# mmeidlinger/lut_ldpc

Hardware: AMD Instinct MI355X
Metric: decoded codewords/sec, DVB-S2 N=64800 4-bit LUT 50-iter (higher is better)
Workload: dtype u8

## Files before the change

### include/lut_ldpc_hip.h

```cpp
#ifndef LUT_LDPC_HIP_H
#define LUT_LDPC_HIP_H

#include <stdint.h>
#include <stddef.h>

#ifdef __cplusplus
extern "C" {
#endif

#define LUTLDPC_OK               0
#define LUTLDPC_ERR_ARG         -1
#define LUTLDPC_ERR_PARSE       -2
#define LUTLDPC_ERR_UNSUPPORTED -3
#define LUTLDPC_ERR_HIP         -4
#define LUTLDPC_ERR_STATE       -5

typedef struct lutldpc_decoder lutldpc_decoder;

const char *lutldpc_last_error(void);

const char *lutldpc_version(void);

int lutldpc_device_count(void);

int lutldpc_decoder_create(int nvar, int nchk, const int32_t *dv, const int32_t *dc,
                           const int32_t *cn_msg_idx,
                           int Nq_Cha, const int32_t *Nq_Msg, const uint8_t *reuse_vec, int max_iters,
                           int min_lut, const char *var_trees_txt, const char *chk_trees_txt,
                           int device, lutldpc_decoder **out);

int lutldpc_decoder_destroy(lutldpc_decoder *d);

int lutldpc_decoder_set_exit_conditions(lutldpc_decoder *d, int max_iters, int psc, int pisc);

int lutldpc_decoder_decode_batch(lutldpc_decoder *d, const uint8_t *cha, const uint8_t *msg0, int B,
                                 uint8_t *out_bits, int32_t *out_iters);

#define LUTLDPC_IN_BYTES   0
#define LUTLDPC_IN_NIBBLES 1
typedef struct {
    int32_t in_format;
    const int32_t *cha2msg_map;
    int32_t out_first, out_count;
} lutldpc_packed_io;

int lutldpc_decoder_decode_batch_packed(lutldpc_decoder *d, const lutldpc_packed_io *io, const uint8_t *cha, const uint8_t *msg0,
                                        int B, uint32_t *out_words, int32_t *out_iters);

int lutldpc_decoder_decode_batch_device(lutldpc_decoder *d, const uint8_t *d_cha, const uint8_t *d_msg0, int B,
                                        uint8_t *d_out_bits, int32_t *d_out_iters, int sync);

int lutldpc_decoder_decode_batch_trace(lutldpc_decoder *d, const uint8_t *cha, const uint8_t *msg0, int B, int level, uint8_t *out_bits,
                                       int32_t *out_iters, uint8_t *trace, int64_t trace_cap, int32_t *n_dumps);

int lutldpc_decoder_decode_llr_batch(lutldpc_decoder *d, const double *llr, int B,
                                     const double *qb_Cha, int n_qb_Cha,
                                     const double *qb_Msg, int n_qb_Msg,
                                     int initial_message_mode, const int32_t *cha2msg_map,
                                     uint8_t *out_bits, int32_t *out_iters);

#define LUTLDPC_LLR_F64 0
#define LUTLDPC_LLR_F32 1
#define LUTLDPC_LLR_F16 2
#define LUTLDPC_LLR_I8  3
typedef struct {
    int32_t dtype;
    int32_t on_device;
    int64_t frame_stride;
    double  scale;
    const double *qb_Cha; int32_t n_qb_Cha;
    const double *qb_Msg; int32_t n_qb_Msg;
    int32_t initial_message_mode; const int32_t *cha2msg_map;
    int32_t out_first, out_count;
    int32_t sync;
} lutldpc_llr_io;
int lutldpc_decoder_decode_llr_packed(lutldpc_decoder *d, const lutldpc_llr_io *io, const void *llr, int B,
                                      uint32_t *out_words, int32_t *out_iters, uint8_t *out_cha, uint8_t *out_msg0);

int lutldpc_llr_cell_table(const lutldpc_llr_io *io, int Nq_Cha, int Nq_Msg0,
                           double *thr, int32_t thr_cap, int32_t *n_thr,
                           uint8_t lut_cha[256], uint8_t lut_msg[256]);

typedef struct {
    int32_t n_cells;
    const uint64_t *thr;
    const uint8_t *cha_label;
    const uint8_t *msg_label;
    const uint8_t *slicer_neg;
    const uint8_t *cha_label_mirror;
    const uint8_t *msg_label_mirror;
} lutldpc_channel_cells;

#define LUTLDPC_STREAM_MAX 0x7FFFFFFFu
int lutldpc_check_stream(uint32_t stream);

int lutldpc_decoder_sim_batch(lutldpc_decoder *d, const lutldpc_channel_cells *cells, uint64_t seed, uint32_t stream,
                              uint64_t frame0, int B, const uint8_t *codewords, int K_info, int32_t *frame_stats,
                              uint8_t *cha_out, uint8_t *bits_out);

int lutldpc_decoder_set_generator(lutldpc_decoder *d, int K, int R, const uint64_t *rows);
int lutldpc_decoder_encode_random(lutldpc_decoder *d, uint64_t seed, uint32_t stream, uint64_t frame0, int B, uint8_t *codewords);
int lutldpc_decoder_sim_batch_random(lutldpc_decoder *d, const lutldpc_channel_cells *cells, uint64_t seed, uint32_t stream,
                                     uint64_t frame0, int B, int K_info, int32_t *frame_stats, uint8_t *cha_out, uint8_t *bits_out);

int lutldpc_decoder_sample_labels(lutldpc_decoder *d, const lutldpc_channel_cells *cells, uint64_t seed, uint32_t stream,
                                  uint64_t frame0, int B, const uint8_t *codewords, uint8_t *cha, uint8_t *msg0);

int lutldpc_decoder_set_edge_groups(lutldpc_decoder *d, const int32_t *edge_group, int n_groups);
int lutldpc_decoder_histogram_shape(lutldpc_decoder *d, int level, int32_t *out4);
int lutldpc_decoder_histogram_batch(lutldpc_decoder *d, const uint8_t *cha, const uint8_t *msg0, const uint8_t *sent, int B, int level, int mode,
                                    int n_labels, uint8_t *out_bits, int32_t *out_iters, int64_t *hist, int64_t hist_cap, int32_t *n_dumps);
int lutldpc_decoder_sim_batch_histogram(lutldpc_decoder *d, const lutldpc_channel_cells *cells, uint64_t seed, uint32_t stream, uint64_t frame0,
                                        int B, const uint8_t *codewords, int device_codewords, int level, int mode, int n_labels,
                                        int64_t *hist, int64_t hist_cap, int32_t *n_dumps);

#define LUTLDPC_EV_CODEWORD   0
#define LUTLDPC_EV_INFO       1
#define LUTLDPC_EV_FAILED     2
#define LUTLDPC_EV_UNDETECTED 3
typedef struct {
    int32_t select;
    int32_t max_frames, max_pos, max_chk;
    int32_t *events;
    int32_t *positions;
    int32_t *checks;
    int64_t *node_errors;
    int64_t *check_fails;
    int32_t n_selected;
    int32_t n_stored;
} lutldpc_event_request;

int lutldpc_decoder_events_batch(lutldpc_decoder *d, const uint8_t *cha, const uint8_t *msg0, const uint8_t *sent, int B, int K_info,
                                 uint8_t *out_bits, int32_t *out_iters, lutldpc_event_request *req);
int lutldpc_decoder_sim_batch_events(lutldpc_decoder *d, const lutldpc_channel_cells *cells, uint64_t seed, uint32_t stream, uint64_t frame0,
                                     int B, const uint8_t *codewords, int device_codewords, int K_info, int32_t *frame_stats,
                                     lutldpc_event_request *req);

void *lutldpc_decoder_stream(lutldpc_decoder *d);

#define LUTLDPC_K_CN_PASS   0
#define LUTLDPC_K_VN_PASS   1
#define LUTLDPC_K_DECISION  2
#define LUTLDPC_K_SYNDROME  3
#define LUTLDPC_K_LAYOUT    4
#define LUTLDPC_K_FRONTEND  5
#define LUTLDPC_K_FUSED_PASS 6
#define LUTLDPC_K_RESIDENT  7
#define LUTLDPC_K_HISTOGRAM 8
#define LUTLDPC_K_COUNT     9

int lutldpc_decoder_set_profiling(lutldpc_decoder *d, int enable);
int lutldpc_decoder_get_profile(lutldpc_decoder *d, int kind, double *total_ms, int64_t *launches);
int lutldpc_decoder_reset_profile(lutldpc_decoder *d);
int64_t lutldpc_decoder_device_bytes(lutldpc_decoder *d);
const char *lutldpc_decoder_describe(lutldpc_decoder *d);

int lutldpc_selftest_program_eval(lutldpc_decoder *d, int kind, int set, int cls,
                                  const int32_t *in, int n_in, int32_t *out, int n_out);
int lutldpc_selftest_program_stats(lutldpc_decoder *d, int kind, int set, int cls,
                                   int32_t *n_ops, int32_t *n_ops_naive, int32_t *n_slots);

int64_t lutldpc_selftest_jit_source(lutldpc_decoder *d, int kind, int set, int cls, char *buf, int64_t cap, int compile);
int64_t lutldpc_selftest_resident_source(lutldpc_decoder *d, int G, char *buf, int64_t cap, int compile, int32_t *info);

#ifdef __cplusplus
}
#endif
#endif
```

### lut_ldpc_amd/_capi.py

```python
from __future__ import annotations

import ctypes as C
import os
from pathlib import Path

_PKG = Path(__file__).resolve().parent
LIB_PATH = _PKG / "lib" / "liblut_ldpc_amd.so"
if os.environ.get("LUTLDPC_LIB"):
    LIB_PATH = Path(os.environ["LUTLDPC_LIB"])

OK, ERR_ARG, ERR_PARSE, ERR_UNSUPPORTED, ERR_HIP, ERR_STATE = 0, -1, -2, -3, -4, -5
K_CN_PASS, K_VN_PASS, K_DECISION, K_SYNDROME, K_LAYOUT, K_FRONTEND, K_FUSED_PASS, K_RESIDENT, K_HISTOGRAM, K_COUNT = 0, 1, 2, 3, 4, 5, 6, 7, 8, 9
KIND_NAMES = ["cn_pass", "vn_pass", "decision", "syndrome", "layout", "frontend", "fused_pass", "resident", "histogram"]


class LutLdpcError(RuntimeError):
    def __init__(self, code: int, msg: str):
        super().__init__(f"[{code}] {msg}")
        self.code = code


def _load() -> C.CDLL:
    if not LIB_PATH.exists():
        raise ImportError(
            f"{LIB_PATH} is missing: build it with `python -c 'import __graft_entry__ as g; g.build()'` "
            "or `make -C lut_ldpc_amd/csrc` (hipcc, gfx950). There is no CPU fallback."
        )
    return C.CDLL(str(LIB_PATH), mode=C.RTLD_GLOBAL)


lib = _load()

_vp, _ip, _u8p, _dp, _cp = C.c_void_p, C.POINTER(C.c_int32), C.POINTER(C.c_uint8), C.POINTER(C.c_double), C.c_char_p
_i64p = C.POINTER(C.c_int64)


class EventRequest(C.Structure):
    _fields_ = [("select", C.c_int32), ("max_frames", C.c_int32), ("max_pos", C.c_int32), ("max_chk", C.c_int32),
                ("events", _ip), ("positions", _ip), ("checks", _ip), ("node_errors", _i64p), ("check_fails", _i64p),
                ("n_selected", C.c_int32), ("n_stored", C.c_int32)]


_evp = C.POINTER(EventRequest)
IN_BYTES, IN_NIBBLES = 0, 1


class PackedIO(C.Structure):
    _fields_ = [("in_format", C.c_int32), ("cha2msg_map", _ip), ("out_first", C.c_int32), ("out_count", C.c_int32)]


LLR_F64, LLR_F32, LLR_F16, LLR_I8 = 0, 1, 2, 3


class LlrIO(C.Structure):
    _fields_ = [("dtype", C.c_int32), ("on_device", C.c_int32), ("frame_stride", C.c_int64), ("scale", C.c_double),
                ("qb_Cha", _dp), ("n_qb_Cha", C.c_int32), ("qb_Msg", _dp), ("n_qb_Msg", C.c_int32),
                ("initial_message_mode", C.c_int32), ("cha2msg_map", _ip), ("out_first", C.c_int32), ("out_count", C.c_int32),
                ("sync", C.c_int32)]


_u32p = C.POINTER(C.c_uint32)
_SIGNATURES = {
    "lutldpc_decoder_decode_llr_packed": (C.c_int, [_vp, C.POINTER(LlrIO), _vp, C.c_int, _vp, _vp, _vp, _vp]),
    "lutldpc_llr_cell_table": (C.c_int, [C.POINTER(LlrIO), C.c_int, C.c_int, _dp, C.c_int32, _ip, _u8p, _u8p]),
    "lutldpc_last_error": (_cp, []),
    "lutldpc_version": (_cp, []),
    "lutldpc_device_count": (C.c_int, []),
    "lutldpc_decoder_create": (C.c_int, [C.c_int, C.c_int, _ip, _ip, _ip, C.c_int, _ip, _u8p, C.c_int, C.c_int, _cp, _cp, C.c_int,
                                         C.POINTER(_vp)]),
    "lutldpc_decoder_destroy": (C.c_int, [_vp]),
    "lutldpc_decoder_set_exit_conditions": (C.c_int, [_vp, C.c_int, C.c_int, C.c_int]),
    "lutldpc_decoder_decode_batch": (C.c_int, [_vp, _u8p, _u8p, C.c_int, _u8p, _ip]),
    "lutldpc_decoder_decode_batch_packed": (C.c_int, [_vp, C.POINTER(PackedIO), _u8p, _u8p, C.c_int, _u32p, _ip]),
    "lutldpc_decoder_decode_batch_device": (C.c_int, [_vp, _vp, _vp, C.c_int, _vp, _vp, C.c_int]),
    "lutldpc_decoder_decode_llr_batch": (C.c_int, [_vp, _dp, C.c_int, _dp, C.c_int, _dp, C.c_int, C.c_int, _ip, _u8p, _ip]),
    "lutldpc_decoder_stream": (_vp, [_vp]),
    "lutldpc_decoder_set_profiling": (C.c_int, [_vp, C.c_int]),
    "lutldpc_decoder_get_profile": (C.c_int, [_vp, C.c_int, _dp, C.POINTER(C.c_int64)]),
    "lutldpc_decoder_reset_profile": (C.c_int, [_vp]),
    "lutldpc_decoder_device_bytes": (C.c_int64, [_vp]),
    "lutldpc_decoder_describe": (_cp, [_vp]),
    "lutldpc_selftest_program_eval": (C.c_int, [_vp, C.c_int, C.c_int, C.c_int, _ip, C.c_int, _ip, C.c_int]),
    "lutldpc_selftest_program_stats": (C.c_int, [_vp, C.c_int, C.c_int, C.c_int, _ip, _ip, _ip]),
    "lutldpc_decoder_decode_batch_trace": (C.c_int, [_vp, _u8p, _u8p, C.c_int, C.c_int, _u8p, _ip, _u8p, C.c_int64, _ip]),
    "lutldpc_selftest_jit_source": (C.c_int64, [_vp, C.c_int, C.c_int, C.c_int, C.c_char_p, C.c_int64, C.c_int]),
    "lutldpc_selftest_resident_source": (C.c_int64, [_vp, C.c_int, C.c_char_p, C.c_int64, C.c_int, C.POINTER(C.c_int32)]),
    "lutldpc_check_stream": (C.c_int, [C.c_uint32]),
    "lutldpc_decoder_set_generator": (C.c_int, [_vp, C.c_int, C.c_int, C.POINTER(C.c_uint64)]),
    "lutldpc_decoder_encode_random": (C.c_int, [_vp, C.c_uint64, C.c_uint32, C.c_uint64, C.c_int, _u8p]),
    "lutldpc_decoder_sim_batch_random": (C.c_int, [_vp, _vp, C.c_uint64, C.c_uint32, C.c_uint64, C.c_int, C.c_int, _ip, _u8p, _u8p]),
    "lutldpc_decoder_set_edge_groups": (C.c_int, [_vp, _ip, C.c_int]),
    "lutldpc_decoder_histogram_shape": (C.c_int, [_vp, C.c_int, _ip]),
    "lutldpc_decoder_histogram_batch": (C.c_int, [_vp, _u8p, _u8p, _u8p, C.c_int, C.c_int, C.c_int, C.c_int, _u8p, _ip, _i64p, C.c_int64, _ip]),
    "lutldpc_decoder_sim_batch_histogram": (C.c_int, [_vp, _vp, C.c_uint64, C.c_uint32, C.c_uint64, C.c_int, _u8p, C.c_int, C.c_int, C.c_int, C.c_int,
                                                      _i64p, C.c_int64, _ip]),
    "lutldpc_decoder_events_batch": (C.c_int, [_vp, _u8p, _u8p, _u8p, C.c_int, C.c_int, _u8p, _ip, _evp]),
    "lutldpc_decoder_sim_batch_events": (C.c_int, [_vp, _vp, C.c_uint64, C.c_uint32, C.c_uint64, C.c_int, _u8p, C.c_int, C.c_int, _ip, _evp]),
}
for _name, (_res, _args) in _SIGNATURES.items():
    if hasattr(lib, _name):
        _fn = getattr(lib, _name)
        _fn.restype, _fn.argtypes = _res, _args


def last_error() -> str:
    return lib.lutldpc_last_error().decode()


def check(rc: int) -> None:
    if rc != OK:
        raise LutLdpcError(rc, last_error())


def device_count() -> int:
    return lib.lutldpc_device_count()

_HOST_SIGNATURES = {
    "lutldpc_codec_create": (C.c_int, [_cp, C.c_int, C.c_int, C.c_int, C.POINTER(_vp)]),
    "lutldpc_codec_load": (C.c_int, [_cp, C.c_int, C.POINTER(_vp)]),
    "lutldpc_codec_save": (C.c_int, [_vp, _cp]),
    "lutldpc_codec_destroy": (C.c_int, [_vp]),
    "lutldpc_codec_design_luts": (C.c_int, [_vp, _cp, C.c_int, C.c_double, C.c_int, _u8p, C.c_int, _ip, C.c_int, _dp]),
    "lutldpc_codec_design_from_cache": (C.c_int, [_vp]),
    "lutldpc_codec_set_exit_conditions": (C.c_int, [_vp, C.c_int, C.c_int, C.c_int]),
    "lutldpc_codec_set_initial_message_mode": (C.c_int, [_vp, C.c_int]),
    "lutldpc_codec_initial_message_mode": (C.c_int, [_vp]),
    "lutldpc_codec_set_output_verbosity": (C.c_int, [_vp, C.c_int]),
    "lutldpc_codec_dims": (C.c_int, [_vp, _ip, _ip, _ip, _ip]),
    "lutldpc_codec_graph": (C.c_int, [_vp, _ip, _ip, _ip]),
    "lutldpc_codec_var_trees_txt": (C.c_int64, [_vp, C.c_char_p, C.c_int64]),
    "lutldpc_codec_chk_trees_txt": (C.c_int64, [_vp, C.c_char_p, C.c_int64]),
    "lutldpc_codec_qb": (C.c_int, [_vp, C.c_int, _dp, C.c_int]),
    "lutldpc_codec_cha2msg_map": (C.c_int, [_vp, _ip, C.c_int]),
    "lutldpc_codec_rate": (C.c_double, [_vp]),
    "lutldpc_codec_decoder": (_vp, [_vp]),
    "lutldpc_codec_decode_llr_batch": (C.c_int, [_vp, _dp, C.c_int, _u8p, _ip]),
    "lutldpc_codec_lut_decode_batch": (C.c_int, [_vp, _u8p, _u8p, C.c_int, _u8p, _ip]),
    "lutldpc_codec_lut_decode_dump": (C.c_int64, [_vp, _u8p, _u8p, C.c_int, C.c_int, _u8p, _ip, C.c_char_p, C.c_int64]),
    "lutldpc_codec_encode": (C.c_int, [_vp, _u8p, _u8p]),
    "lutldpc_de_threshold": (C.c_int, [_ip, _dp, C.c_int, _ip, _dp, C.c_int, C.c_int, C.c_int, C.c_int, C.c_int, _cp, _cp, C.c_double,
                                       C.c_double, C.c_double, C.c_int, C.c_int, C.c_double, C.c_int, _dp]),
}
for _name, (_res, _args) in _HOST_SIGNATURES.items():
    if hasattr(lib, _name):
        _fn = getattr(lib, _name)
        _fn.restype, _fn.argtypes = _res, _args

_u64p, _i64p = C.POINTER(C.c_uint64), C.POINTER(C.c_int64)
_SIM_SIGNATURES = {
    "lutldpc_codec_sim_batch": (C.c_int, [_vp, C.c_double, C.c_uint64, C.c_uint32, C.c_uint64, C.c_int, C.c_int, _ip]),
    "lutldpc_codec_sample_labels": (C.c_int, [_vp, C.c_double, C.c_uint64, C.c_uint32, C.c_uint64, C.c_int, C.c_int, _u8p, _u8p, _u8p]),
    "lutldpc_codec_encode_random": (C.c_int, [_vp, C.c_uint64, C.c_uint32, C.c_uint64, C.c_int, _u8p]),
    "lutldpc_codec_channel_cells": (C.c_int, [_vp, C.c_double, _u64p, _u8p, _u8p, _u8p, _u8p, _u8p]),
    "lutldpc_ber_sim_run": (C.c_int, [_cp, _cp, C.c_int, _cp, C.c_int, C.c_int, C.c_int, _dp, _i64p, C.c_int]),
    "lutldpc_ber_sim_main": (C.c_int, [C.c_int, C.POINTER(C.c_char_p)]),
    "lutldpc_selftest_write_results_it": (C.c_int, [_cp, _dp, _i64p, C.c_int, C.c_int, C.c_int, C.c_double]),
    "lutldpc_bersim_create": (C.c_int, [_cp, _cp, C.c_int, _cp, C.c_int, C.POINTER(_vp)]),
    "lutldpc_bersim_destroy": (C.c_int, [_vp]),
    "lutldpc_bersim_info": (C.c_int, [_vp, _i64p, _dp, _dp, C.c_int]),
    "lutldpc_bersim_batch": (C.c_int, [_vp, C.c_int, C.c_int64, C.c_int, _ip]),
    "lutldpc_bersim_add_point": (C.c_int, [_vp, C.c_double, _i64p]),
    "lutldpc_bersim_save": (C.c_int, [_vp, C.c_double]),
    "lutldpc_bersim_results_path": (C.c_int64, [_vp, C.c_char_p, C.c_int64]),
    "lutldpc_codec_message_histogram": (C.c_int, [_vp, C.c_double, C.c_uint64, C.c_uint32, C.c_uint64, C.c_int, C.c_int, C.c_int, C.c_int, C.c_int,
                                                  _i64p, C.c_int64, _ip]),
    "lutldpc_bersim_message_histogram": (C.c_int, [_vp, C.c_int, C.c_int64, C.c_int, C.c_int, C.c_int, C.c_int, _i64p, C.c_int64, _ip]),
    "lutldpc_codec_error_events": (C.c_int, [_vp, C.c_double, C.c_uint64, C.c_uint32, C.c_uint64, C.c_int, C.c_int, _evp]),
    "lutldpc_bersim_error_events": (C.c_int, [_vp, C.c_int, C.c_int64, C.c_int, _evp]),
    "lutldpc_bersim_decoder": (_vp, [_vp]),
    "lutldpc_bersim_code": (C.c_int, [_vp, _ip, _ip, _ip, _ip, _ip]),
}
for _name, (_res, _args) in _SIM_SIGNATURES.items():
    if hasattr(lib, _name):
        _fn = getattr(lib, _name)
        _fn.restype, _fn.argtypes = _res, _args
```

### lut_ldpc_amd/csrc/hip/decoder.hip

```cpp
#include "decoder_state.hpp"

#include <climits>
#include <cstdlib>

#pragma GCC visibility push(hidden)

static thread_local std::string g_err;
int fail(int code, const std::string &msg) { g_err = msg; return code; }

hipEvent_t ev_get(lutldpc_decoder *d) {
    if (!d->ev_pool.empty()) { hipEvent_t e = d->ev_pool.back(); d->ev_pool.pop_back(); return e; }
    hipEvent_t e;
    (void)hipEventCreate(&e);
    return e;
}
void prof_fold(lutldpc_decoder *d) {
    if (d->ev_live.empty()) return;
    (void)hipStreamSynchronize(d->stream);
    for (auto &e : d->ev_live) {
        float ms = 0;
        if (hipEventElapsedTime(&ms, e.a, e.b) == hipSuccess) { d->prof_ms[e.kind] += ms; d->prof_n[e.kind]++; }
        d->ev_pool.push_back(e.a); d->ev_pool.push_back(e.b);
    }
    d->ev_live.clear();
}

static uint32_t crc32(uint32_t crc, const void *p, size_t n) {
    crc = ~crc;
    for (size_t i = 0; i < n; i++) {
        crc ^= static_cast<const uint8_t *>(p)[i];
        for (int k = 0; k < 8; k++) crc = (crc >> 1) ^ (0xEDB88320u & (0u - (crc & 1u)));
    }
    return ~crc;
}

void make_describe(lutldpc_decoder *d) {
    std::ostringstream o;
    o << "{\"build\":\"" << __DATE__ << " " << __TIME__ << "\",\"kernel_sources\":\"" <<
#include "kernel_src_hash.inc"
      << "\",\"tile_frames\":" << d->tile() << ",\"message_bytes\":" << (d->pack == 2 ? "0.5" : "1") << ",\"pack\":" << d->pack << ",\"vector_bytes_per_lane\":4"
      << ",\"nodes_per_block\":" << d->opt.nodes_per_block << ",\"vn_edges_per_wave\":" << d->opt.vn_edges_per_wave << ",\"cn_edges_per_wave\":" << d->cn_epw() << ",\"use_fast\":" << d->opt.use_fast
      << ",\"nodes_per_wave\":" << d->opt.nodes_per_wave << ",\"nodes_per_wave_cn\":" << d->opt.nodes_per_wave_cn << ",\"tail_front\":" << d->opt.tail_front
      << ",\"fused_prio\":" << d->opt.fused_prio << ",\"chk_full_labels\":" << d->opt.chk_full_labels
      << ",\"vn_classes\":[";
    for (size_t i = 0; i < d->vclass.size(); i++) {
        const TreeClassPlan *t = d->tree_class(TT_VAR, 0, (int)i);
        const bool f = t && fast_covers(d, t->fast, d->vclass[i].deg);
        o << (i ? "," : "") << "{\"deg\":" << d->vclass[i].deg << ",\"nodes\":" << d->vclass[i].nodes.size() << ",\"nodes_per_wave\":" << d->npw_vn(d->vclass[i].deg) << ",\"kernel\":\""
          << (f ? "vn_balanced_fast_kernel" : t && t->jit ? "lutldpc_jit_pass" : "tree_pass_kernel<VAR>") << "\"}";
    }
    o << "],\"cn_classes\":[";
    for (size_t i = 0; i < d->cclass.size(); i++) {
        int n_fast = 0;
        for (int nq : d->Nq_Msg)
            n_fast += d->opt.use_fast && d->min_lut && cn_minsum_shape(nq / 2, d->cclass[i].deg);
        const char *minsum = n_fast == (int)d->Nq_Msg.size() ? "cn_minsum_fast_kernel"
                           : n_fast == 0 ? "cn_minsum_generic_kernel" : "cn_minsum_fast_kernel+cn_minsum_generic_kernel";
        int chained = 0;
        if (d->opt.use_chain && d->cclass[i].chain_off >= 0)
            for (size_t j = 0; j < d->cclass[i].nodes.size(); j++) chained += d->fast_idx[(size_t)d->cclass[i].chain_off + 2 * j + 1] != 0;
        const TreeClassPlan *t = d->tree_class(TT_CHK, 0, (int)i);
        o << (i ? "," : "") << "{\"deg\":" << d->cclass[i].deg << ",\"nodes\":" << d->cclass[i].nodes.size() << ",\"nodes_per_wave\":" << d->npw_cn_class(i)
          << ",\"chain_nodes\":" << chained << ",\"kernel\":\""
          << (d->min_lut ? minsum
                         : t && t->jit ? "lutldpc_jit_pass" : "tree_pass_kernel<CHK>") << "\"}";
    }
    o << "],\"resident\":" << (resident_active(d) ? 1 : 0) << ",\"skewed_pipeline\":" << ((d->opt.skew && d->skew_ok) ? 1 : 0) << ",\"fused_bucket\":" << d->fused_bucket_id << ",\"compaction\":" << (d->opt.use_compact < 0 ? 2 : d->opt.use_compact) << ",\"compaction_min_groups\":" << compaction_min_groups(d) << ",\"chain_nodes\":" << (d->opt.use_chain ? d->n_chain_nodes : 0) << ",\"placement\":" << d->place_info;
    if (d->gen_set) o << ",\"generator\":{\"K\":" << d->gen_K << ",\"R\":" << d->gen_R << "}";
    {
        uint32_t ops = 0;
        for (const Op &op : d->all_ops) ops = crc32(crc32(ops, &op, offsetof(Op, child) + sizeof(op.child)), &op.mult, sizeof(Op) - offsetof(Op, mult));
        char b[160];
        snprintf(b, sizeof(b), ",\"static\":{\"ops\":%zu,\"ops_crc\":\"%08x\",\"tables_bytes\":%zu,\"tables_crc\":\"%08x\",\"index_words\":%zu,\"index_crc\":\"%08x\"}", d->all_ops.size(), ops,
                 d->all_tables.size(), crc32(0, d->all_tables.data(), d->all_tables.size()), d->fast_idx.size(), crc32(0, d->fast_idx.data(), 4 * d->fast_idx.size()));
        o << b;
    }
    o << "}";
    d->describe = o.str();
}

using Options = lutldpc_decoder::Options;
enum KnobType { FLAG, INT, REAL, REAL_BELOW };
struct Knob { const char *name; KnobType type; int Options::*i; double Options::*r; double lo, hi; const char *meaning; };
#define KNOB_F(name, field, meaning) {name, FLAG, &Options::field, nullptr, 0, 1, meaning}
#define KNOB_I(name, field, lo, hi, meaning) {name, INT, &Options::field, nullptr, lo, hi, meaning}
#define KNOB_R(name, type, field, lo, hi, meaning) {name, type, nullptr, &Options::field, lo, hi, meaning}
static const Knob kKnobs[] = {
    KNOB_F("LUTLDPC_USE_FAST", use_fast, "1: compile-time specialised kernels (and with them the fused pipeline, the generated kernels, the resident decoder); 0: interpreter kernels only"),
    KNOB_F("LUTLDPC_JIT", use_jit, "1: run-time generated kernels for shapes the compile-time path does not cover (jit.hpp)"),
    KNOB_I("LUTLDPC_PACK", pack, 1, 1, "1: byte rows even where every alphabet has <= 16 labels (unset: nibble rows there)"),
    KNOB_F("LUTLDPC_CHK_FULL", chk_full_labels, "1: generated check kernels on full-label tables; 0: on (sign, magnitude) tables as the reference walks them"),
    KNOB_F("LUTLDPC_COMPOSE", use_compose, "1: exact table composition for the resident kernel's trees (measured slower: LDS bank conflicts, see compile_all)"),
    KNOB_I("LUTLDPC_COMPOSE_SPACE", compose_space, 0, 65536, "largest composed table, entries"),
    KNOB_F("LUTLDPC_CHAIN", use_chain, "1: degree-2 nodes between neighbouring checks of a wave are updated inside the check pass (build_fast_index)"),
    KNOB_F("LUTLDPC_LATE_HARD", late_hard, "1: decided bits of early-terminated frames recovered once, at the end, from their frozen messages; 0: stored by every variable pass"),
    KNOB_F("LUTLDPC_FIRST_FROM_NODES", first_from_nodes, "1: the first check pass reads the initial-message rows; 0: init_edges_kernel copies them to the edge rows first"),
    KNOB_I("LUTLDPC_NODES_PER_BLOCK", nodes_per_block, 1, 4096, "interpreter kernels: nodes per 64-thread block"),
    KNOB_I("LUTLDPC_NODES_PER_WAVE", nodes_per_wave, 1, 4096, "specialised kernels: fixed nodes per wave, variable AND check side (unset: edges per wave / degree)"),
    KNOB_I("LUTLDPC_NODES_PER_WAVE_CN", nodes_per_wave_cn, 1, 4096, "... check side only (overrides LUTLDPC_NODES_PER_WAVE there)"),
    KNOB_I("LUTLDPC_VN_EDGES_PER_WAVE", vn_edges_per_wave, 1, 65536, "variable side: edges per wave"),
    KNOB_I("LUTLDPC_CN_EDGES_PER_WAVE", cn_edges_per_wave, 1, 65536, "check side: edges per wave (unset: 42, chain-rich classes widened by build_fast_index; given: no widening)"),
    KNOB_F("LUTLDPC_SKEW", skew, "1: two-half skewed pipeline through pass_fused_kernel where every class has a case in it"),
    KNOB_I("LUTLDPC_FUSED_BUCKET_MIN", fused_bucket_min, 0, kFusedBuckets - 1, "run a code of small degrees through a wider bucket's fused kernel (can only widen; what a bucket costs)"),
    KNOB_F("LUTLDPC_PRIO", fused_prio, "1: the look-up-heavy (variable) waves of the fused kernel raise their issue priority (no gain measured)"),
    KNOB_R("LUTLDPC_TAIL_FRONT", REAL_BELOW, tail_front, 0, 0.9, "fused launches: share of the item list that the slowest role stays clear of at the end"),
    KNOB_I("LUTLDPC_PLACE", place_candidates, 0, 32, "placement search of the row buffers: at most n candidate allocations, 0 / 1: off (place_rows)"),
    KNOB_F("LUTLDPC_GRAPH", use_graph, "1: repeated decodes replayed as one hipGraph launch"),
    KNOB_F("LUTLDPC_COMPACT", use_compact, "1 / 0: on / off (unset: automatic, long iterations only -- compaction_on)"),
    KNOB_F("LUTLDPC_COMPACT_KEEP", compact_keep, "1: frames that left keep their rows, bits recovered once at the end; 0: recovered at the check point, rows dropped"),
    KNOB_I("LUTLDPC_COMPACT_FIRST", compact_first, 1, INT_MAX, "first iteration with a check point"),
    KNOB_I("LUTLDPC_COMPACT_EVERY", compact_every, 1, INT_MAX, "iterations between check points (unset: 2)"),
    KNOB_R("LUTLDPC_COMPACT_MARGIN", REAL_BELOW, compact_margin, 0, 100, "permute when the remaining iterations pay for it by this factor (0: whenever a group falls idle)"),
    KNOB_R("LUTLDPC_COMPACT_MIN_SHARE", REAL, compact_min_share, 0, 1, "... and at least this share of the live groups falls idle at once"),
    KNOB_I("LUTLDPC_RESIDENT", use_resident, INT_MIN, INT_MAX, "0: off (streaming kernels); 1: where the code fits and it pays; >= 2: wherever it fits"),
    KNOB_I("LUTLDPC_RESIDENT_S", resident_force_S, 1, 64, "sets (64 frames each) per workgroup (unset: resident_pick)"),
    KNOB_I("LUTLDPC_RESIDENT_NT", resident_force_NT, 256, 1024, "threads per workgroup: 256, 512, 768 or 1024 (unset: resident_pick)"),
    KNOB_I("LUTLDPC_RESIDENT_U", resident_U, 1, 4, "frames per lane step of the variable items: 1, 2 or 4 (unset: generator's choice)"),
    KNOB_F("LUTLDPC_RESIDENT_XCD", resident_xcd, "1: workgroup ids remapped so that neighbours share an XCD"),
    KNOB_F("LUTLDPC_RESIDENT_FM", resident_fm, "1: the kernel reads / writes the caller's frame-major buffers itself; 0: always through the row layout"),
    KNOB_F("LUTLDPC_RESIDENT_FLAG_REDUCE", resident_flag_reduce, "wave-reduced exit-test flags (unset: small trees only, resident_spec)"),
    KNOB_F("LUTLDPC_RESIDENT_CN_PERSISTENT", resident_cn_persistent, "check items keep their LDS addresses in registers (unset: where registers allow, resident_spec)"),
    KNOB_I("LUTLDPC_RESIDENT_WAVES_EU", resident_waves_eu, 0, 8, "amdgpu_waves_per_eu of the generated kernel (0: none)"),
    KNOB_F("LUTLDPC_VALIDATE", validate, "1: the class parameters of every per-class launch checked against the allocation sizes (fused roles always are), stream synchronised after every launch so that a device fault names ONE launch; no graph replay"),
    KNOB_F("LUTLDPC_DEBUG_ADDR", debug_addr, "1: print where the row buffers landed (tools/config4_place_ab.sh)"),
};
#undef KNOB_F
#undef KNOB_I
#undef KNOB_R

static void read_knobs(Options &o) {
    for (const Knob &k : kKnobs) {
        const char *e = getenv(k.name);
        if (!e) continue;
        if (k.type == FLAG) o.*k.i = atoi(e) ? 1 : 0;
        else if (k.type == INT) { const int v = atoi(e); if (v >= k.lo && v <= k.hi) o.*k.i = v; }
        else { const double v = atof(e); if (v >= k.lo && (k.type == REAL ? v <= k.hi : v < k.hi)) o.*k.r = v; }
    }
    if (o.nodes_per_wave_cn == 0) o.nodes_per_wave_cn = o.nodes_per_wave;
    o.use_resident = o.use_resident >= 2 ? 2 : o.use_resident ? 1 : 0;
    if (o.resident_force_NT % 256) o.resident_force_NT = 0;
    if (o.resident_U == 3) o.resident_U = 0;
    if (o.validate) o.use_graph = 0;
    o.compact_margin = (float)o.compact_margin; o.compact_min_share = (float)o.compact_min_share;
}

lutldpc_decoder::~lutldpc_decoder() {
    if (device < 0) return;
    (void)hipSetDevice(device);
    if (stream) (void)hipStreamSynchronize(stream);
    drop_graphs();
    for (auto &e : ev_live) { (void)hipEventDestroy(e.a); (void)hipEventDestroy(e.b); }
    for (auto &e : ev_pool) (void)hipEventDestroy(e);
}

static int decode_staged_labels(lutldpc_decoder *d, int B, uint8_t *out_bits, int32_t *out_iters) {
    const size_t n = (size_t)B * (size_t)d->nvar;
    HIP_TRY(d->d_out_bits.alloc(n)); HIP_TRY(d->d_out_iters.alloc((size_t)B));
    int rc = decode_device(d, d->d_in_cha.p, d->d_in_msg.p, B, d->d_out_bits.p, d->d_out_iters.p);
    if (rc || (rc = copy_to_host(d, out_bits, d->d_out_bits.p, n)) || (rc = iters_to_host(d, out_iters, B))) return rc;
    HIP_TRY(hipStreamSynchronize(d->stream));
    return LUTLDPC_OK;
}

struct TraceScope {
    lutldpc_decoder *d;
    explicit TraceScope(lutldpc_decoder *d_) : d(d_) {}
    ~TraceScope() { d->trace = lutldpc_decoder::Trace(); }
};

#pragma GCC visibility pop

extern "C" {

const char *lutldpc_last_error(void) { return g_err.c_str(); }
void lutldpc_set_last_error(const char *msg) { g_err = msg ? msg : ""; }
const char *lutldpc_version(void) { return "lut_ldpc_amd 0.1 gfx950"; }

int lutldpc_device_count(void) {
    int n = 0;
    if (hipGetDeviceCount(&n) != hipSuccess) return 0;
    return n;
}

int lutldpc_decoder_create(int nvar, int nchk, const int32_t *dv, const int32_t *dc, const int32_t *cn_msg_idx,
                           int Nq_Cha, const int32_t *Nq_Msg, const uint8_t *reuse_vec, int max_iters,
                           int min_lut, const char *var_trees_txt, const char *chk_trees_txt, int device,
                           lutldpc_decoder **out) {
    if (!out) return fail(LUTLDPC_ERR_ARG, "out is NULL");
    *out = nullptr;
    if (nvar <= 0 || nchk <= 0 || !dv || !dc || !cn_msg_idx || !Nq_Msg || !reuse_vec || max_iters < 1 || !var_trees_txt)
        return fail(LUTLDPC_ERR_ARG, "missing or non-positive argument");
    if (Nq_Cha < 2 || Nq_Cha > 128 || (Nq_Cha & 1)) return fail(LUTLDPC_ERR_ARG, "Nq_Cha must be even and in [2,128]");
    for (int i = 0; i < max_iters; i++)
        if (Nq_Msg[i] < 2 || Nq_Msg[i] > 128 || (Nq_Msg[i] & 1)) return fail(LUTLDPC_ERR_ARG, "Nq_Msg entries must be even and in [2,128]");
    if (reuse_vec[0] || reuse_vec[max_iters - 1]) return fail(LUTLDPC_ERR_ARG, "first and last iteration are exempt from tree reuse");
    std::unique_ptr<lutldpc_decoder> d(new lutldpc_decoder);
    d->nvar = nvar; d->nchk = nchk;
    d->dv.assign(dv, dv + nvar); d->dc.assign(dc, dc + nchk);
    long long ev = 0, ec = 0;
    for (int v = 0; v < nvar; v++) { if (dv[v] < 1 || dv[v] > 255) return fail(LUTLDPC_ERR_ARG, "variable degree outside [1,255]"); ev += dv[v]; }
    for (int c = 0; c < nchk; c++) { if (dc[c] < 1 || dc[c] > 255) return fail(LUTLDPC_ERR_ARG, "check degree outside [1,255]"); ec += dc[c]; }
    if (ev != ec || ev > (1ll << 30)) return fail(LUTLDPC_ERR_ARG, "sum(dv) != sum(dc)");
    d->E = (int)ev;
    d->cn_msg_idx.assign(cn_msg_idx, cn_msg_idx + d->E);
    d->vn_ptr.resize((size_t)nvar + 1); d->cn_ptr.resize((size_t)nchk + 1);
    for (int v = 0; v < nvar; v++) d->vn_ptr[(size_t)v + 1] = d->vn_ptr[(size_t)v] + dv[v];
    for (int c = 0; c < nchk; c++) d->cn_ptr[(size_t)c + 1] = d->cn_ptr[(size_t)c] + dc[c];
    {
        d->edge_vn.resize((size_t)d->E);
        for (int v = 0; v < nvar; v++) for (int e = d->vn_ptr[(size_t)v]; e < d->vn_ptr[(size_t)v + 1]; e++) d->edge_vn[(size_t)e] = v;
        std::vector<uint8_t> seen((size_t)d->E, 0);
        d->cn_vn.resize((size_t)d->E);
        for (int k = 0; k < d->E; k++) {
            int e = cn_msg_idx[k];
            if (e < 0 || e >= d->E || seen[(size_t)e]) return fail(LUTLDPC_ERR_ARG, "cn_msg_idx is not a permutation of the edges");
            seen[(size_t)e] = 1;
            d->cn_vn[(size_t)k] = d->edge_vn[(size_t)e];
        }
    }
    if ((uint64_t)d->E * kRowBytes >= (1ull << 32) || (uint64_t)nvar * kRowBytes >= (1ull << 32))
        return fail(LUTLDPC_ERR_UNSUPPORTED, "code too large: the rows of one frame group must stay below 4 GiB");
    build_classes(d->dv, d->vclass, d->vn_list);
    build_classes(d->dc, d->cclass, d->cn_list);
    d->Nq_Cha = Nq_Cha; d->Nq_Msg.assign(Nq_Msg, Nq_Msg + max_iters);
    d->max_iters_created = d->max_iters = max_iters; d->psc = 1; d->pisc = 0; d->min_lut = min_lut ? 1 : 0;
    d->iter_set.resize((size_t)max_iters);
    { int cum = 0; for (int i = 0; i < max_iters; i++) { cum += reuse_vec[i] ? 0 : 1; d->iter_set[(size_t)i] = cum - 1; } }
    std::string err;
    if (!parse_tree_array(var_trees_txt, d->var_trees, err)) return fail(LUTLDPC_ERR_PARSE, "var_trees_txt: " + err);
    if (!d->min_lut) {
        if (!chk_trees_txt || !parse_tree_array(chk_trees_txt, d->chk_trees, err)) return fail(LUTLDPC_ERR_PARSE, "chk_trees_txt: " + err);
    }
    read_knobs(d->opt);
    d->pack = 2;
    if (Nq_Cha > 16 || d->opt.pack == 1) d->pack = 1;
    for (int i = 0; i < max_iters; i++) if (Nq_Msg[i] > 16) d->pack = 1;
    int rc = compile_all(d.get());
    if (rc) return rc;
    d->skew_ok = skew_eligible(d.get());
    {
        int max_cn = 0, max_vn = 0;
        for (auto &c : d->cclass) max_cn = std::max(max_cn, c.deg);
        for (auto &c : d->vclass) max_vn = std::max(max_vn, c.deg);
        d->fused_bucket_id = std::max(0, fused_bucket(max_vn, max_cn));
        const int v = d->opt.fused_bucket_min;
        if (v >= 0 && fused_bucket_rank(v) > fused_bucket_rank(d->fused_bucket_id)) d->fused_bucket_id = v;
    }
    d->device = device;
    if (device >= 0) { rc = upload_static(d.get()); if (rc) return rc; }
    d->resident_ok = resident_eligible(d.get());
    make_describe(d.get());
    *out = d.release();
    return LUTLDPC_OK;
}

int lutldpc_decoder_destroy(lutldpc_decoder *d) {
    if (!d) return LUTLDPC_OK;
    delete d;
    return LUTLDPC_OK;
}

int lutldpc_decoder_set_exit_conditions(lutldpc_decoder *d, int max_iters, int psc, int pisc) {
    if (!d) return fail(LUTLDPC_ERR_ARG, "NULL decoder");
    if (max_iters < 1 || max_iters > d->max_iters_created) return fail(LUTLDPC_ERR_ARG, "max_iters outside [1, value at creation]");
    if (!d->tree_set(TT_DEC, d->iter_set[(size_t)(max_iters - 1)])->valid)
        return fail(LUTLDPC_ERR_ARG, "the tree set of iteration max_iters-1 is not a decision tree set");
    d->max_iters = max_iters; d->psc = psc ? 1 : 0; d->pisc = pisc ? 1 : 0;
    return LUTLDPC_OK;
}

int lutldpc_decoder_decode_batch_device(lutldpc_decoder *d, const uint8_t *d_cha, const uint8_t *d_msg0, int B,
                                        uint8_t *d_out_bits, int32_t *d_out_iters, int sync) {
    if (!d || !d_cha || !d_msg0 || !d_out_bits || !d_out_iters) return fail(LUTLDPC_ERR_ARG, "NULL argument");
    int rc = batch_entry(d, B);
    if (rc || (rc = decode_device(d, d_cha, d_msg0, B, d_out_bits, d_out_iters))) return rc;
    if (sync) HIP_TRY(hipStreamSynchronize(d->stream));
    return LUTLDPC_OK;
}

int lutldpc_decoder_decode_batch(lutldpc_decoder *d, const uint8_t *cha, const uint8_t *msg0, int B, uint8_t *out_bits, int32_t *out_iters) {
    if (!d || !cha || !msg0 || !out_bits || !out_iters) return fail(LUTLDPC_ERR_ARG, "NULL argument");
    int rc = batch_entry(d, B);
    if (rc || (rc = labels_from_host(d, cha, msg0, B))) return rc;
    return decode_staged_labels(d, B, out_bits, out_iters);
}

int lutldpc_decoder_decode_batch_trace(lutldpc_decoder *d, const uint8_t *cha, const uint8_t *msg0, int B, int level, uint8_t *out_bits, int32_t *out_iters,
                                       uint8_t *trace, int64_t trace_cap, int32_t *n_dumps) {
    if (!d || !cha || !msg0 || !out_bits || !out_iters || !trace) return fail(LUTLDPC_ERR_ARG, "NULL argument");
    if (level < 2 || level > 3) return fail(LUTLDPC_ERR_ARG, "trace level must be 2 or 3");
    int rc = batch_entry(d, B);
    if (rc) return rc;
    if (B > 4096) return fail(LUTLDPC_ERR_ARG, "the message trace is a debug path: 1..4096 frames");
    const int64_t need = (int64_t)(1 + d->max_iters * (level - 1)) * B * d->E;
    if (trace_cap < need) return fail(LUTLDPC_ERR_ARG, "trace buffer too small: " + std::to_string(need) + " bytes needed");
    TraceScope scope(d);
    d->trace.level = level; d->trace.host = trace; d->trace.cap = (size_t)trace_cap; d->trace.n = 0; d->trace.B = B;
    if ((rc = labels_from_host(d, cha, msg0, B)) == LUTLDPC_OK) rc = decode_staged_labels(d, B, out_bits, out_iters);
    if (n_dumps) *n_dumps = d->trace.n;
    return rc;
}

int lutldpc_decoder_decode_llr_batch(lutldpc_decoder *d, const double *llr, int B, const double *qb_Cha, int n_qb_Cha,
                                     const double *qb_Msg, int n_qb_Msg, int mode, const int32_t *map,
                                     uint8_t *out_bits, int32_t *out_iters) {
    if (!d || !llr || !qb_Cha || !out_bits || !out_iters) return fail(LUTLDPC_ERR_ARG, "NULL argument");
    int rc = batch_entry(d, B);
    if (rc) return rc;
    if (n_qb_Cha != d->Nq_Cha - 1) return fail(LUTLDPC_ERR_ARG, "qb_Cha must hold Nq_Cha-1 boundaries");
    if (mode == 0 && (!qb_Msg || n_qb_Msg != d->Nq_Msg[0] - 1)) return fail(LUTLDPC_ERR_ARG, "qb_Msg must hold Nq_Msg[0]-1 boundaries");
    if (mode == 1 && !map) return fail(LUTLDPC_ERR_ARG, "QCHA mode needs cha2msg_map");
    if (mode != 0 && mode != 1) return fail(LUTLDPC_ERR_ARG, "initial_message_mode must be 0 (CONT) or 1 (QCHA)");
    size_t n = (size_t)B * (size_t)d->nvar;
    HIP_TRY(d->d_llr.alloc(n)); HIP_TRY(d->d_in_cha.alloc(n)); HIP_TRY(d->d_in_msg.alloc(n));
    HIP_TRY(d->d_qb_cha.alloc((size_t)n_qb_Cha)); HIP_TRY(d->d_qb_msg.alloc((size_t)(n_qb_Msg > 0 ? n_qb_Msg : 1))); HIP_TRY(d->d_map.alloc((size_t)d->Nq_Cha));
    HIP_TRY(hipMemcpyAsync(d->d_llr.p, llr, n * sizeof(double), hipMemcpyHostToDevice, d->stream));
    HIP_TRY(hipMemcpyAsync(d->d_qb_cha.p, qb_Cha, sizeof(double) * (size_t)n_qb_Cha, hipMemcpyHostToDevice, d->stream));
    if (mode == 0) HIP_TRY(hipMemcpyAsync(d->d_qb_msg.p, qb_Msg, sizeof(double) * (size_t)n_qb_Msg, hipMemcpyHostToDevice, d->stream));
    else HIP_TRY(hipMemcpyAsync(d->d_map.p, map, sizeof(int32_t) * (size_t)d->Nq_Cha, hipMemcpyHostToDevice, d->stream));
    if ((rc = launch_quantize_llr(d, n, n_qb_Cha, n_qb_Msg, mode))) return rc;
    return decode_staged_labels(d, B, out_bits, out_iters);
}

void *lutldpc_decoder_stream(lutldpc_decoder *d) { return d ? (void *)d->stream.s : nullptr; }

int lutldpc_decoder_set_profiling(lutldpc_decoder *d, int enable) {
    if (!d) return fail(LUTLDPC_ERR_ARG, "NULL decoder");
    if (!enable && d->device >= 0) prof_fold(d);
    d->profiling = enable != 0;
    return LUTLDPC_OK;
}
int lutldpc_decoder_get_profile(lutldpc_decoder *d, int kind, double *total_ms, int64_t *launches) {
    if (!d || kind < 0 || kind >= LUTLDPC_K_COUNT) return fail(LUTLDPC_ERR_ARG, "bad kind");
    if (d->device >= 0) prof_fold(d);
    if (total_ms) *total_ms = d->prof_ms[kind];
    if (launches) *launches = d->prof_n[kind];
    return LUTLDPC_OK;
}
int lutldpc_decoder_reset_profile(lutldpc_decoder *d) {
    if (!d) return fail(LUTLDPC_ERR_ARG, "NULL decoder");
    if (d->device >= 0) prof_fold(d);
    for (int i = 0; i < LUTLDPC_K_COUNT; i++) { d->prof_ms[i] = 0; d->prof_n[i] = 0; }
    return LUTLDPC_OK;
}
int64_t lutldpc_decoder_device_bytes(lutldpc_decoder *d) {
    if (!d) return 0;
    return (int64_t)(d->d_msgs.bytes() + d->d_cha_t.bytes() + d->d_msg0_t.bytes() + d->d_hard.bytes() + d->d_state.bytes() + d->d_vfail.bytes() +
                     d->d_iters.bytes() + d->d_in_cha.bytes() + d->d_in_msg.bytes() + d->d_out_bits.bytes() + d->d_out_iters.bytes() + d->d_llr.bytes() + d->d_llr_in.bytes() +
                     d->d_ops.bytes() + d->d_tables.bytes() + d->d_cn_idx.bytes() + d->d_cn_vn.bytes());
}
const char *lutldpc_decoder_describe(lutldpc_decoder *d) { return d ? d->describe.c_str() : ""; }

static const Program *find_prog(lutldpc_decoder *d, int kind, int set, int cls) {
    const bool full = kind == TT_CHK + 32, comp = !full && (kind & 16) != 0;
    const TreeClassPlan *c = d->tree_class(full ? TT_CHK : kind & 15, set, cls);
    if (!c || (full && c->full.tab.bytes == 0)) return nullptr;
    return full ? &c->full.prog : comp ? &c->composed.prog : &c->base.prog;
}
int lutldpc_selftest_program_eval(lutldpc_decoder *d, int kind, int set, int cls, const int32_t *in, int n_in, int32_t *out, int n_out) {
    if (!d || !in || !out) return fail(LUTLDPC_ERR_ARG, "NULL argument");
    const Program *p = find_prog(d, kind, set, cls);
    if (!p) return fail(LUTLDPC_ERR_ARG, "no such program");
    if (n_in != p->n_in || n_out != p->n_out) return fail(LUTLDPC_ERR_ARG, "program arity mismatch");
    if (!eval_program(*p, in, out)) return fail(LUTLDPC_ERR_ARG, "input label outside its alphabet");
    return LUTLDPC_OK;
}
int lutldpc_selftest_program_stats(lutldpc_decoder *d, int kind, int set, int cls, int32_t *n_ops, int32_t *n_ops_naive, int32_t *n_slots) {
    if (!d) return fail(LUTLDPC_ERR_ARG, "NULL decoder");
    const Program *p = find_prog(d, kind, set, cls);
    if (!p) return fail(LUTLDPC_ERR_ARG, "no such program");
    if (n_ops) *n_ops = (int32_t)p->ops.size();
    if (n_ops_naive) *n_ops_naive = p->n_ops_naive;
    if (n_slots) *n_slots = p->n_slots;
    return LUTLDPC_OK;
}

static int64_t give_source(const std::string &src, char *buf, int64_t cap, int compile) {
    if (compile) {
        std::vector<char> code; std::string log;
        if (!jit_compile(src, code, log)) return fail(LUTLDPC_ERR_HIP, "hiprtc: " + log.substr(0, 4000));
    }
    if (buf && cap > (int64_t)src.size()) std::memcpy(buf, src.c_str(), src.size() + 1);
    return (int64_t)src.size() + 1;
}

int64_t lutldpc_selftest_jit_source(lutldpc_decoder *d, int kind, int set, int cls, char *buf, int64_t cap, int compile) {
    if (!d) return fail(LUTLDPC_ERR_ARG, "NULL decoder");
    const Program *p = find_prog(d, kind, set, cls);
    if (!p) return fail(LUTLDPC_ERR_ARG, "no such program");
    std::string src, err;
    if (!jit_class_source(d, kind, (size_t)set, (size_t)cls, src, err)) return fail(LUTLDPC_ERR_UNSUPPORTED, err);
    return give_source(src, buf, cap, compile);
}

int64_t lutldpc_selftest_resident_source(lutldpc_decoder *d, int G, char *buf, int64_t cap, int compile, int32_t *info) {
    if (!d || G < 1) return fail(LUTLDPC_ERR_ARG, "NULL decoder / bad G");
    int S = 0, NT = 0, lds = 0;
    if (!resident_pick(d, G, S, NT, lds)) return fail(LUTLDPC_ERR_UNSUPPORTED, "resident decoder: the code does not fit the LDS");
    std::string src, err;
    if (!jit_resident_source(resident_spec(d, S, NT), src, err)) return fail(LUTLDPC_ERR_UNSUPPORTED, "resident decoder: " + err);
    if (info) { info[0] = S; info[1] = NT; info[2] = lds; }
    return give_source(src, buf, cap, compile);
}

}
```

### lut_ldpc_amd/csrc/hip/decoder_setup.hip

```cpp
#include "decoder_state.hpp"

#pragma GCC visibility push(hidden)

void build_classes(const std::vector<int> &deg, std::vector<NodeClass> &cls, std::vector<int> &list) {
    std::map<int, std::vector<int>> by;
    for (size_t i = 0; i < deg.size(); i++) by[deg[i]].push_back((int)i);
    cls.clear(); list.clear();
    for (auto &kv : by) { NodeClass c; c.deg = kv.first; c.nodes = kv.second; cls.push_back(std::move(c)); }
    for (auto &c : cls) list.insert(list.end(), c.nodes.begin(), c.nodes.end());
}

static int build_plan(lutldpc_decoder *d, const std::vector<NodeClass> &cls, const TreeSetPlan *set, PassPlan &plan) {
    if ((int)cls.size() > kMaxSeg) return fail(LUTLDPC_ERR_UNSUPPORTED, "more than 32 distinct node degrees in one pass");
    PassParams &P = plan.P;
    std::memset(&P, 0, sizeof(P));
    P.n_seg = (int)cls.size();
    P.nodes_per_block = d->opt.nodes_per_block;
    P.E = d->E; P.N = d->nvar;
    int blk = 0, node_off = 0, max_slots = 0, max_tab = 0, max_out = 1;
    for (size_t i = 0; i < cls.size(); i++) {
        PassSeg &S = P.seg[i];
        S.block_begin = blk;
        S.n_nodes = (int)cls[i].nodes.size();
        S.node_off = node_off;
        S.deg = cls[i].deg;
        if (set) {
            const TreeClassPlan &c = set->cls[i];
            const Program &pr = c.base.prog;
            S.op_off = c.op_off; S.n_ops = (int)pr.ops.size();
            S.tab_off = c.base.tab.off; S.tab_bytes = c.base.tab.bytes;
            S.n_in = pr.n_in; S.n_out = pr.n_out; S.n_slots = pr.n_slots;
            max_slots = std::max(max_slots, pr.n_slots);
            max_tab = std::max(max_tab, c.base.tab.bytes);
            max_out = std::max(max_out, pr.n_out);
        }
        blk += (S.n_nodes + P.nodes_per_block - 1) / P.nodes_per_block;
        node_off += S.n_nodes;
    }
    P.blocks_per_group = blk;
    P.slots_lds = max_slots;
    plan.out_slots = max_out;
    int slots_bytes = (max_slots + max_out) * kWave * 4;
    if (slots_bytes > 60 * 1024) return fail(LUTLDPC_ERR_UNSUPPORTED, "node program needs more than 60 KiB of LDS slots");
    plan.lds_tab = (slots_bytes + max_tab) <= 64 * 1024;
    plan.lds_bytes = slots_bytes + (plan.lds_tab ? max_tab : 0);
    plan.valid = true;
    return LUTLDPC_OK;
}

static void build_fast_index(lutldpc_decoder *d) {
    d->fast_idx.clear();
    for (auto &c : d->cclass) { c.chain_off = -1; c.npw = 0; }
    for (auto &c : d->vclass) {
        c.red_off = -1; c.red_n = 0;
        c.idx_off = (int)d->fast_idx.size();
        for (int v : c.nodes) { d->fast_idx.push_back(v); d->fast_idx.push_back(d->vn_ptr[(size_t)v]); }
    }
    std::vector<int> edge_chk((size_t)d->E, -1), cls_of((size_t)d->nchk, -1), pos_of((size_t)d->nchk, -1);
    for (int c = 0; c < d->nchk; c++)
        for (int k = d->cn_ptr[(size_t)c]; k < d->cn_ptr[(size_t)c + 1]; k++) edge_chk[(size_t)d->cn_msg_idx[(size_t)k]] = c;
    for (size_t ci = 0; ci < d->cclass.size(); ci++)
        for (size_t j = 0; j < d->cclass[ci].nodes.size(); j++) { cls_of[(size_t)d->cclass[ci].nodes[j]] = (int)ci; pos_of[(size_t)d->cclass[ci].nodes[j]] = (int)j; }
    std::vector<int> back((size_t)d->nchk, 0), fwd((size_t)d->nchk, 0);
    std::vector<char> internal((size_t)d->nvar, 0);
    if (d->opt.use_chain && d->min_lut) {
        std::vector<int> cand(d->cclass.size(), 0);
        for (int v = 0; v < d->nvar; v++) {
            if (d->dv[(size_t)v] != 2) continue;
            const int e0 = d->vn_ptr[(size_t)v], c1 = edge_chk[(size_t)e0], c2 = edge_chk[(size_t)e0 + 1];
            if (c1 < 0 || c2 < 0 || c1 == c2 || cls_of[(size_t)c1] != cls_of[(size_t)c2]) continue;
            if (std::abs(pos_of[(size_t)c1] - pos_of[(size_t)c2]) == 1) cand[(size_t)cls_of[(size_t)c1]]++;
        }
        for (size_t ci = 0; ci < d->cclass.size(); ci++)
            if (2 * cand[ci] >= (int)d->cclass[ci].nodes.size() && d->opt.nodes_per_wave_cn <= 0) {
                const int n = (int)d->cclass[ci].nodes.size();
                d->cclass[ci].npw = std::max(4, d->npw_cn(d->cclass[ci].deg));
                if (d->opt.cn_edges_per_wave <= 0) d->cclass[ci].npw = std::max(d->cclass[ci].npw, std::min(12, n / 2048));
            }
    }
    if (d->opt.use_chain && d->min_lut)
        for (int v = 0; v < d->nvar; v++) {
            if (d->dv[(size_t)v] != 2) continue;
            const int e0 = d->vn_ptr[(size_t)v];
            int c1 = edge_chk[(size_t)e0], c2 = edge_chk[(size_t)e0 + 1];
            if (c1 < 0 || c2 < 0 || c1 == c2 || cls_of[(size_t)c1] != cls_of[(size_t)c2]) continue;
            if (pos_of[(size_t)c1] > pos_of[(size_t)c2]) std::swap(c1, c2);
            const int deg = d->cclass[(size_t)cls_of[(size_t)c1]].deg, npw = d->npw_cn_class((size_t)cls_of[(size_t)c1]);
            if (deg < 2 || deg > fused_max_cn_deg() || pos_of[(size_t)c2] != pos_of[(size_t)c1] + 1 || pos_of[(size_t)c1] / npw != pos_of[(size_t)c2] / npw) continue;
            if (fwd[(size_t)c1] || back[(size_t)c2]) continue;
            fwd[(size_t)c1] = v + 1; back[(size_t)c2] = v + 1; internal[(size_t)v] = 1;
        }
    for (size_t ci = 0; ci < d->cclass.size(); ci++) {
        auto &c = d->cclass[ci];
        c.idx_off = (int)d->fast_idx.size();
        bool any = false;
        for (int cn : c.nodes) {
            std::vector<int> es;
            for (int k = 0; k < c.deg; k++) es.push_back(d->cn_msg_idx[(size_t)(d->cn_ptr[(size_t)cn] + k)]);
            auto to_slot = [&](int v1, size_t slot) {
                if (!v1) return;
                for (size_t k = 0; k < es.size(); k++)
                    if (es[k] == d->vn_ptr[(size_t)(v1 - 1)] || es[k] == d->vn_ptr[(size_t)(v1 - 1)] + 1) { std::swap(es[k], es[slot]); return; }
            };
            to_slot(back[(size_t)cn], 0); to_slot(fwd[(size_t)cn], 1);
            if (back[(size_t)cn] && fwd[(size_t)cn] && c.deg >= 2) {
                const int vb = back[(size_t)cn] - 1;
                if (es[0] != d->vn_ptr[(size_t)vb] && es[0] != d->vn_ptr[(size_t)vb] + 1) to_slot(back[(size_t)cn], 0);
            }
            for (int e : es) d->fast_idx.push_back(e);
            any = any || back[(size_t)cn] || fwd[(size_t)cn];
        }
        if (any) {
            c.chain_off = (int)d->fast_idx.size();
            for (int cn : c.nodes) { d->fast_idx.push_back(back[(size_t)cn]); d->fast_idx.push_back(fwd[(size_t)cn]); }
        }
    }
    for (auto &c : d->cclass) {
        const size_t off = (size_t)c.idx_off, cnt = c.nodes.size() * (size_t)c.deg;
        c.nidx_off = (int)d->fast_idx.size();
        for (size_t j = 0; j < cnt; j++) d->fast_idx.push_back(d->edge_vn[(size_t)d->fast_idx[off + j]]);
    }
    for (auto &c : d->cclass) {
        const size_t n = c.nodes.size();
        c.tidx_off = (int)d->fast_idx.size();
        for (int k = 0; k < c.deg; k++) for (size_t j = 0; j < n; j++) d->fast_idx.push_back(d->cn_msg_idx[(size_t)(d->cn_ptr[(size_t)c.nodes[j]] + k)]);
        c.tnidx_off = (int)d->fast_idx.size();
        for (int k = 0; k < c.deg; k++) for (size_t j = 0; j < n; j++) d->fast_idx.push_back(d->edge_vn[(size_t)d->cn_msg_idx[(size_t)(d->cn_ptr[(size_t)c.nodes[j]] + k)]]);
    }
    for (auto &c : d->vclass) {
        c.tidx_off = (int)d->fast_idx.size();
        for (int v : c.nodes) d->fast_idx.push_back(v);
        for (int v : c.nodes) d->fast_idx.push_back(d->vn_ptr[(size_t)v]);
    }
    for (size_t vi = 0; vi < d->vclass.size(); vi++) {
        auto &c = d->vclass[vi];
        if (c.deg != 2) continue;
        c.red_off = (int)d->fast_idx.size();
        for (int v : c.nodes)
            if (!internal[(size_t)v]) { d->fast_idx.push_back(v); d->fast_idx.push_back(d->vn_ptr[(size_t)v]); c.red_n++; }
        d->chain_vclass = (int)vi;
    }
    d->n_chain_nodes = 0;
    for (char x : internal) d->n_chain_nodes += x;
    d->chain_internal.assign(internal.begin(), internal.end());
}

static int validate_fast_index(const lutldpc_decoder *d) {
    const size_t n = d->fast_idx.size();
    int rc = LUTLDPC_OK;
    auto check = [&](const char *name, int off, size_t cnt, size_t first, size_t step, int hi) {
        if (rc) return;
        if (off < 0 || (size_t)off + cnt > n) { rc = fail(LUTLDPC_ERR_STATE, std::string("index table check failed: ") + name + " table outside the blob"); return; }
        for (size_t j = first; j < cnt && !rc; j += step)
            if (d->fast_idx[(size_t)off + j] < 0 || d->fast_idx[(size_t)off + j] >= hi) rc = fail(LUTLDPC_ERR_STATE, std::string("index table check failed: ") + name + " entry out of range");
    };
    for (const auto &c : d->vclass) {
        const size_t m = c.nodes.size(), r = (size_t)c.red_n;
        const int N = d->nvar, e_hi = d->E - c.deg + 1;
        check("variable class", c.idx_off, 2 * m, 0, 2, N); check("variable class", c.idx_off, 2 * m, 1, 2, e_hi);
        if (c.red_off >= 0) { check("reduced variable class", c.red_off, 2 * r, 0, 2, N); check("reduced variable class", c.red_off, 2 * r, 1, 2, e_hi); }
        check("transposed variable class", c.tidx_off, m, 0, 1, N); check("transposed variable class", c.tidx_off, 2 * m, m, 1, e_hi);
    }
    for (const auto &c : d->cclass) {
        const size_t cnt = c.nodes.size() * (size_t)c.deg;
        check("check class edge", c.idx_off, cnt, 0, 1, d->E); check("check class node", c.nidx_off, cnt, 0, 1, d->nvar);
        check("transposed check class edge", c.tidx_off, cnt, 0, 1, d->E); check("transposed check class node", c.tnidx_off, cnt, 0, 1, d->nvar);
        if (c.chain_off >= 0) check("chain link", c.chain_off, 2 * c.nodes.size(), 0, 1, d->nvar + 1);
    }
    return rc;
}

static void append_tables(lutldpc_decoder *d, ProgramForm &f, bool align16) {
    while (align16 && (d->all_tables.size() & 15)) d->all_tables.push_back(0);
    f.tab = {(int)d->all_tables.size(), (int)f.prog.tables.size()};
    d->all_tables.insert(d->all_tables.end(), f.prog.tables.begin(), f.prog.tables.end());
}

static int add_forms(lutldpc_decoder *d, int kind, int s, bool composed) {
    const std::vector<Tree> &trees = (kind == TT_CHK ? d->chk_trees : d->var_trees)[(size_t)s];
    const std::vector<NodeClass> &cls = kind == TT_CHK ? d->cclass : d->vclass;
    TreeSetPlan &S = *d->tree_set(kind, s);
    if (!composed) S.cls.assign(cls.size(), TreeClassPlan());
    for (size_t i = 0; i < cls.size(); i++) {
        if (cls[i].tree_class >= (int)trees.size()) return fail(LUTLDPC_ERR_ARG, "tree set is missing a degree class");
        const Tree &t = trees[(size_t)cls[i].tree_class];
        TreeClassPlan &c = S.cls[i];
        ProgramForm &f = composed ? c.composed : c.base;
        std::string e;
        if (!(composed ? compile_program(compose_tree(t, kind, d->opt.use_compose ? (uint64_t)d->opt.compose_space : 0), kind, cls[i].deg, f.prog, e)
                       : compile_program(t, kind, cls[i].deg, f.prog, e)))
            return fail(LUTLDPC_ERR_UNSUPPORTED, (composed ? "composed tree, degree " : "degree ") + std::to_string(cls[i].deg) + ": " + e);
        append_tables(d, f, false);
        if (composed) { f.prog.node_tabs.clear(); continue; }
        c.op_off = (int)d->all_ops.size();
        d->all_ops.insert(d->all_ops.end(), f.prog.ops.begin(), f.prog.ops.end());
        if (kind != TT_CHK) {
            std::map<const TreeNode *, std::pair<uint32_t, uint32_t>> tab_of;
            for (auto &nt : f.prog.node_tabs) tab_of[nt.first] = {(uint32_t)f.tab.off + nt.second[0], nt.second[1]};
            c.fast = plan_fast_vn(t, kind, cls[i].deg, tab_of);
        }
    }
    if (!composed) {
        if (int rc = build_plan(d, cls, &S, S.pass)) return rc;
        S.valid = true;
    }
    for (size_t i = 0; i < cls.size() && kind == TT_CHK && d->opt.chk_full_labels; i++) {
        ProgramForm f;
        if (!chk_full_label_program((composed ? S.cls[i].composed : S.cls[i].base).prog, f.prog) || f.prog.tables.empty()) continue;
        append_tables(d, f, true);
        (composed ? S.cls[i].composed_full : S.cls[i].full) = std::move(f);
    }
    return LUTLDPC_OK;
}

int compile_all(lutldpc_decoder *d) {
    std::string err;
    build_fast_index(d);
    if (int rc = validate_fast_index(d)) return rc;
    if (d->var_trees.empty()) return fail(LUTLDPC_ERR_ARG, "no variable-node trees");
    int n_sets = 0;
    for (int i = 0; i < d->max_iters_created; i++) n_sets = std::max(n_sets, d->iter_set[(size_t)i] + 1);
    if ((int)d->var_trees.size() < n_sets) return fail(LUTLDPC_ERR_ARG, "fewer variable tree sets than reuse_vec requires");
    for (auto &c : d->vclass) {
        c.tree_class = -1;
        for (size_t k = 0; k < d->var_trees[0].size(); k++) if (d->var_trees[0][k].num_leaves == c.deg) { c.tree_class = (int)k; break; }
        if (c.tree_class < 0) return fail(LUTLDPC_ERR_ARG, "no variable tree for degree " + std::to_string(c.deg));
    }
    if (!d->min_lut) {
        if ((int)d->chk_trees.size() < n_sets) return fail(LUTLDPC_ERR_ARG, "fewer check tree sets than reuse_vec requires");
        for (auto &c : d->cclass) {
            c.tree_class = -1;
            for (size_t k = 0; k < d->chk_trees[0].size(); k++) if (d->chk_trees[0][k].num_leaves + 1 == c.deg) { c.tree_class = (int)k; break; }
            if (c.tree_class < 0) return fail(LUTLDPC_ERR_ARG, "no check tree for degree " + std::to_string(c.deg));
        }
    }
    d->all_ops.clear(); d->all_tables.clear();
    for (auto &plans : d->tree_plans) plans.assign((size_t)n_sets, TreeSetPlan());
    for (int s = 0; s < n_sets; s++) {
        const int vkind = !d->var_trees[(size_t)s].empty() && d->var_trees[(size_t)s][0].type == TT_DEC ? TT_DEC : TT_VAR;
        int rc;
        if ((rc = add_forms(d, vkind, s, false))) return rc;
        if (!d->min_lut && (rc = add_forms(d, TT_CHK, s, false))) return rc;
        if ((rc = add_forms(d, vkind, s, true))) return rc;
        if (!d->min_lut && (rc = add_forms(d, TT_CHK, s, true))) return rc;
    }
    if (d->min_lut) { int rc = build_plan(d, d->cclass, nullptr, d->cn_minsum_plan); if (rc) return rc; }
    return LUTLDPC_OK;
}

JitRegistry &jit_registry() { static JitRegistry *r = new JitRegistry; return *r; }

JitKernel *jit_get(int device, const std::string &src, std::string &log) {
    JitRegistry &reg = jit_registry();
    std::lock_guard<std::mutex> lock(reg.mu);
    const std::string key = std::to_string(device) + "\n" + src;
    auto it = reg.by_src.find(key);
    if (it == reg.by_src.end()) {
        if (reg.by_src.size() >= kJitRegistryMax) return nullptr;
        std::vector<char> code; JitKernel k; std::string out;
        if (!jit_compile(src, code, out) || !jit_load(code, k, out)) { k = JitKernel(); log = out.empty() ? "hiprtc returned no code object" : out; }
        it = reg.by_src.emplace(key, k).first;
    }
    return &it->second;
}

bool jit_class_source(const lutldpc_decoder *d, int kind, size_t s, size_t i, std::string &src, std::string &err) {
    const bool full = kind == TT_CHK + 32;
    const TreeClassPlan *c = d->tree_class(full ? TT_CHK : kind, (int)s, (int)i);
    if (!c || (full && c->full.tab.bytes == 0)) { err = "only variable / decision / check-tree programs are generated"; return false; }
    const ProgramForm &f = full ? c->full : c->base;
    return full || kind == TT_CHK ? jit_cn_source(f.prog, d->cclass[i].deg, d->pack, f.tab.bytes, src, err)
                                 : jit_vn_source(f.prog, kind, d->vclass[i].deg, d->pack, f.tab.bytes, src, err);
}

static int preload_code_objects(int device) {
    static std::mutex mu;
    static std::vector<int> done;
    std::lock_guard<std::mutex> lock(mu);
    if (std::find(done.begin(), done.end(), device) != done.end()) return LUTLDPC_OK;
    HIP_TRY(preload_stream_kernels()); HIP_TRY(preload_frontend_kernels());
    HIP_TRY((preload_fused<2, 0>())); HIP_TRY((preload_fused<2, 1>())); HIP_TRY((preload_fused<2, 2>())); HIP_TRY((preload_fused<2, 3>()));
    HIP_TRY((preload_vn_fast<TT_VAR, 1>())); HIP_TRY((preload_vn_fast<TT_VAR, 2>())); HIP_TRY((preload_vn_fast<TT_DEC, 2>()));
    HIP_TRY((preload_cn_fast<2>()));
    HIP_TRY(preload_compact_kernels());
    HIP_TRY(preload_stats_kernels());
    HIP_TRY(preload_events_kernels());
    HIP_TRY(preload_packed_kernels());
    HIP_TRY(preload_llr_kernels());
    HIP_TRY(hipDeviceSynchronize());
    done.push_back(device);
    return LUTLDPC_OK;
}

static void build_jit(lutldpc_decoder *d) {
    if (!d->opt.use_jit || !d->opt.use_fast) return;
    for (size_t s = 0; s < d->tree_plans[TT_VAR].size(); s++)
        for (int kind : {TT_VAR, TT_DEC, TT_CHK}) {
            TreeSetPlan &S = *d->tree_set(kind, (int)s);
            const auto &cls = kind == TT_CHK ? d->cclass : d->vclass;
            for (size_t i = 0; i < S.cls.size(); i++) {
                if (kind != TT_CHK && fast_covers(d, S.cls[i].fast, cls[i].deg)) continue;
                std::string src, log;
                const bool full = kind == TT_CHK && d->chk_form((int)s, (int)i, false) == &S.cls[i].full;
                if (!jit_class_source(d, full ? TT_CHK + 32 : kind, s, i, src, log)) { d->jit_log = log; continue; }
                JitKernel *k = jit_get(d->device, src, log);
                if (!k) { d->jit_log = "generated-kernel registry full"; continue; }
                if (!log.empty()) d->jit_log = log;
                if (k->ok()) S.cls[i].jit = k;
            }
        }
}

int upload_static(lutldpc_decoder *d) {
    HIP_TRY(hipSetDevice(d->device));
    if (int rc = preload_code_objects(d->device)) return rc;
    HIP_TRY(hipStreamCreateWithFlags(&d->stream.s, hipStreamNonBlocking));
    HIP_TRY(d->d_vn_ptr.upload(d->vn_ptr));
    HIP_TRY(d->d_cn_ptr.upload(d->cn_ptr));
    HIP_TRY(d->d_cn_idx.upload(d->cn_msg_idx));
    {
        std::vector<int32_t> f((size_t)d->E + 8, 0);
        for (int c = 0; c < d->nchk; c++)
            for (int k = d->cn_ptr[(size_t)c]; k < d->cn_ptr[(size_t)c + 1]; k++)
                f[(size_t)k] = (int32_t)((uint32_t)d->cn_vn[(size_t)k] | (k + 1 == d->cn_ptr[(size_t)c + 1] ? 0x80000000u : 0u));
        HIP_TRY(d->d_cn_vn.upload(f));
    }
    HIP_TRY(d->d_vn_list.upload(d->vn_list));
    HIP_TRY(d->d_cn_list.upload(d->cn_list));
    HIP_TRY(d->d_fast_idx.upload(d->fast_idx));
    HIP_TRY(d->d_chain_internal.upload(d->chain_internal));
    HIP_TRY(d->d_edge_vn.upload(d->edge_vn));
    HIP_TRY(d->d_ops.upload(d->all_ops));
    {
        std::vector<uint8_t> t = d->all_tables;
        t.resize((t.size() + 3) / 4 * 4 + 16, 0);
        HIP_TRY(d->d_tables.upload(t));
    }
    build_jit(d);
    return LUTLDPC_OK;
}

#pragma GCC visibility pop
```

### lut_ldpc_amd/csrc/hip/decoder_state.hpp

```cpp
#pragma once
#include "../../../include/lut_ldpc_hip.h"
#include "kernels_common.hpp"
#include "kernels_fast.hpp"
#include "lut_program.hpp"
#include "jit.hpp"
#include "jit_resident.hpp"

#include <algorithm>
#include <array>
#include <cmath>
#include <cstdio>
#include <cstring>
#include <map>
#include <memory>
#include <mutex>
#include <sstream>
#include <string>
#include <vector>

namespace lutldpc { LUTLDPC_FAST_LAUNCHERS(extern) }
namespace lutldpc { struct ChannelCells; }

using namespace lutldpc;

#pragma GCC visibility push(hidden)

int fail(int code, const std::string &msg);

#define HIP_TRY(expr)                                                                               \
    do {                                                                                            \
        hipError_t e_ = (expr);                                                                     \
        if (e_ != hipSuccess)                                                                       \
            return fail(LUTLDPC_ERR_HIP, std::string(#expr) + ": " + hipGetErrorString(e_));        \
    } while (0)

template <class T>
struct DevBuf {
    T *p = nullptr;
    size_t n = 0;
    DevBuf() = default;
    DevBuf(const DevBuf &) = delete;
    DevBuf &operator=(const DevBuf &) = delete;
    DevBuf(DevBuf &&o) noexcept : p(o.p), n(o.n) { o.p = nullptr; o.n = 0; }
    DevBuf &operator=(DevBuf &&o) noexcept {
        if (this != &o) { release(); p = o.p; n = o.n; o.p = nullptr; o.n = 0; }
        return *this;
    }
    ~DevBuf() { release(); }
    hipError_t alloc(size_t count) {
        if (count <= n) return hipSuccess;
        release();
        hipError_t e = hipMalloc((void **)&p, count * sizeof(T));
        if (e == hipSuccess) n = count; else p = nullptr;
        return e;
    }
    hipError_t upload(const std::vector<T> &h) {
        hipError_t e = alloc(h.size() ? h.size() : 1);
        if (e != hipSuccess || h.empty()) return e;
        return hipMemcpy(p, h.data(), h.size() * sizeof(T), hipMemcpyHostToDevice);
    }
    void release() { if (p) (void)hipFree(p); p = nullptr; n = 0; }
    size_t bytes() const { return n * sizeof(T); }
};

struct StreamHolder {
    hipStream_t s = nullptr;
    StreamHolder() = default;
    StreamHolder(const StreamHolder &) = delete;
    StreamHolder &operator=(const StreamHolder &) = delete;
    ~StreamHolder() { if (s) (void)hipStreamDestroy(s); }
    operator hipStream_t() const { return s; }
};

struct NodeClass {
    int deg = 0;
    std::vector<int> nodes;
    int tree_class = -1;
    int idx_off = 0, tidx_off = 0;
    int nidx_off = 0, tnidx_off = 0, chain_off = -1, npw = 0;
    int red_off = -1, red_n = 0;
};

struct PassPlan {
    PassParams P{};
    int lds_bytes = 0;
    int out_slots = 0;
    bool lds_tab = true;
    bool valid = false;
};

struct TreeClassPlan {
    ProgramForm base;
    int op_off = 0;
    ProgramForm full;
    ProgramForm composed, composed_full;
    FastClassPlan fast;
    const JitKernel *jit = nullptr;
};
struct TreeSetPlan {
    bool valid = false;
    PassPlan pass;
    std::vector<TreeClassPlan> cls;
};

#pragma GCC visibility pop

struct lutldpc_decoder {
    struct Options {
        int nodes_per_block = 16;
        int use_fast = 1;
        int pack = 0;
        int nodes_per_wave = 0, nodes_per_wave_cn = 0;
        int vn_edges_per_wave = 16, cn_edges_per_wave = 0;
        int first_from_nodes = 1;
        int use_jit = 1;
        int use_compose = 0, compose_space = 4096;
        int chk_full_labels = 1;
        int use_chain = 1;
        int use_resident = 1, resident_force_S = 0, resident_force_NT = 0, resident_U = 0, resident_xcd = 1, resident_fm = 1;
        int resident_flag_reduce = -1, resident_cn_persistent = -1, resident_waves_eu = 0;
        int place_candidates = 16;
        int use_compact = -1, compact_keep = 1, compact_first = 8, compact_every = 0;
        double compact_margin = 1.0, compact_min_share = 0.35;
        int use_graph = 1;
        int fused_prio = 0;
        double tail_front = 0.25;
        int skew = 1;
        int late_hard = 1;
        int validate = 0;
        int fused_bucket_min = -1;
        int debug_addr = 0;
    } opt;
    int nvar = 0, nchk = 0, E = 0;
    std::vector<int> dv, dc, cn_msg_idx, vn_ptr, cn_ptr, cn_vn;
    std::vector<NodeClass> vclass, cclass;
    std::vector<int> vn_list, cn_list;
    int Nq_Cha = 0, max_iters_created = 0, max_iters = 0, psc = 1, pisc = 0, min_lut = 1;
    std::vector<int> Nq_Msg, iter_set;
    TreeArray var_trees, chk_trees;
    std::vector<TreeSetPlan> tree_plans[3];
    const TreeSetPlan *tree_set(int kind, int set) const {
        return kind >= 0 && kind < 3 && set >= 0 && (size_t)set < tree_plans[kind].size() ? &tree_plans[kind][(size_t)set] : nullptr;
    }
    const TreeClassPlan *tree_class(int kind, int set, int cls) const {
        const TreeSetPlan *s = tree_set(kind, set);
        return s && cls >= 0 && (size_t)cls < s->cls.size() ? &s->cls[(size_t)cls] : nullptr;
    }
    const ProgramForm *chk_form(int set, int cls, bool composed) const {
        const TreeClassPlan *c = tree_class(TT_CHK, set, cls);
        if (!c) return nullptr;
        const ProgramForm &f = composed ? c->composed_full : c->full;
        return f.tab.bytes > 0 ? &f : composed ? &c->composed : &c->base;
    }
    TreeSetPlan *tree_set(int kind, int set) { return const_cast<TreeSetPlan *>(const_cast<const lutldpc_decoder *>(this)->tree_set(kind, set)); }
    TreeClassPlan *tree_class(int kind, int set, int cls) { return const_cast<TreeClassPlan *>(const_cast<const lutldpc_decoder *>(this)->tree_class(kind, set, cls)); }
    std::vector<Op> all_ops;
    std::vector<uint8_t> all_tables;
    PassPlan cn_minsum_plan;
    std::vector<int32_t> fast_idx;
    int chain_vclass = -1, n_chain_nodes = 0;
    std::vector<uint8_t> chain_internal;
    std::vector<int32_t> edge_vn;
    int pack = 1;
    bool skew_ok = false;
    int fused_bucket_id = 0;
    bool resident_ok = false;
    int device = -1;
    StreamHolder stream;
    DevBuf<int32_t> d_vn_ptr, d_cn_ptr, d_cn_idx, d_cn_vn, d_vn_list, d_cn_list, d_fast_idx;
    DevBuf<Op> d_ops;
    DevBuf<uint8_t> d_tables;
    DevBuf<uint8_t> d_chain_internal;
    DevBuf<int32_t> d_edge_vn;
    int Bcap = 0;
    DevBuf<uint8_t> d_msgs, d_cha_t, d_msg0_t, d_hard, d_state, d_vfail;
    DevBuf<int32_t> d_iters;
    DevBuf<uint8_t> d_in_cha, d_in_msg, d_out_bits;
    DevBuf<int32_t> d_out_iters;
    DevBuf<uint32_t> d_out_words;
    DevBuf<double> d_llr, d_qb_cha, d_qb_msg;
    DevBuf<uint64_t> d_llr_in;
    DevBuf<int32_t> d_map;
    DevBuf<uint8_t> d_codewords;
    DevBuf<int32_t> d_stats;
    bool gen_set = false;
    int gen_K = 0, gen_R = 0, gen_W32p = 0;
    DevBuf<uint32_t> d_gen;
    DevBuf<uint8_t> d_sent;
    DevBuf<int32_t> d_frame_of, d_perm, d_tmp3, d_ctl, d_slot_of, d_iters_tmp;
    DevBuf<int32_t> d_grp;
    struct ParamArena {
        std::map<std::string, size_t> off_of;
        std::vector<DevBuf<uint8_t>> chunks;
        std::vector<size_t> chunk_base;
        size_t used = 0, cap = 0;
        void clear() { chunks.clear(); chunk_base.clear(); off_of.clear(); used = cap = 0; }
    } params;
    struct Trace {
        int level = 0; uint8_t *host = nullptr; size_t cap = 0; int n = 0; int B = 0;
        unsigned long long *hist = nullptr; const uint8_t *sent = nullptr; const int32_t *last_dump = nullptr; int n_labels = 0, n_dumps = 0;
    };
    Trace trace;
    DevBuf<uint8_t> d_trace;
    int hist_groups = 1, hist_chunk_edges = 0;
    std::vector<int32_t> hist_edges, hist_run, hist_chunks;
    DevBuf<int32_t> d_hist_edges, d_hist_chunks, d_last_dump;
    DevBuf<unsigned long long> d_hist;
    struct Events {
        DevBuf<int32_t> frame_w, slot_of, counters, records, positions, checks, off_n, off_c;
        DevBuf<uint8_t> cnt_n, cnt_c;
        DevBuf<unsigned long long> node_errors, check_fails;
    } ev;
    const uint8_t *fm_cha = nullptr, *fm_msg0 = nullptr;
    uint8_t *fm_bits = nullptr;
    struct ResidentPlan { int S = 0, NT = 0, lds = 0; const JitKernel *k = nullptr; };
    std::map<int, ResidentPlan> resident_plans;
    std::string resident_log;
    std::string jit_log;
    struct GraphSlot { int seen = 0; hipGraphExec_t exec = nullptr; };
    std::map<std::array<int, 4>, GraphSlot> graphs;
    void drop_graphs() { for (auto &kv : graphs) if (kv.second.exec) (void)hipGraphExecDestroy(kv.second.exec); graphs.clear(); }
    int cn_epw() const { return opt.cn_edges_per_wave > 0 ? opt.cn_edges_per_wave : 42; }
    int npw_vn(int deg) const { return opt.nodes_per_wave > 0 ? opt.nodes_per_wave : std::max(1, opt.vn_edges_per_wave / std::max(deg, 1)); }
    int npw_cn(int deg) const { return opt.nodes_per_wave_cn > 0 ? opt.nodes_per_wave_cn : std::max(1, cn_epw() / std::max(deg, 1)); }
    int npw_cn_class(size_t ci) const { return cclass[ci].npw > 0 ? cclass[ci].npw : npw_cn(cclass[ci].deg); }
    std::string place_info = "null";
    struct SkewSlot { int n_roles = 0; size_t role_off = 0; const int32_t *items = nullptr; int nb = 0; int state_half = -1, state_ii = 0; };
    struct SkewPlan { std::vector<SkewSlot> slots; std::vector<ClassParams> h_roles; DevBuf<ClassParams> d_roles; };
    std::map<std::array<int, 3>, std::unique_ptr<SkewPlan>> skew_plans;
    std::map<std::pair<std::vector<int>, std::vector<int>>, DevBuf<int32_t>> item_tabs;
    void drop_plans() { skew_plans.clear(); item_tabs.clear(); }
    int tile() const { return kRowBytes * pack; }
    int bpad(int B) const { return (B + tile() - 1) / tile() * tile(); }
    bool profiling = false;
    struct Ev { hipEvent_t a, b; int kind; };
    std::vector<Ev> ev_live;
    std::vector<hipEvent_t> ev_pool;
    double prof_ms[LUTLDPC_K_COUNT] = {0};
    int64_t prof_n[LUTLDPC_K_COUNT] = {0};
    std::string describe;

    lutldpc_decoder() = default;
    lutldpc_decoder(const lutldpc_decoder &) = delete;
    lutldpc_decoder &operator=(const lutldpc_decoder &) = delete;
    ~lutldpc_decoder();
};

#pragma GCC visibility push(hidden)

#define LAUNCH_CHECK()                                                                              \
    do {                                                                                            \
        hipError_t e_ = hipGetLastError();                                                          \
        if (e_ != hipSuccess) return fail(LUTLDPC_ERR_HIP, std::string("kernel launch: ") + hipGetErrorString(e_)); \
        if (d->opt.validate) {                                                                      \
            e_ = hipStreamSynchronize(d->stream);                                                   \
            if (e_ == hipSuccess) e_ = hipGetLastError();                                           \
            if (e_ != hipSuccess) return fail(LUTLDPC_ERR_HIP, std::string("launch failed on the device (") + __func__ + ":" + std::to_string(__LINE__) + "): " + hipGetErrorString(e_)); \
        }                                                                                           \
    } while (0)

const void *dev_param_bytes(lutldpc_decoder *d, const void *src, size_t n);
template <class T> const T *dev_param(lutldpc_decoder *d, const T &v) { return static_cast<const T *>(dev_param_bytes(d, &v, sizeof(T))); }
#define DEV_PARAM(var, d, v)                      \
    const auto *var = dev_param((d), (v));        \
    if (!var) return LUTLDPC_ERR_HIP

#define PACK_DISPATCH(d, ...)                        \
    do {                                             \
        if ((d)->pack == 2) { constexpr int PK = 2; __VA_ARGS__; } \
        else { constexpr int PK = 1; __VA_ARGS__; }  \
    } while (0)

hipEvent_t ev_get(lutldpc_decoder *d);
void prof_fold(lutldpc_decoder *d);
struct Timed {
    lutldpc_decoder *d; int kind; hipEvent_t a{}, b{};
    Timed(lutldpc_decoder *d_, int k) : d(d_), kind(k) {
        if (d->profiling) { a = ev_get(d); b = ev_get(d); (void)hipEventRecord(a, d->stream); }
    }
    ~Timed() {
        if (d->profiling) { (void)hipEventRecord(b, d->stream); d->ev_live.push_back({a, b, kind}); }
    }
};
void make_describe(lutldpc_decoder *d);

void build_classes(const std::vector<int> &deg, std::vector<NodeClass> &cls, std::vector<int> &list);
int compile_all(lutldpc_decoder *d);
int upload_static(lutldpc_decoder *d);
struct JitRegistry { std::mutex mu; std::map<std::string, JitKernel> by_src; };
constexpr size_t kJitRegistryMax = 4096;
JitRegistry &jit_registry();
JitKernel *jit_get(int device, const std::string &src, std::string &log);
bool jit_class_source(const lutldpc_decoder *d, int kind, size_t s, size_t i, std::string &src, std::string &err);

int ensure_batch(lutldpc_decoder *d, int B);
int check_batch_buffers(const lutldpc_decoder *d, int Bpad);
int device_entry(lutldpc_decoder *d);
int batch_entry(lutldpc_decoder *d, int B, uint32_t stream = 0);
int tiles_from_device(lutldpc_decoder *d, const uint8_t *d_cha, const uint8_t *d_msg0, int B);
int labels_from_host(lutldpc_decoder *d, const uint8_t *cha, const uint8_t *msg0, int B);
int tiles_from_host(lutldpc_decoder *d, const uint8_t *cha, const uint8_t *msg0, int B);
int copy_to_host(lutldpc_decoder *d, void *host_dst, const void *src, size_t bytes);
int rows_to_host(lutldpc_decoder *d, const uint8_t *rows, uint8_t *host_dst, int B, int n_rows = 0);
int iters_to_host(lutldpc_decoder *d, int32_t *dst, int B);

hipError_t preload_stream_kernels();
int launch_state(lutldpc_decoder *d, int B, int Bpad, int mode, int value, int f0 = 0, int f1 = -1, int sel = 0);
int launch_transpose_in(lutldpc_decoder *d, const uint8_t *src, uint8_t *dst_rows, int B, int G, int limit);
int launch_transpose_out(lutldpc_decoder *d, const uint8_t *src_rows, uint8_t *dst, int B, int G, int rows = 0);
int launch_quantize_llr(lutldpc_decoder *d, size_t n, int n_qb_Cha, int n_qb_Msg, int mode);
bool chain_active(const lutldpc_decoder *d, int set);
struct HalfRange { int g0, G; };
constexpr int kPerClassLaunch = -1;
ClassParams cn_class_params(const lutldpc_decoder *d, size_t ci, HalfRange groups, int nz, int check, int skew_ii = kPerClassLaunch);
ClassParams lut_cn_class_params(const lutldpc_decoder *d, int set, size_t ci, HalfRange groups, int nz, int check);
ClassParams vn_class_params(const lutldpc_decoder *d, int kind, int set, size_t ci, HalfRange groups, int nz, int check, int write_hard, int skew_ii = kPerClassLaunch);
inline bool fast_covers(const lutldpc_decoder *d, const FastClassPlan &f, int deg) { return d->opt.use_fast && f.ok && deg <= kFastMaxDeg; }
struct KernelCases { int tree_kind; bool generated; int max_vn_deg, max_cn_deg; const char *limit; };
int validate_class(const lutldpc_decoder *d, const ClassParams &P, const std::string &where, const KernelCases &k);
inline PassBufs pass_bufs(const lutldpc_decoder *d) {
    return {d->d_msgs.p, d->d_cha_t.p, d->d_hard.p, reinterpret_cast<const uint32_t *>(d->d_state.p), reinterpret_cast<uint32_t *>(d->d_vfail.p), d->d_tables.p,
            d->d_fast_idx.p, d->d_msg0_t.p};
}
bool late_hard_active(const lutldpc_decoder *d, bool skewed, bool *chain_skip);
int launch_late_hard(lutldpc_decoder *d, bool skewed, int g0, int G, const int32_t *ctl);
int decode_tiles(lutldpc_decoder *d, int B);
int decode_device(lutldpc_decoder *d, const uint8_t *d_cha, const uint8_t *d_msg0, int B, uint8_t *d_out_bits, int32_t *d_out_iters);

hipError_t preload_compact_kernels();
bool skew_eligible(const lutldpc_decoder *d);
bool compaction_on(const lutldpc_decoder *d, int G);
int compaction_min_groups(const lutldpc_decoder *d);
int launch_uncompaction(lutldpc_decoder *d, const HalfRange (&half)[2], int Bpad);
int iterate_skewed(lutldpc_decoder *d, int B, int Bpad, int G);

ResidentSpec resident_spec(const lutldpc_decoder *d, int S, int NT);
bool resident_eligible(const lutldpc_decoder *d);
bool resident_pick(const lutldpc_decoder *d, int G, int &S_out, int &NT_out, int &lds_out);
inline bool resident_active(const lutldpc_decoder *d) { return d->resident_ok && d->opt.use_resident; }
int resident_plan_for(lutldpc_decoder *d, int G, lutldpc_decoder::ResidentPlan **out);
int launch_resident(lutldpc_decoder *d, int G, int B);

hipError_t preload_frontend_kernels();
int fill_cells(const lutldpc_channel_cells *c, const lutldpc_decoder *d, ChannelCells &C);
int sample_tiles(lutldpc_decoder *d, const ChannelCells &C, uint64_t seed, uint32_t stream, uint64_t frame0, int B, const uint8_t *sent_rows);
int encode_tiles(lutldpc_decoder *d, uint64_t seed, uint32_t stream, uint64_t frame0, int B);
int sent_rows_of(lutldpc_decoder *d, const uint8_t *codewords, bool device_codewords, uint64_t seed, uint32_t stream, uint64_t frame0, int B,
                 const uint8_t **rows);
int sim_batch_impl(lutldpc_decoder *d, const lutldpc_channel_cells *cells, uint64_t seed, uint32_t stream, uint64_t frame0, int B, const uint8_t *codewords,
                   bool device_codewords, int K_info, int32_t *frame_stats, uint8_t *cha_out, uint8_t *bits_out, lutldpc_event_request *req = nullptr);

hipError_t preload_stats_kernels();
int hist_dump(lutldpc_decoder *d);
int sent_rows_from_host(lutldpc_decoder *d, const uint8_t *codewords, int B, const uint8_t **rows);

hipError_t preload_events_kernels();
int event_request_check(const lutldpc_event_request *req);
int capture_events(lutldpc_decoder *d, int B, int K_info, const uint8_t *sent_rows, const int32_t *stats, lutldpc_event_request *req);

hipError_t preload_packed_kernels();
int launch_bits_out(lutldpc_decoder *d, uint32_t *dst, int B, int G, int first, int count);

hipError_t preload_llr_kernels();

#pragma GCC visibility pop
```

### lut_ldpc_amd/csrc/hip/decoder_stream.hip

```cpp
#include "decoder_state.hpp"
#include "kernels_generic.hpp"

#pragma GCC visibility push(hidden)

hipError_t preload_stream_kernels() {
    hipFuncAttributes a;
    return hipFuncGetAttributes(&a, reinterpret_cast<const void *>(&frame_state_kernel));
}

int launch_state(lutldpc_decoder *d, int B, int Bpad, int mode, int value, int f0, int f1, int sel) {
    Timed t(d, LUTLDPC_K_LAYOUT);
    if (f1 < 0) f1 = Bpad;
    if (f1 <= f0) return LUTLDPC_OK;
    if (mode == 0) HIP_TRY(hipMemsetAsync(d->d_vfail.p + (size_t)kVfailSlots * d->Bcap, 0, (size_t)kVfailSlots * d->Bcap, d->stream));
    launch_k(frame_state_kernel, dim3((unsigned)((f1 - f0) / 256)), dim3(256), 0, d->stream,
                       d->d_state.p, d->d_vfail.p + (size_t)sel * kVfailSlots * d->Bcap, d->d_iters.p, B, f0, f1, mode, value, d->Bcap);
    LAUNCH_CHECK();
    return LUTLDPC_OK;
}

static int launch_syndrome(lutldpc_decoder *d, int G, int sel = 0) {
    Timed t(d, LUTLDPC_K_SYNDROME);
    const int cpw = 8;
    unsigned bx = (unsigned)((d->nchk + 4 * cpw - 1) / (4 * cpw));
    PACK_DISPATCH(d, launch_k(syndrome_bits_kernel<PK>, dim3(bx, (unsigned)G), dim3(256), 0, d->stream, d->d_hard.p,
                       reinterpret_cast<const uint32_t *>(d->d_state.p), reinterpret_cast<uint32_t *>(d->d_vfail.p + (size_t)sel * kVfailSlots * d->Bcap),
                       d->d_cn_ptr.p, reinterpret_cast<const uint32_t *>(d->d_cn_vn.p), d->nchk, d->nvar, cpw, d->Bcap / 4, -1, (const int32_t *)nullptr, (int32_t *)nullptr));
    LAUNCH_CHECK();
    return LUTLDPC_OK;
}
static int launch_syndrome_of_labels(lutldpc_decoder *d, int G) {
    Timed t(d, LUTLDPC_K_SYNDROME);
    const int cpw = 8, sbit = __builtin_ctz((unsigned)(d->Nq_Cha / 2));
    HIP_TRY(hipMemsetAsync(d->d_grp.p, 0, sizeof(int32_t) * (size_t)G, d->stream));
#define SYN_ARGS(CPW, SKIP, OUT) d->d_cha_t.p, reinterpret_cast<const uint32_t *>(d->d_state.p), reinterpret_cast<uint32_t *>(d->d_vfail.p), d->d_cn_ptr.p, \
                     reinterpret_cast<const uint32_t *>(d->d_cn_vn.p), d->nchk, d->nvar, CPW, d->Bcap / 4, sbit, SKIP, OUT
    PACK_DISPATCH(d, launch_k(syndrome_bits_kernel<PK>, dim3(1u, (unsigned)G), dim3(64), 0, d->stream, SYN_ARGS(64, (const int32_t *)nullptr, d->d_grp.p)));
    unsigned bx = (unsigned)((d->nchk + 4 * cpw - 1) / (4 * cpw));
    PACK_DISPATCH(d, launch_k(syndrome_bits_kernel<PK>, dim3(bx, (unsigned)G), dim3(256), 0, d->stream, SYN_ARGS(cpw, (const int32_t *)d->d_grp.p, (int32_t *)nullptr)));
#undef SYN_ARGS
    LAUNCH_CHECK();
    return LUTLDPC_OK;
}

int launch_transpose_in(lutldpc_decoder *d, const uint8_t *src, uint8_t *dst_rows, int B, int G, int limit) {
    const int N = d->nvar;
    if (N % 4 == 0 && (reinterpret_cast<uintptr_t>(src) & 3u) == 0)
        PACK_DISPATCH(d, launch_k(transpose_in_vec_kernel<PK>, dim3((unsigned)((N + 127) / 128), (unsigned)G), dim3(256), 0, d->stream, src, dst_rows, B, N, limit));
    else
        PACK_DISPATCH(d, launch_k(transpose_in_kernel<PK>, dim3((unsigned)((N + 31) / 32), (unsigned)G), dim3(256), 0, d->stream, src, dst_rows, B, N, limit));
    LAUNCH_CHECK();
    return LUTLDPC_OK;
}
int launch_transpose_out(lutldpc_decoder *d, const uint8_t *src_rows, uint8_t *dst, int B, int G, int rows) {
    const int N = rows > 0 ? rows : d->nvar;
    if (N % 4 == 0 && (reinterpret_cast<uintptr_t>(dst) & 3u) == 0)
        PACK_DISPATCH(d, launch_k(transpose_out_vec_kernel<PK>, dim3((unsigned)((N + 127) / 128), (unsigned)G), dim3(256), 0, d->stream, src_rows, dst, B, N));
    else
        PACK_DISPATCH(d, launch_k(transpose_out_kernel<PK>, dim3((unsigned)((N + 31) / 32), (unsigned)G), dim3(256), 0, d->stream, src_rows, dst, B, N));
    LAUNCH_CHECK();
    return LUTLDPC_OK;
}

static PassParams filter_params(const PassParams &P, const std::vector<char> &keep) {
    PassParams Q = P;
    Q.n_seg = 0;
    int blk = 0;
    for (int i = 0; i < P.n_seg; i++) {
        if (!keep[(size_t)i]) continue;
        PassSeg S = P.seg[i];
        S.block_begin = blk;
        blk += (S.n_nodes + P.nodes_per_block - 1) / P.nodes_per_block;
        Q.seg[Q.n_seg++] = S;
    }
    Q.blocks_per_group = blk;
    return Q;
}

static ClassParams class_params(const lutldpc_decoder *d, int kind, const NodeClass &c, int n_nodes, int idx_off, int npw, HalfRange g, int nz, int check) {
    ClassParams P{};
    P.kind = kind; P.deg = c.deg; P.g0 = g.g0; P.G = g.G;
    P.n_nodes = n_nodes; P.nodes_per_wave = npw; P.waves_per_group = (n_nodes + npw - 1) / npw;
    P.idx_off = idx_off; P.E = d->E; P.N = d->nvar; P.nz = nz; P.check = check; P.vfail_stride_w = d->Bcap / 4;
    return P;
}
ClassParams cn_class_params(const lutldpc_decoder *d, size_t ci, HalfRange groups, int nz, int check, int skew_ii) {
    const NodeClass &c = d->cclass[ci];
    ClassParams P = class_params(d, 0, c, (int)c.nodes.size(), c.idx_off, skew_ii == kPerClassLaunch ? d->npw_cn(c.deg) : d->npw_cn_class(ci), groups, nz, check);
    if (skew_ii == kPerClassLaunch) return P;
    const int ii = skew_ii, buf_w = kVfailSlots * d->Bcap / 4;
    P.vfail_off_w = (ii & 1) * buf_w;
    if (ii == 0 && d->opt.first_from_nodes) { P.first = 1; P.nidx_off = c.nidx_off; }
    const bool on = ii != d->max_iters - 1 && chain_active(d, d->iter_set[(size_t)ii]);
    const bool hard = d->psc && ii >= 1 && chain_active(d, d->iter_set[(size_t)(ii - 1)]) && !late_hard_active(d, true, nullptr);
    if ((on || hard) && c.chain_off >= 0) {
        P.chain.idx_off = c.chain_off;
        P.chain.hard = hard ? 1 : 0;
        if (on) {
            const FastClassPlan &F2 = d->tree_class(TT_VAR, d->iter_set[(size_t)ii], d->chain_vclass)->fast;
            P.chain.on = 1;
            P.chain.tab_off = F2.tab_off[0]; P.chain.tab_len = F2.tab_len[0]; P.chain.tab_shift = F2.tab_shift[0];
            P.chain.check = d->psc ? 1 : 0;
            P.chain.vfail_off_w = ((ii + 1) & 1) * buf_w;
            P.chain.sbit_out = __builtin_ctz((unsigned)(d->Nq_Msg[(size_t)(ii + 1)] / 2) | 0x100u);
        }
    }
    return P;
}
ClassParams lut_cn_class_params(const lutldpc_decoder *d, int set, size_t ci, HalfRange groups, int nz, int check) {
    ClassParams P = cn_class_params(d, ci, groups, nz, check);
    const TabRef tab = d->chk_form(set, (int)ci, false)->tab;
    P.tab_off[0] = tab.off; P.tab_len[0] = tab.bytes;
    return P;
}
ClassParams vn_class_params(const lutldpc_decoder *d, int kind, int set, size_t ci, HalfRange groups, int nz, int check, int write_hard, int skew_ii) {
    const NodeClass &c = d->vclass[ci];
    int n_nodes = (int)c.nodes.size(), idx_off = c.idx_off;
    if (skew_ii != kPerClassLaunch && chain_active(d, set) && (int)ci == d->chain_vclass) { n_nodes = c.red_n; idx_off = c.red_off; }
    ClassParams P = class_params(d, 1, c, n_nodes, idx_off, d->npw_vn(c.deg), groups, nz, check);
    P.write_hard = write_hard;
    if (skew_ii != kPerClassLaunch) P.vfail_off_w = ((skew_ii + 1) & 1) * (kVfailSlots * d->Bcap / 4);
    const TreeClassPlan &t = *d->tree_class(kind, set, (int)ci);
    const FastClassPlan &f = t.fast;
    if (fast_covers(d, f, c.deg)) {
        P.shift_msg = f.shift_msg;
        for (int t = 0; t < f.n_tables; t++) { P.tab_off[t] = f.tab_off[t]; P.tab_len[t] = f.tab_len[t]; P.tab_shift[t] = f.tab_shift[t]; }
    } else {
        P.tab_off[0] = t.base.tab.off; P.tab_len[0] = t.base.tab.bytes;
    }
    return P;
}

int validate_class(const lutldpc_decoder *d, const ClassParams &R, const std::string &where, const KernelCases &k) {
    auto bad = [&](const std::string &what) { return fail(LUTLDPC_ERR_STATE, where + ": " + what); };
    const int groups = d->Bcap / d->tile();
    const size_t idx_n = d->fast_idx.size(), tab_n = d->d_tables.n, vfail_w = d->d_vfail.n / 4;
    auto table_ok = [&](int off, int len, int min_len, int max_len) { return off >= 0 && len >= min_len && len <= max_len && !(off & 3) && (size_t)off + (size_t)len <= tab_n; };
    if (R.G < 1 || R.g0 < 0 || R.g0 + R.G > groups) return bad("frame groups outside the batch buffers");
    if (R.E != d->E || R.N != d->nvar) return bad("E / N");
    if (R.n_nodes < 1 || R.nodes_per_wave < 1 || R.waves_per_group != (R.n_nodes + R.nodes_per_wave - 1) / R.nodes_per_wave) return bad("waves per group");
    if (R.vfail_stride_w != d->Bcap / 4 || R.vfail_off_w < 0 || (size_t)R.vfail_off_w + (size_t)kVfailSlots * (size_t)R.vfail_stride_w > vfail_w) return bad("flag buffer");
    if (R.kind != (k.tree_kind == TT_CHK ? 0 : 1)) return bad("kind");
    if (R.kind == 0) {
        if (R.deg < 2 || R.deg > k.max_cn_deg) return bad(std::string("check degree outside ") + k.limit);
        if (R.idx_off < 0 || (size_t)R.idx_off + (size_t)R.n_nodes * (size_t)R.deg > idx_n) return bad("edge table");
        if (!k.generated && (!is_pow2(R.nz) || R.nz > 64)) return bad("nz");
        if (R.first && (R.nidx_off < 0 || (size_t)R.nidx_off + (size_t)R.n_nodes * (size_t)R.deg > idx_n || R.check || R.chain.hard)) return bad("node table of the first check pass");
        if (R.chain.on || R.chain.hard) {
            if (R.chain.idx_off < 0 || (size_t)R.chain.idx_off + 2 * (size_t)R.n_nodes > idx_n) return bad("chain link table");
            if (R.chain.on && (R.chain.tab_off < 0 || R.chain.tab_len < 4 || R.chain.tab_len > 1024 || (size_t)R.chain.tab_off + (size_t)R.chain.tab_len > tab_n)) return bad("chain table");
            if (R.chain.on && R.chain.check && (R.chain.vfail_off_w < 0 || (size_t)R.chain.vfail_off_w + (size_t)kVfailSlots * (size_t)R.vfail_stride_w > vfail_w)) return bad("chain flag buffer");
        }
    } else {
        if (R.deg < 1 || R.deg > k.max_vn_deg) return bad(std::string("variable degree outside ") + k.limit);
        if (R.idx_off < 0 || (size_t)R.idx_off + 2 * (size_t)R.n_nodes > idx_n) return bad("node table");
    }
    if (k.generated) {
        if (!table_ok(R.tab_off[0], R.tab_len[0], 0, INT32_MAX)) return bad("class tables");
    } else if (R.kind) {
        const int leaves = k.tree_kind == TT_DEC ? R.deg : R.deg - 1, nt = leaves > 1 ? leaves : 1;
        for (int t = 0; t < nt; t++)
            if (!table_ok(R.tab_off[t], R.tab_len[t], 1, kFastTableStride)) return bad("table " + std::to_string(t));
    }
    return LUTLDPC_OK;
}
static int check_class_launch(const lutldpc_decoder *d, const ClassParams &P, int i, int tree_kind, bool generated) {
    if (!d->opt.validate) return LUTLDPC_OK;
    const KernelCases k = generated ? KernelCases{tree_kind, true, INT32_MAX, INT32_MAX, "the generated kernel"} : KernelCases{tree_kind, false, kFastMaxDeg, kFastMaxCnDeg, "the compile-time kernels"};
    return validate_class(d, P, "class launch check failed, class " + std::to_string(i), k);
}

template <int KIND>
static int launch_tree_pass(lutldpc_decoder *d, int set, int G, int nz, int check, int write_hard, int kind_id) {
    const TreeSetPlan *S = d->tree_set(KIND, set);
    if (!S || !S->valid) return fail(LUTLDPC_ERR_STATE, "pass plan missing for this tree set");
    const PassPlan &plan = S->pass;
    Timed t(d, kind_id);
    PassParams P = plan.P;
    P.G = G; P.nz = nz; P.check = check; P.write_hard = write_hard; P.vfail_stride_w = d->Bcap / 4;
    std::vector<char> keep((size_t)P.n_seg, 1);
    bool any = false;
    const PassBufs bufs = pass_bufs(d);
    auto class_of = [&](int i) { return KIND == TT_CHK ? lut_cn_class_params(d, set, (size_t)i, {0, G}, nz, check) : vn_class_params(d, KIND, set, (size_t)i, {0, G}, nz, check, write_hard); };
    const bool sign_bit = KIND != TT_VAR || is_pow2(nz);
    if constexpr (KIND != TT_CHK)
        for (int i = 0; i < P.n_seg && sign_bit; i++) {
            if (!fast_covers(d, S->cls[(size_t)i].fast, P.seg[i].deg)) continue;
            bool ok = false;
            const ClassParams FP = class_of(i);
            if (int rc = check_class_launch(d, FP, i, KIND, false)) return rc;
            DEV_PARAM(dFP, d, FP);
            PACK_DISPATCH(d, ok = launch_vn_fast<KIND, PK>(d->stream, FP, dFP, bufs));
            if (ok) keep[(size_t)i] = 0;
        }
    if (sign_bit)
        for (int i = 0; i < P.n_seg; i++) {
            const JitKernel *k = S->cls[(size_t)i].jit;
            if (!keep[(size_t)i] || !k) continue;
            const ClassParams F = class_of(i);
            if (int rc = check_class_launch(d, F, i, KIND, true)) return rc;
            DEV_PARAM(dF, d, F);
            void *args[] = {&dF, (void *)&bufs.msgs, (void *)&bufs.cha, (void *)&bufs.hard, (void *)&bufs.state_w, (void *)&bufs.vfail_w, (void *)&bufs.tables, (void *)&bufs.fast_idx};
            HIP_TRY(hipModuleLaunchKernel(k->fn, class_blocks(F), 1, 1, 256, 1, 1, 0, d->stream, args, nullptr));
            keep[(size_t)i] = 0;
        }
    for (char k : keep) any = any || k;
    if (any) {
        P = filter_params(P, keep);
        DEV_PARAM(dP, d, P);
        dim3 grid((unsigned)(P.blocks_per_group * G)), block(64);
        const int32_t *list = KIND == TT_CHK ? d->d_cn_list.p : d->d_vn_list.p;
        const int32_t *ptr = KIND == TT_CHK ? d->d_cn_ptr.p : d->d_vn_ptr.p;
        if (plan.lds_tab)
            PACK_DISPATCH(d, launch_k(tree_pass_kernel<KIND, true, PK>, grid, block, (size_t)plan.lds_bytes, d->stream, dP, bufs.msgs, bufs.cha, bufs.hard, bufs.state_w,
                               bufs.vfail_w, d->d_ops.p, bufs.tables, list, ptr, d->d_cn_idx.p, plan.out_slots));
        else
            PACK_DISPATCH(d, launch_k(tree_pass_kernel<KIND, false, PK>, grid, block, (size_t)plan.lds_bytes, d->stream, dP, bufs.msgs, bufs.cha, bufs.hard, bufs.state_w,
                               bufs.vfail_w, d->d_ops.p, bufs.tables, list, ptr, d->d_cn_idx.p, plan.out_slots));
    }
    LAUNCH_CHECK();
    return LUTLDPC_OK;
}

static int launch_cn_minsum(lutldpc_decoder *d, int G, int nz, int check) {
    Timed t(d, LUTLDPC_K_CN_PASS);
    PassParams P = d->cn_minsum_plan.P;
    P.G = G; P.nz = nz; P.check = check; P.vfail_stride_w = d->Bcap / 4;
    std::vector<char> keep((size_t)P.n_seg, 1);
    bool any = false;
    const PassBufs bufs = pass_bufs(d);
    if (d->opt.use_fast)
        for (int i = 0; i < P.n_seg; i++) {
            if (!cn_minsum_shape(nz, P.seg[i].deg)) continue;
            bool ok = false;
            const ClassParams FP = cn_class_params(d, (size_t)i, {0, G}, nz, check);
            if (int rc = check_class_launch(d, FP, i, TT_CHK, false)) return rc;
            DEV_PARAM(dFP, d, FP);
            PACK_DISPATCH(d, ok = launch_cn_fast<PK>(d->stream, FP, dFP, bufs));
            if (ok) keep[(size_t)i] = 0;
        }
    for (char k : keep) any = any || k;
    if (any) {
        P = filter_params(P, keep);
        DEV_PARAM(dP, d, P);
        PACK_DISPATCH(d, launch_k(cn_minsum_generic_kernel<PK>, dim3((unsigned)(P.blocks_per_group * G)), dim3(64), 0, d->stream, dP, bufs.msgs, bufs.state_w, bufs.vfail_w,
                           d->d_cn_list.p, d->d_cn_ptr.p, d->d_cn_idx.p));
    }
    LAUNCH_CHECK();
    return LUTLDPC_OK;
}

bool late_hard_active(const lutldpc_decoder *d, bool skewed, bool *chain_skip) {
    if (chain_skip) *chain_skip = false;
    if (!d->opt.late_hard || !d->psc || !d->min_lut) return false;
    for (int i = 1; i < d->max_iters; i++) if (d->Nq_Msg[(size_t)i] != d->Nq_Msg[0]) return false;
    if (!skewed) return true;
    int on = 0, off = 0;
    for (int ii = 0; ii + 1 < d->max_iters; ii++) (chain_active(d, d->iter_set[(size_t)ii]) ? on : off)++;
    if (on && off) return false;
    if (chain_skip) *chain_skip = on > 0;
    return true;
}

bool chain_active(const lutldpc_decoder *d, int set) {
    if (!d->opt.use_chain || d->chain_vclass < 0 || d->n_chain_nodes == 0) return false;
    const TreeClassPlan *t = d->tree_class(TT_VAR, set, d->chain_vclass);
    return t && t->fast.ok && t->fast.n_tables == 1 && t->fast.tab_len[0] <= 1024;
}

int launch_late_hard(lutldpc_decoder *d, bool skewed, int g0, int G, const int32_t *ctl) {
    bool chain_skip = false;
    if (!late_hard_active(d, skewed, &chain_skip) || G <= 0) return LUTLDPC_OK;
    const unsigned gx = ctl ? 1024u : 2048u;
    PACK_DISPATCH(d, launch_k(hard_from_frozen_kernel<PK>, dim3(std::min<unsigned>(gx, (unsigned)((d->nvar + 3) / 4)), (unsigned)G), dim3(256), 0, d->stream, d->d_msgs.p, d->d_hard.p,
                                        reinterpret_cast<const uint32_t *>(d->d_state.p), d->d_vn_ptr.p, chain_skip ? d->d_chain_internal.p : nullptr, d->nvar, d->E,
                                        d->Nq_Msg[0] / 2, g0, ctl));
    if (chain_skip)
        for (size_t i = 0; i < d->cclass.size(); i++) {
            if (d->cclass[i].chain_off < 0) continue;
            const int n = (int)d->cclass[i].nodes.size(), npw = d->npw_cn_class(i), runs = (n + npw - 1) / npw;
            PACK_DISPATCH(d, launch_k(chain_hard_kernel<PK>, dim3(std::min<unsigned>(512u, (unsigned)((runs + 3) / 4)), (unsigned)G), dim3(256), 0, d->stream, d->d_hard.p,
                                                reinterpret_cast<const uint32_t *>(d->d_state.p), d->d_fast_idx.p + d->cclass[i].idx_off, d->d_fast_idx.p + d->cclass[i].chain_off,
                                                d->d_edge_vn.p, n, d->cclass[i].deg, npw, d->nvar, g0, ctl));
        }
    LAUNCH_CHECK();
    return LUTLDPC_OK;
}

static int trace_dump(lutldpc_decoder *d) {
    lutldpc_decoder::Trace &T = d->trace;
    if (T.hist) return hist_dump(d);
    const size_t one = (size_t)T.B * (size_t)d->E;
    if ((size_t)(T.n + 1) * one > T.cap) return fail(LUTLDPC_ERR_ARG, "trace buffer too small");
    const int G = d->bpad(T.B) / d->tile();
    HIP_TRY(d->d_trace.alloc(one));
    if (int rc = launch_transpose_out(d, d->d_msgs.p, d->d_trace.p, T.B, G, d->E)) return rc;
    LAUNCH_CHECK();
    HIP_TRY(hipMemcpyAsync(T.host + (size_t)T.n * one, d->d_trace.p, one, hipMemcpyDeviceToHost, d->stream));
    HIP_TRY(hipStreamSynchronize(d->stream));
    T.n++;
    return LUTLDPC_OK;
}

int launch_quantize_llr(lutldpc_decoder *d, size_t n, int n_qb_Cha, int n_qb_Msg, int mode) {
    launch_k(quantize_llr_kernel, dim3((unsigned)((n + 255) / 256)), dim3(256), 0, d->stream, d->d_llr.p, n, d->d_qb_cha.p, n_qb_Cha,
                       d->d_qb_msg.p, n_qb_Msg, mode, d->d_map.p, d->d_in_cha.p, d->d_in_msg.p);
    LAUNCH_CHECK();
    return LUTLDPC_OK;
}

static int decode_tiles_launch(lutldpc_decoder *d, int B) {
    int rc;
    const int Bpad = d->bpad(B), G = Bpad / d->tile();
    const int N = d->nvar, E = d->E, I = d->max_iters;
    const int last_set = d->iter_set[(size_t)(I - 1)];
    if (!d->tree_set(TT_DEC, last_set)->valid)
        return fail(LUTLDPC_ERR_STATE, "the tree set of iteration max_iters-1 is not a decision tree set");
    if ((rc = launch_state(d, B, Bpad, 0, 0))) return rc;
    const bool tracing = d->trace.level > 1;
    if (resident_active(d) && !tracing) {
        if ((rc = launch_resident(d, G, B))) return rc;
        if (d->profiling && d->ev_live.size() > 8192) prof_fold(d);
        return LUTLDPC_OK;
    }
    if (d->pisc) {
        if (is_pow2(d->Nq_Cha / 2)) {
            if ((rc = launch_syndrome_of_labels(d, G))) return rc;
        } else {
            {
                Timed t(d, LUTLDPC_K_LAYOUT);
                const size_t n_words = (size_t)G * (size_t)N * kRowBytes / 4;
                PACK_DISPATCH(d, launch_k(hard_from_labels_kernel<PK>, dim3((unsigned)((n_words + 255) / 256)), dim3(256), 0, d->stream, d->d_cha_t.p, d->d_hard.p, n_words, d->Nq_Cha / 2));
                LAUNCH_CHECK();
            }
            if ((rc = launch_syndrome(d, G))) return rc;
        }
        if ((rc = launch_state(d, B, Bpad, 1, 0))) return rc;
        {
            Timed t(d, LUTLDPC_K_LAYOUT);
            PACK_DISPATCH(d, launch_k(hard_from_labels_masked_kernel<PK>, dim3(std::min<unsigned>(1024u, (unsigned)((N + 3) / 4)), (unsigned)G), dim3(256), 0, d->stream,
                                                d->d_cha_t.p, d->d_hard.p, reinterpret_cast<const uint32_t *>(d->d_state.p), N, d->Nq_Cha / 2, 0));
            LAUNCH_CHECK();
        }
    }
    const bool skewed = d->opt.skew && d->skew_ok && !tracing;
    if (!(skewed && d->opt.first_from_nodes)) {
        Timed t(d, LUTLDPC_K_LAYOUT);
        launch_k(init_edges_kernel, dim3((unsigned)((N + 3) / 4), (unsigned)G), dim3(256), 0, d->stream, d->d_msg0_t.p, d->d_msgs.p, d->d_vn_ptr.p, N, E);
        LAUNCH_CHECK();
    }
    if (tracing && (rc = trace_dump(d))) return rc;
    if (skewed && (rc = iterate_skewed(d, B, Bpad, G))) return rc;
    for (int ii = 0; ii < I && !skewed; ii++) {
        const int set = d->iter_set[(size_t)ii];
        const int nz_in = d->Nq_Msg[(size_t)ii] / 2;
        const int chk_check = (d->psc && ii > 0) ? 1 : 0;
        if (d->min_lut) rc = launch_cn_minsum(d, G, nz_in, chk_check);
        else rc = launch_tree_pass<TT_CHK>(d, set, G, nz_in, chk_check, 0, LUTLDPC_K_CN_PASS);
        if (rc) return rc;
        if (chk_check && (rc = launch_state(d, B, Bpad, 2, ii))) return rc;
        if (d->trace.level > 2 && (rc = trace_dump(d))) return rc;
        if (ii != I - 1) {
            const int nz_out = d->Nq_Msg[(size_t)(ii + 1)] / 2;
            rc = launch_tree_pass<TT_VAR>(d, set, G, nz_out, d->psc ? 1 : 0,
                                          (d->psc && !late_hard_active(d, false, nullptr)) ? 1 : 0, LUTLDPC_K_VN_PASS);
            if (rc) return rc;
        }
        if (tracing && (rc = trace_dump(d))) return rc;
    }
    if (d->trace.hist) {
        if (d->profiling && d->ev_live.size() > 8192) prof_fold(d);
        return LUTLDPC_OK;
    }
    {
        Timed t(d, LUTLDPC_K_LAYOUT);
        if ((rc = launch_late_hard(d, skewed, 0, G, nullptr))) return rc;
        if (skewed && d->psc && d->pisc && compaction_on(d, G) && late_hard_active(d, true, nullptr) && d->opt.compact_keep) {
            PACK_DISPATCH(d, launch_k(hard_from_labels_masked_kernel<PK>, dim3(std::min<unsigned>(1024u, (unsigned)((N + 3) / 4)), (unsigned)G), dim3(256), 0, d->stream,
                                                d->d_cha_t.p, d->d_hard.p, reinterpret_cast<const uint32_t *>(d->d_state.p), N, d->Nq_Cha / 2, 0));
            LAUNCH_CHECK();
        }
    }
    if ((rc = launch_tree_pass<TT_DEC>(d, last_set, G, 0, 0, 0, LUTLDPC_K_DECISION))) return rc;
    const int fsel = skewed ? (I & 1) : 0;
    if ((rc = launch_syndrome(d, G, fsel))) return rc;
    if ((rc = launch_state(d, B, Bpad, 3, I, 0, -1, fsel))) return rc;
    if (skewed && d->psc && compaction_on(d, G)) {
        const HalfRange half[2] = {{0, (G + 1) / 2}, {(G + 1) / 2, G - (G + 1) / 2}};
        if ((rc = launch_uncompaction(d, half, Bpad))) return rc;
    }
    if (d->profiling && d->ev_live.size() > 8192) prof_fold(d);
    return LUTLDPC_OK;
}

int decode_tiles(lutldpc_decoder *d, int B) {
    if (int rc = check_batch_buffers(d, d->bpad(B))) return rc;
    if (resident_active(d) && !d->trace.hist) {
        lutldpc_decoder::ResidentPlan *pl = nullptr;
        if (int rc = resident_plan_for(d, d->bpad(B) / d->tile(), &pl)) return rc;
    }
    if (!d->opt.use_graph || d->profiling || d->trace.level > 1 || resident_active(d)) return decode_tiles_launch(d, B);
    const std::array<int, 4> key = {B, d->psc, d->pisc, d->max_iters};
    if (d->graphs.size() > 32 && !d->graphs.count(key)) d->drop_graphs();
    auto &slot = d->graphs[key];
    if (slot.exec) {
        HIP_TRY(hipGraphLaunch(slot.exec, d->stream));
        return LUTLDPC_OK;
    }
    if (slot.seen++ == 0) return decode_tiles_launch(d, B);
    HIP_TRY(hipStreamBeginCapture(d->stream, hipStreamCaptureModeThreadLocal));
    const int rc = decode_tiles_launch(d, B);
    hipGraph_t g = nullptr;
    const hipError_t e = hipStreamEndCapture(d->stream, &g);
    if (rc || e != hipSuccess || !g) {
        if (g) (void)hipGraphDestroy(g);
        (void)hipGetLastError();
        d->opt.use_graph = 0;
        return rc ? rc : decode_tiles_launch(d, B);
    }
    const hipError_t ei = hipGraphInstantiate(&slot.exec, g, nullptr, nullptr, 0);
    (void)hipGraphDestroy(g);
    if (ei != hipSuccess) { slot.exec = nullptr; d->opt.use_graph = 0; (void)hipGetLastError(); return decode_tiles_launch(d, B); }
    HIP_TRY(hipGraphLaunch(slot.exec, d->stream));
    return LUTLDPC_OK;
}

int decode_device(lutldpc_decoder *d, const uint8_t *d_cha, const uint8_t *d_msg0, int B, uint8_t *d_out_bits, int32_t *d_out_iters) {
    const bool direct = resident_active(d) && d->opt.resident_fm && d->trace.level <= 1;
    int rc = direct ? ensure_batch(d, B) : tiles_from_device(d, d_cha, d_msg0, B);
    if (rc) return rc;
    const int G = d->bpad(B) / d->tile();
    if (direct) { d->fm_cha = d_cha; d->fm_msg0 = d_msg0; d->fm_bits = d_out_bits; }
    rc = decode_tiles(d, B);
    d->fm_cha = d->fm_msg0 = nullptr; d->fm_bits = nullptr;
    if (rc) return rc;
    {
        Timed t(d, LUTLDPC_K_LAYOUT);
        if (!direct && (rc = launch_transpose_out(d, d->d_hard.p, d_out_bits, B, G))) return rc;
        HIP_TRY(hipMemcpyAsync(d_out_iters, d->d_iters.p, sizeof(int32_t) * (size_t)B, hipMemcpyDeviceToDevice, d->stream));
    }
    return LUTLDPC_OK;
}

#pragma GCC visibility pop
```

### lut_ldpc_amd/csrc/hip/kernels_common.hpp

```cpp
#pragma once
#ifndef __HIPCC_RTC__
#include <hip/hip_runtime.h>
#include <stdint.h>
#else
typedef unsigned char uint8_t;
typedef unsigned short uint16_t;
typedef unsigned int uint32_t;
typedef unsigned long long uint64_t;
typedef short int16_t;
typedef int int32_t;
typedef long long int64_t;
#endif

namespace lutldpc {

constexpr int kRowBytes = 256;
constexpr int kTileFrames = kRowBytes;
constexpr int kWave = 64;
constexpr int kMaxSeg = 32;

constexpr uint32_t ST_ACTIVE = 0, ST_DONE_PSC = 1, ST_DONE_PISC = 2, ST_PAD = 3;
constexpr uint32_t ST_DONE_SAVED = 4;

struct PassSeg {
    int32_t block_begin;
    int32_t n_nodes;
    int32_t node_off;
    int32_t deg;
    int32_t op_off;
    int32_t n_ops;
    int32_t tab_off;
    int32_t tab_bytes;
    int32_t n_in, n_out, n_slots;
    int32_t fast;
};

struct PassParams {
    int32_t n_seg;
    int32_t blocks_per_group;
    int32_t nodes_per_block;
    int32_t G;
    int32_t E;
    int32_t N;
    int32_t nz;
    int32_t check;
    int32_t write_hard;
    int32_t slots_lds;
    int32_t vfail_stride_w;
    PassSeg seg[kMaxSeg];
};

template <int PACK>
__device__ __forceinline__ uint32_t unpack_half(uint32_t x, int h) {
    if constexpr (PACK == 1) return x;
    else return h ? ((x >> 4) & 0x0F0F0F0Fu) : (x & 0x0F0F0F0Fu);
}
template <int PACK>
__device__ __forceinline__ uint32_t pack_halves(const uint32_t (&r)[PACK]) {
    if constexpr (PACK == 1) return r[0];
    else return r[0] | (r[1] << 4);
}
template <int PACK>
__device__ __forceinline__ uint32_t pack_masks(const uint32_t (&m)[PACK]) {
    if constexpr (PACK == 1) return m[0];
    else return (m[0] & 0x0F0F0F0Fu) | (m[1] & 0xF0F0F0F0u);
}
template <int PACK>
__device__ __forceinline__ int frame_word(int g, int lane, int h) { return (g * kWave + lane) * PACK + h; }

__device__ __forceinline__ uint32_t swar_lt(uint32_t x, uint32_t t) {
    uint32_t d = (x | 0x80808080u) - t * 0x01010101u;
    return (~d >> 7) & 0x01010101u;
}
__device__ __forceinline__ uint32_t swar_zero_mask(uint32_t x) {
    uint32_t nz = ((x & 0x7F7F7F7Fu) + 0x7F7F7F7Fu) | x;
    uint32_t z = (~nz >> 7) & 0x01010101u;
    return z * 0xFFu;
}
__device__ __forceinline__ uint32_t bfi(uint32_t m, uint32_t a, uint32_t b) { return __builtin_amdgcn_bitop3_b32(m, a, b, (0xCC & 0xF0) | (0xAA & 0x0F)); }

using rsrc_t = __amdgpu_buffer_rsrc_t;
__device__ __forceinline__ rsrc_t make_rsrc(const void *p, uint32_t bytes) {
    return __builtin_amdgcn_make_buffer_rsrc(const_cast<void *>(p), 0, (int)bytes, 0x00020000);
}
#ifndef LUTLDPC_LD_AUX
#define LUTLDPC_LD_AUX 2
#endif
#ifndef LUTLDPC_ST_AUX
#define LUTLDPC_ST_AUX 2
#endif
__device__ __forceinline__ uint32_t ld_row(rsrc_t r, uint32_t row_off, uint32_t lane4) {
    return (uint32_t)__builtin_amdgcn_raw_buffer_load_b32(r, (int)lane4, (int)row_off, LUTLDPC_LD_AUX);
}
__device__ __forceinline__ void st_row(rsrc_t r, uint32_t row_off, uint32_t lane4, uint32_t v) {
    __builtin_amdgcn_raw_buffer_store_b32(v, r, (int)lane4, (int)row_off, LUTLDPC_ST_AUX);
}

__device__ __forceinline__ void pipeline_entry_fence() {
    asm volatile("" ::: "memory");
    __builtin_amdgcn_sched_barrier(0);
    __builtin_amdgcn_s_waitcnt(0x0F70);
    __builtin_amdgcn_sched_barrier(0);
    asm volatile("" ::: "memory");
}

__device__ __forceinline__ bool wave_all_zero(uint32_t x) { return __ballot(x != 0) == 0ull; }

template <int PACK>
__device__ __forceinline__ bool load_active(const uint32_t *__restrict__ state_w, int g, int lane, uint32_t (&amask)[PACK]) {
    uint32_t any = 0;
#pragma unroll
    for (int h = 0; h < PACK; h++) { amask[h] = swar_zero_mask(state_w[frame_word<PACK>(g, lane, h)]); any |= amask[h]; }
    return wave_all_zero(any);
}

template <int PACK>
__device__ __forceinline__ void store_blend(uint32_t *p, uint32_t val, uint32_t old, uint32_t smask) {
    *p = bfi(smask, val, old);
}
template <int PACK>
__device__ __forceinline__ void store_row_masked(uint32_t *p, uint32_t val, uint32_t smask) {
    if (smask == 0xFFFFFFFFu) *p = val;
    else if (smask) *p = bfi(smask, val, *p);
}

constexpr int kVfailSlots = 32;
template <int PACK>
__device__ __forceinline__ void flag_frames(uint32_t *__restrict__ vfail_w, int stride_w, int g, int lane, const uint32_t (&fail)[PACK], const uint32_t (&amask)[PACK]) {
    uint32_t *slot = vfail_w + (size_t)(blockIdx.x & (kVfailSlots - 1)) * (size_t)stride_w;
#pragma unroll
    for (int h = 0; h < PACK; h++) {
        const uint32_t f = fail[h] & amask[h] & 0x01010101u;
        if (f) atomicOr(&slot[frame_word<PACK>(g, lane, h)], f);
    }
}

constexpr int kFastMaxTables = 32;
constexpr int kFastTableStride = 256;

struct ChainParams {
    int32_t on;
    int32_t idx_off;
    int32_t tab_off, tab_len, tab_shift;
    int32_t check, hard, vfail_off_w, sbit_out;
};
struct ClassParams {
    int32_t kind;
    int32_t deg;
    int32_t g0, G;
    int32_t n_nodes, nodes_per_wave, waves_per_group;
    int32_t idx_off;
    int32_t E, N;
    int32_t nz;
    int32_t shift_msg;
    int32_t check, write_hard;
    int32_t vfail_stride_w;
    int32_t vfail_off_w;
    int32_t first, nidx_off;
    ChainParams chain;
    int32_t tab_off[kFastMaxTables];
    int32_t tab_len[kFastMaxTables];
    int32_t tab_shift[kFastMaxTables];
};

__device__ __forceinline__ uint32_t lshl_or(uint32_t x, int s, uint32_t y) {
    uint32_t r;
    asm("v_lshl_or_b32 %0, %1, %2, %3" : "=v"(r) : "v"(x), "s"(s), "v"(y));
    return r;
}

__device__ __forceinline__ uint32_t xad(uint32_t a, uint32_t b, uint32_t c) {
    uint32_t r;
    asm("v_xad_u32 %0, %1, %2, %3" : "=v"(r) : "v"(a), "s"(b), "v"(c));
    return r;
}
__device__ __forceinline__ uint32_t xor3(uint32_t a, uint32_t b, uint32_t c) { return __builtin_amdgcn_bitop3_b32(a, b, c, 0xF0 ^ 0xCC ^ 0xAA); }
__device__ __forceinline__ uint32_t xor_or(uint32_t a, uint32_t b, uint32_t c) { return __builtin_amdgcn_bitop3_b32(a, b, c, (0xF0 ^ 0xCC) | 0xAA); }

#ifndef __HIPCC_RTC__
constexpr size_t kMaxKernelArgBytes = 128;
template <typename... KArgs, typename... Args>
inline void launch_k(void (*kernel)(KArgs...), dim3 grid, dim3 block, size_t shmem, hipStream_t stream, Args &&...args) {
    static_assert((((sizeof(KArgs) + 7) / 8 * 8) + ... + 0) <= kMaxKernelArgBytes, "kernel argument segment above 128 bytes: pass the structure through device memory");
    hipLaunchKernelGGL(kernel, grid, block, shmem, stream, static_cast<KArgs>(args)...);
}
#endif

__device__ __forceinline__ int find_seg(const PassParams &P, int b) {
    int s = 0;
#pragma unroll 1
    for (int i = 1; i < P.n_seg; i++) if (b >= P.seg[i].block_begin) s = i;
    return s;
}

}
```

### lut_ldpc_amd/csrc/hip/kernels_fast.hpp

```cpp
#pragma once
#include "kernels_common.hpp"
#include "lut_program.hpp"

#include <utility>

namespace lutldpc {

constexpr int kCnAllButOneMaxDeg = 16;
template <int DEG, int UNR, int PACK, bool CHAIN, bool FIRST = false, int ABO = kCnAllButOneMaxDeg>
__device__ __forceinline__ void cn_minsum_body(
    const ClassParams &P, int block, uint8_t *msgs, const uint32_t *__restrict__ state_w, uint32_t *__restrict__ vfail_w,
    const int32_t *__restrict__ fast_idx, uint8_t *lds_tab = nullptr,
    const uint8_t *cha = nullptr, const uint8_t *__restrict__ tables = nullptr, uint8_t *hard = nullptr, const uint8_t *msg0 = nullptr)
{
    static_assert(!CHAIN || (UNR == 1 && DEG >= 2), "chain fusion: one check per step");
    const ChainParams CH = P.chain;
    if constexpr (CHAIN) {
        const int i = threadIdx.x;
        if (CH.on && i < CH.tab_len / 4) reinterpret_cast<uint32_t *>(lds_tab)[i] = reinterpret_cast<const uint32_t *>(tables + CH.tab_off)[i];
        __syncthreads();
    }
    const int lane = threadIdx.x & 63;
    const int wave = __builtin_amdgcn_readfirstlane(block * 4 + (threadIdx.x >> 6));
    const int gl = wave / P.waves_per_group;
    if (gl >= P.G) return;
    const int chunk = wave - gl * P.waves_per_group;
    const int g = gl + P.g0;
    uint32_t amask[PACK];
    if (load_active<PACK>(state_w, g, lane, amask)) return;
    const uint32_t smask = pack_masks<PACK>(amask);
    const bool all_active = __ballot(smask != 0xFFFFFFFFu) == 0ull;
    const rsrc_t base = make_rsrc(msgs + (size_t)g * (size_t)P.E * kRowBytes, (uint32_t)P.E * kRowBytes);
    const uint32_t lane4 = (uint32_t)lane * 4u;
    const int32_t *edges = fast_idx + P.idx_off;
    const int32_t *nodes = edges;
    rsrc_t nbase = base;
    if constexpr (FIRST) {
        nodes = fast_idx + P.nidx_off;
        nbase = make_rsrc(msg0 + (size_t)g * (size_t)P.N * kRowBytes, (uint32_t)P.N * kRowBytes);
    }
    const int first = chunk * P.nodes_per_wave;
    int last = first + P.nodes_per_wave;
    if (last > P.n_nodes) last = P.n_nodes;
    constexpr uint32_t ONE = PACK == 2 ? 0x11111111u : 0x01010101u;
    const int sbit = __builtin_ctz((unsigned)P.nz);
    const uint32_t SB = (uint32_t)P.nz * ONE, LOW = SB - ONE;
    const uint32_t odd = (DEG & 1) ? SB : 0u;
    uint32_t failw = 0;

    const int32_t *links = CHAIN ? fast_idx + CH.idx_off : nullptr;
    const rsrc_t cbase = CHAIN ? make_rsrc(cha + (size_t)g * (size_t)P.N * kRowBytes, (uint32_t)P.N * kRowBytes) : base;
    int lb = 0, lf = 0, lbn = 0, lfn = 0;
    uint32_t xc = 0, xcn = 0;
    uint32_t pend = 0, pend_old = 0, chainfail = 0;
    int pend_e = 0;
    auto fetch = [&](int i, uint32_t (&xx)[UNR][DEG], int (&ee)[UNR][DEG]) {
#pragma unroll
        for (int u = 0; u < UNR; u++) {
            const int ii = (i + u < last) ? i + u : last - 1;
#pragma unroll
            for (int k = 0; k < DEG; k++) ee[u][k] = edges[(size_t)ii * DEG + k];
            if constexpr (CHAIN) { lbn = links[2 * (size_t)ii]; lfn = links[2 * (size_t)ii + 1]; }
        }
#pragma unroll
        for (int u = 0; u < UNR; u++) {
            const uint32_t off = lane4 | ((i + u < last) ? 0u : 0x80000000u);
#pragma unroll
            for (int k = 0; k < DEG; k++) {
                if constexpr (FIRST) {
                    const int ii = (i + u < last) ? i + u : last - 1;
                    xx[u][k] = ld_row(nbase, (uint32_t)nodes[(size_t)ii * DEG + k] * kRowBytes, off);
                } else xx[u][k] = ld_row(base, (uint32_t)ee[u][k] * kRowBytes, off);
            }
            if constexpr (CHAIN) xcn = ld_row(cbase, (uint32_t)(lbn > 0 ? lbn - 1 : 0) * kRowBytes, (i + u < last && lbn > 0 && CH.on) ? lane4 : (lane4 | 0x80000000u));
        }
    };
    auto to_mc = [&](uint32_t xh) -> uint32_t {
        const uint32_t pos = xh & SB;
        return (xh ^ (pos - (pos >> sbit))) & LOW;
    };
    auto from_mc = [&](uint32_t mc, uint32_t po) -> uint32_t {
        return xor_or(mc, po - (po >> sbit), po);
    };
    auto eval = [&](int i, const uint32_t (&x)[UNR][DEG], const int (&e)[UNR][DEG]) {
#pragma unroll
        for (int u = 0; u < UNR; u++) {
            if (i + u >= last) break;
            uint32_t r[DEG];
            uint32_t tn;
            if constexpr (DEG <= ABO) {
            auto mx = [&](uint32_t a, uint32_t b) -> uint32_t {
                const uint32_t gt = xad(b, LOW, a) & SB;
                return bfi(gt - (gt >> sbit), a, b);
            };
            uint32_t mcs[DEG], spp = 0;
#pragma unroll
            for (int k = 0; k < DEG; k++) {
                const uint32_t xh = x[u][k];
                mcs[k] = to_mc(xh);
                if (k & 1) spp = xor3(spp, x[u][k - 1], xh);
                else if (k == DEG - 1) spp ^= xh;
            }
            tn = (spp ^ odd) & SB;
            uint32_t oc[DEG];
            if constexpr (DEG == 1) oc[0] = 0u;
            else if constexpr (DEG == 2) { oc[0] = mcs[1]; oc[1] = mcs[0]; }
            else {
                uint32_t suf[DEG];
                suf[DEG - 1] = mcs[DEG - 1];
#pragma unroll
                for (int k = DEG - 2; k >= 1; k--) suf[k] = mx(mcs[k], suf[k + 1]);
                uint32_t pre = mcs[0];
                oc[0] = suf[1];
#pragma unroll
                for (int k = 1; k <= DEG - 2; k++) { oc[k] = mx(pre, suf[k + 1]); pre = mx(pre, mcs[k]); }
                oc[DEG - 1] = pre;
            }
#pragma unroll
            for (int k = 0; k < DEG; k++) r[k] = from_mc(oc[k], (tn ^ x[u][k]) & SB);
            } else {
            uint32_t min1 = LOW, min2 = LOW, spp = 0;
            uint32_t mg[DEG];
#pragma unroll
            for (int k = 0; k < DEG; k++) {
                const uint32_t xh = x[u][k];
                const uint32_t mag = to_mc(xh) ^ LOW;
                spp ^= xh;
                mg[k] = mag;
                if (k == 0) {
                    min1 = mag;
                } else {
                    const uint32_t g1 = ((mag | SB) - min1) & SB;
                    const uint32_t k1 = g1 - (g1 >> sbit);
                    const uint32_t lo = bfi(k1, min1, mag);
                    const uint32_t hi = mag ^ min1 ^ lo;
                    if (k == 1) {
                        min2 = hi;
                    } else {
                        const uint32_t g2 = ((min2 | SB) - hi) & SB;
                        const uint32_t k2 = g2 - (g2 >> sbit);
                        min2 = bfi(k2, hi, min2);
                    }
                    min1 = lo;
                }
            }
            tn = (spp ^ odd) & SB;
            const uint32_t m1c = min1 ^ LOW, m2c = min2 ^ LOW;
#pragma unroll
            for (int k = 0; k < DEG; k++) {
                const uint32_t eq = ~(((mg[k] ^ min1) | SB) - ONE) & SB;
                const uint32_t ke = eq - (eq >> sbit);
                r[k] = from_mc(bfi(ke, m2c, m1c), (tn ^ x[u][k]) & SB);
            }
            }
            if (P.check) failw |= tn >> sbit;
            if constexpr (CHAIN) {
                [[maybe_unused]] constexpr int F = 4 * PACK, BITS = 8 / PACK;
                if (lb && CH.hard) {
                    const uint32_t neg = (~x[u][0] >> sbit) & ONE;
                    store_row_masked<PACK>(reinterpret_cast<uint32_t *>(hard + ((size_t)g * (size_t)P.N + (size_t)(lb - 1)) * kRowBytes + lane4), neg, smask);
                }
                if (lb && CH.on) {
                    uint32_t o_prev = 0, o_this = 0, dif = 0;
                    if constexpr (PACK == 2) {
                        constexpr uint32_t NIB = 0x0F0F0F0Fu;
                        const uint32_t c_lo = xc & NIB, c_hi = (xc >> 4) & NIB;
                        const uint32_t ia_lo = lshl_or(c_lo, CH.tab_shift, pend & NIB), ia_hi = lshl_or(c_hi, CH.tab_shift, (pend >> 4) & NIB);
                        const uint32_t ib_lo = lshl_or(c_lo, CH.tab_shift, r[0] & NIB), ib_hi = lshl_or(c_hi, CH.tab_shift, (r[0] >> 4) & NIB);
#pragma unroll 1
                        for (int s = 0; s < 32; s += 8) {
                            const uint32_t vp0 = lds_tab[__builtin_amdgcn_ubfe(ib_lo, (uint32_t)s, 8u)], vt0 = lds_tab[__builtin_amdgcn_ubfe(ia_lo, (uint32_t)s, 8u)];
                            const uint32_t vp1 = lds_tab[__builtin_amdgcn_ubfe(ib_hi, (uint32_t)s, 8u)], vt1 = lds_tab[__builtin_amdgcn_ubfe(ia_hi, (uint32_t)s, 8u)];
                            o_prev = lshl_or(vp0, s, o_prev);
                            o_this = lshl_or(vt0, s, o_this);
                            o_prev = lshl_or(vp1, s + 4, o_prev);
                            o_this = lshl_or(vt1, s + 4, o_this);
                        }
                    } else {
#pragma unroll 1
                    for (int s = 0; s < F * BITS; s += 2 * BITS) {
#pragma unroll
                        for (int t = 0; t < 2; t++) {
                            const int sb = s + t * BITS;
                            const uint32_t a = __builtin_amdgcn_ubfe(pend, (uint32_t)sb, (uint32_t)BITS), b = __builtin_amdgcn_ubfe(r[0], (uint32_t)sb, (uint32_t)BITS);
                            const uint32_t c = __builtin_amdgcn_ubfe(xc, (uint32_t)sb, (uint32_t)BITS);
                            const uint32_t vp = lds_tab[lshl_or(c, CH.tab_shift, b)], vt = lds_tab[lshl_or(c, CH.tab_shift, a)];
                            o_prev = lshl_or(vp, sb, o_prev);
                            o_this = lshl_or(vt, sb, o_this);
                        }
                    }
                    }
                    if (CH.check) dif = ((o_prev ^ o_this) >> CH.sbit_out) & ONE;
                    chainfail |= dif;
                    st_row(base, (uint32_t)__builtin_amdgcn_readfirstlane(pend_e) * kRowBytes, lane4, bfi(smask, o_prev, pend_old));
                    r[0] = o_this;
                }
                if (lf && CH.on) { pend = r[1]; pend_e = e[u][1]; pend_old = x[u][1]; }
#pragma unroll
                for (int k = 0; k < DEG; k++)
                    if (!(k == 1 && lf && CH.on)) st_row(base, (uint32_t)e[u][k] * kRowBytes, lane4, bfi(smask, r[k], x[u][k]));
            } else if (all_active) {
#pragma unroll
                for (int k = 0; k < DEG; k++) st_row(base, (uint32_t)e[u][k] * kRowBytes, lane4, r[k]);
            } else {
#pragma unroll
                for (int k = 0; k < DEG; k++) st_row(base, (uint32_t)e[u][k] * kRowBytes, lane4, bfi(smask, r[k], x[u][k]));
            }
        }
    };
    if constexpr (DEG <= 16) {
        uint32_t x[UNR][DEG], xn[UNR][DEG];
        int e[UNR][DEG], en[UNR][DEG];
        fetch(first, x, e);
        if constexpr (CHAIN) { lb = lbn; lf = lfn; xc = xcn; }
        fetch(first + UNR, xn, en);
        eval(first, x, e);
        pipeline_entry_fence();
        for (int i = first + UNR; i < last; i += UNR) {
#pragma unroll
            for (int u = 0; u < UNR; u++)
#pragma unroll
                for (int k = 0; k < DEG; k++) { x[u][k] = xn[u][k]; e[u][k] = en[u][k]; }
            if constexpr (CHAIN) { lb = lbn; lf = lfn; xc = xcn; }
            fetch(i + UNR, xn, en);
            eval(i, x, e);
        }
    } else {
        for (int i = first; i < last; i += UNR) {
            uint32_t x[UNR][DEG];
            int e[UNR][DEG];
            fetch(i, x, e);
            if constexpr (CHAIN) { lb = lbn; lf = lfn; xc = xcn; }
            eval(i, x, e);
        }
    }
    if (P.check) {
        uint32_t fail[PACK];
#pragma unroll
        for (int h = 0; h < PACK; h++) fail[h] = unpack_half<PACK>(failw, h);
        flag_frames<PACK>(vfail_w + P.vfail_off_w, P.vfail_stride_w, g, lane, fail, amask);
    }
    if constexpr (CHAIN) {
        if (CH.check && CH.on) {
            uint32_t fail[PACK];
#pragma unroll
            for (int h = 0; h < PACK; h++) fail[h] = unpack_half<PACK>(chainfail, h);
            flag_frames<PACK>(vfail_w + CH.vfail_off_w, P.vfail_stride_w, g, lane, fail, amask);
        }
    }
}

template <int DEG, int UNR, int PACK>
__global__ __launch_bounds__(256) void cn_minsum_fast_kernel(
    const ClassParams *__restrict__ Pp, uint8_t *__restrict__ msgs, const uint32_t *__restrict__ state_w, uint32_t *__restrict__ vfail_w,
    const int32_t *__restrict__ fast_idx)
{
    const ClassParams &P = *Pp;
    cn_minsum_body<DEG, UNR, PACK, false>(P, (int)blockIdx.x, msgs, state_w, vfail_w, fast_idx);
}

template <int N>
struct BalShape {
    static constexpr int NI = N > 1 ? N - 1 : 0;
    int left[NI > 0 ? NI : 1] = {};
    int right[NI > 0 ? NI : 1] = {};
    int size[2 * N] = {};
    int first[2 * N] = {};
    int off[NI > 0 ? NI : 1] = {};
    int top = 0;
    int total = 0;
};

template <int N>
constexpr BalShape<N> make_bal_shape() {
    BalShape<N> S{};
    int fifo[2 * N + 2] = {};
    int head = 0, tail = 0, next = N;
    for (int l = 0; l < N; l++) { fifo[tail++] = l; S.size[l] = 1; }
    while (tail - head > 1) {
        const int a = fifo[head++], b = fifo[head++];
        S.left[next - N] = a; S.right[next - N] = b;
        S.size[next] = S.size[a] + S.size[b];
        fifo[tail++] = next++;
    }
    S.top = fifo[head];
    int stack[2 * N + 2] = {};
    int sp = 0, pos = 0;
    stack[sp++] = S.top;
    while (sp > 0) {
        const int nd = stack[--sp];
        S.first[nd] = pos;
        if (nd < N) { pos += 1; continue; }
        stack[sp++] = S.right[nd - N];
        stack[sp++] = S.left[nd - N];
    }
    int total = 0;
    for (int j = 0; j < BalShape<N>::NI; j++) { S.off[j] = total; total += S.size[N + j] + 1; }
    S.total = total;
    return S;
}


__device__ __forceinline__ uint32_t lut1(const uint8_t *lds_tab, int t, uint32_t a, uint32_t b, int sh) {
    return lds_tab[t * kFastTableStride + lshl_or(b, sh, a)];
}

template <int N, int C, int KC>
__device__ __forceinline__ uint32_t bal_child(const uint32_t *in, const uint32_t *v) {
    constexpr BalShape<N> S = make_bal_shape<N>();
    if constexpr (C < N) { constexpr int idx = S.first[C] + (KC ? 0 : 1); return in[idx]; }
    else { constexpr int idx = S.off[C - N] + KC; return v[idx]; }
}

template <int N, int J, int K>
__device__ __forceinline__ void bal_node_variant(const uint32_t *in, uint32_t *v, const uint8_t *tab, int sh) {
    constexpr BalShape<N> S = make_bal_shape<N>();
    constexpr int L = S.left[J], R = S.right[J], sl = S.size[L];
    constexpr int kl = K < sl ? K : sl, kr = K > sl ? K - sl : 0;
    constexpr int dst = S.off[J] + K;
    v[dst] = lut1(tab, J, bal_child<N, L, kl>(in, v), bal_child<N, R, kr>(in, v), sh);
}

template <int N, int J, int... Ks>
__device__ __forceinline__ void bal_node_all(const uint32_t *in, uint32_t *v, const uint8_t *tab, int sh, std::integer_sequence<int, Ks...>) {
    (bal_node_variant<N, J, Ks>(in, v, tab, sh), ...);
}
template <int N, bool ALL, int... Js>
__device__ __forceinline__ void bal_all_nodes(const uint32_t *in, uint32_t *v, const uint8_t *tab, int sh, std::integer_sequence<int, Js...>) {
    if constexpr (ALL) (bal_node_all<N, Js>(in, v, tab, sh, std::make_integer_sequence<int, make_bal_shape<N>().size[N + Js] + 1>{}), ...);
    else (bal_node_variant<N, Js, make_bal_shape<N>().size[N + Js]>(in, v, tab, sh), ...);
}

template <int DV, int KIND, bool CHECK, int PACK>
__device__ __forceinline__ void vn_balanced_body(
    const ClassParams &P, int block, uint8_t *lds_tab, uint8_t *msgs, const uint8_t *cha, uint8_t *__restrict__ hard,
    const uint32_t *__restrict__ state_w, uint32_t *__restrict__ vfail_w, const uint8_t *__restrict__ tables,
    const int32_t *__restrict__ fast_idx)
{
    constexpr int N = (KIND == TT_DEC) ? DV : DV - 1;
    constexpr int NI = N > 1 ? N - 1 : 0;
    constexpr int NB = N > 1 ? N : 2;
    {
        uint32_t tmp[NI + 1];
        const int i = threadIdx.x;
#pragma unroll
        for (int t = 0; t <= NI; t++) tmp[t] = (i < P.tab_len[t] / 4) ? reinterpret_cast<const uint32_t *>(tables + P.tab_off[t])[i] : 0u;
#pragma unroll
        for (int t = 0; t <= NI; t++) if (i < P.tab_len[t] / 4) reinterpret_cast<uint32_t *>(lds_tab + t * kFastTableStride)[i] = tmp[t];
    }
    __syncthreads();

    const int lane = threadIdx.x & 63;
    const int wave = __builtin_amdgcn_readfirstlane(block * 4 + (threadIdx.x >> 6));
    const int gl = wave / P.waves_per_group;
    if (gl >= P.G) return;
    const int chunk = wave - gl * P.waves_per_group;
    const int g = gl + P.g0;
    uint32_t amask[PACK];
    if (load_active<PACK>(state_w, g, lane, amask)) return;
    const uint32_t smask = pack_masks<PACK>(amask);
    const int32_t *vtab = fast_idx + P.idx_off;
    const rsrc_t mbase = make_rsrc(msgs + (size_t)g * (size_t)P.E * kRowBytes, (uint32_t)P.E * kRowBytes);
    const rsrc_t cbase = make_rsrc(cha + (size_t)g * (size_t)P.N * kRowBytes, (uint32_t)P.N * kRowBytes);
    uint8_t *hbase = hard + (size_t)g * (size_t)P.N * kRowBytes;
    const uint32_t lane4 = (uint32_t)lane * 4u;
    const int first = chunk * P.nodes_per_wave;
    int last = first + P.nodes_per_wave;
    if (last > P.n_nodes) last = P.n_nodes;
    const int sh = P.shift_msg, shr = P.tab_shift[NI];
    const int sbit = (KIND == TT_VAR && CHECK) ? __builtin_ctz((unsigned)P.nz | 0x100u) : 0;
    uint32_t failw = 0;

    auto fetch = [&](int i, int &vv, int &ee, uint32_t (&r)[DV + 1]) {
        const int ic = i < last ? i : last - 1;
        vv = vtab[2 * (size_t)ic]; ee = vtab[2 * (size_t)ic + 1];
        const uint32_t off = lane4 | (i < last ? 0u : 0x80000000u);
#pragma unroll
        for (int k = 0; k < DV; k++) r[k] = ld_row(mbase, (uint32_t)(ee + k) * kRowBytes, off);
        r[DV] = ld_row(cbase, (uint32_t)vv * kRowBytes, off);
    };
    auto eval = [&](const uint32_t (&raw)[DV + 1], int v, int e0) {
        constexpr int F = 4 * PACK, BITS = 8 / PACK;
        constexpr int U = DV <= 8 ? 2 : 1;
        constexpr BalShape<NB> SH = make_bal_shape<NB>();
        constexpr int top_off = SH.off[SH.top - NB];
        uint32_t out[DV], hardw = 0;
#pragma unroll
        for (int o = 0; o < DV; o++) out[o] = 0;
#pragma unroll 1
        for (int sp = 0; sp < F * BITS; sp += U * BITS) {
#pragma unroll
            for (int u = 0; u < U; u++) {
                const int s = sp + u * BITS;
                uint32_t in[DV + 1];
#pragma unroll
                for (int k = 0; k <= DV; k++) in[k] = __builtin_amdgcn_ubfe(raw[k], (uint32_t)s, (uint32_t)BITS);
                const uint32_t ch = in[DV];
                uint32_t val[(N > 1 ? SH.total : 1)];
                if constexpr (N > 1) bal_all_nodes<N, KIND == TT_VAR>(in, val, lds_tab, sh, std::make_integer_sequence<int, NI>{});
                if constexpr (KIND == TT_DEC) {
                    uint32_t top;
                    if constexpr (N > 1) top = val[top_off + N];
                    else top = in[0];
                    hardw = lshl_or(lut1(lds_tab, NI, top, ch, shr) < 1u ? 1u : 0u, s, hardw);
                } else {
#pragma unroll
                    for (int o = 0; o < DV; o++) {
                        uint32_t r;
                        if constexpr (N == 0) {
                            r = lut1(lds_tab, 0, ch, 0u, 0);
                        } else {
                            uint32_t top;
                            if constexpr (N > 1) top = val[top_off + o];
                            else top = in[o == 0 ? 1 : 0];
                            r = lut1(lds_tab, NI, top, ch, shr);
                        }
                        out[o] = lshl_or(r, s, out[o]);
                    }
                }
            }
        }
        if constexpr (KIND == TT_VAR && CHECK) {
            constexpr uint32_t ONE = PACK == 2 ? 0x11111111u : 0x01010101u;
            uint32_t diff = 0;
#pragma unroll
            for (int o = 1; o < DV; o++) diff |= out[o] ^ out[0];
            failw |= (diff >> sbit) & ONE;
            if (P.write_hard) hardw = (~out[0] >> sbit) & ONE;
        }
        if constexpr (KIND == TT_DEC) {
            store_row_masked<PACK>(reinterpret_cast<uint32_t *>(hbase + (size_t)v * kRowBytes + lane4), hardw, smask);
        } else {
#pragma unroll
            for (int o = 0; o < DV; o++) st_row(mbase, (uint32_t)(e0 + o) * kRowBytes, lane4, bfi(smask, out[o], raw[o]));
            if (CHECK && P.write_hard)
                store_row_masked<PACK>(reinterpret_cast<uint32_t *>(hbase + (size_t)v * kRowBytes + lane4), hardw, smask);
        }
    };
    int v, e0, vn, en;
    uint32_t raw[DV + 1], nxt[DV + 1];
    fetch(first, v, e0, raw);
    fetch(first + 1, vn, en, nxt);
    eval(raw, v, e0);
    pipeline_entry_fence();
    for (int i = first + 1; i < last; i++) {
#pragma unroll
        for (int k = 0; k <= DV; k++) raw[k] = nxt[k];
        v = vn; e0 = en;
        fetch(i + 1, vn, en, nxt);
        eval(raw, v, e0);
    }
    if (KIND == TT_VAR && CHECK) {
        uint32_t fail[PACK];
#pragma unroll
        for (int h = 0; h < PACK; h++) fail[h] = unpack_half<PACK>(failw, h);
        flag_frames<PACK>(vfail_w + P.vfail_off_w, P.vfail_stride_w, g, lane, fail, amask);
    }
}

template <int DV, int KIND, bool CHECK, int PACK>
__global__ __launch_bounds__(256) void vn_balanced_fast_kernel(
    const ClassParams *__restrict__ Pp, uint8_t *msgs, const uint8_t *cha, uint8_t *__restrict__ hard,
    const uint32_t *__restrict__ state_w, uint32_t *__restrict__ vfail_w, const uint8_t *__restrict__ tables,
    const int32_t *__restrict__ fast_idx)
{
    constexpr int NT = (KIND == TT_DEC ? DV : DV - 1) > 1 ? (KIND == TT_DEC ? DV : DV - 1) : 1;
    __shared__ __attribute__((aligned(16))) uint8_t lds_tab[NT * kFastTableStride];
    const ClassParams &P = *Pp;
    vn_balanced_body<DV, KIND, CHECK, PACK>(P, (int)blockIdx.x, lds_tab, msgs, cha, hard, state_w, vfail_w, tables, fast_idx);
}

#ifndef LUTLDPC_B0_WAVES_MIN
#define LUTLDPC_B0_WAVES_MIN 7
#endif
#ifndef LUTLDPC_B0_WAVES_MAX
#define LUTLDPC_B0_WAVES_MAX 8
#endif
constexpr int kFusedMaxRoles = 10;
constexpr int kFusedBuckets = 4;
constexpr int kFusedVnDeg[kFusedBuckets] = {8, 12, 20, 8};
constexpr int kFusedCnDeg[kFusedBuckets] = {8, 16, 32, 10};
constexpr int kFusedAboDeg[kFusedBuckets] = {8, 10, 16, 8};
constexpr int kFusedBucketOrder[kFusedBuckets] = {0, 3, 1, 2};
inline int fused_bucket(int max_vn_deg, int max_cn_deg) {
    for (int b : kFusedBucketOrder) if (max_vn_deg <= kFusedVnDeg[b] && max_cn_deg <= kFusedCnDeg[b]) return b;
    return -1;
}
inline int fused_bucket_rank(int bucket) { for (int i = 0; i < kFusedBuckets; i++) if (kFusedBucketOrder[i] == bucket) return i; return -1; }
inline constexpr int fused_max_cn_deg() { int m = 0; for (int b = 0; b < kFusedBuckets; b++) m = kFusedCnDeg[b] > m ? kFusedCnDeg[b] : m; return m; }

template <int PACK, bool CHAIN, bool FIRST, int ABO, int... Ds>
__device__ __forceinline__ void fused_cn_switch(const ClassParams &P, int block, std::integer_sequence<int, Ds...>, uint8_t *msgs, const uint32_t *state_w,
                                                uint32_t *vfail_w, const int32_t *fast_idx, uint8_t *lds_tab, const uint8_t *cha, const uint8_t *tables, uint8_t *hard,
                                                const uint8_t *msg0) {
    ((P.deg == Ds + 2 ? (cn_minsum_body<Ds + 2, 1, PACK, CHAIN, FIRST, ABO>(P, block, msgs, state_w, vfail_w, fast_idx, lds_tab, cha, tables, hard, msg0), 0) : 0), ...);
}
template <int PACK, bool CHECK, int... Ds>
__device__ __forceinline__ void fused_vn_switch(const ClassParams &P, int block, std::integer_sequence<int, Ds...>, uint8_t *lds_tab, uint8_t *msgs,
                                                const uint8_t *cha, uint8_t *hard, const uint32_t *state_w, uint32_t *vfail_w, const uint8_t *tables,
                                                const int32_t *fast_idx) {
    ((P.deg == Ds + 1 ? (vn_balanced_body<Ds + 1, TT_VAR, CHECK, PACK>(P, block, lds_tab, msgs, cha, hard, state_w, vfail_w, tables, fast_idx), 0) : 0), ...);
}

template <int PACK, bool CHECK, int BUCKET>
__global__ __launch_bounds__(256) __attribute__((amdgpu_waves_per_eu((BUCKET == 0 || BUCKET == 3) ? LUTLDPC_B0_WAVES_MIN : BUCKET == 1 ? 4 : 3, (BUCKET == 0 || BUCKET == 3) ? LUTLDPC_B0_WAVES_MAX : 8))) void pass_fused_kernel(
    const ClassParams *__restrict__ roles, const int2 *__restrict__ items, int prio, uint8_t *msgs, const uint8_t *cha, uint8_t *__restrict__ hard,
    const uint32_t *__restrict__ state_w, uint32_t *__restrict__ vfail_w, const uint8_t *__restrict__ tables, const int32_t *__restrict__ fast_idx,
    const uint8_t *__restrict__ msg0)
{
    constexpr int MAXVN = kFusedVnDeg[BUCKET], MAXCN = kFusedCnDeg[BUCKET];
    __shared__ __attribute__((aligned(16))) uint8_t lds_tab[MAXVN * kFastTableStride];
    const int2 it = items[blockIdx.x];
    const int r = __builtin_amdgcn_readfirstlane(it.x), rb = __builtin_amdgcn_readfirstlane(it.y);
    const ClassParams &P = roles[r];
    if (prio && P.kind) {
        if (P.deg >= 4) __builtin_amdgcn_s_setprio(3); else __builtin_amdgcn_s_setprio(1);
    }
    if (P.kind == 0) {
        constexpr auto degs = std::make_integer_sequence<int, MAXCN - 1>{};
        if (!P.first) {
            if (P.chain.on || P.chain.hard) fused_cn_switch<PACK, true, false, kFusedAboDeg[BUCKET]>(P, rb, degs, msgs, state_w, vfail_w, fast_idx, lds_tab, cha, tables, hard, msg0);
            else fused_cn_switch<PACK, false, false, kFusedAboDeg[BUCKET]>(P, rb, degs, msgs, state_w, vfail_w, fast_idx, lds_tab, cha, tables, hard, msg0);
        } else {
            if (P.chain.on) fused_cn_switch<PACK, true, true, kFusedAboDeg[BUCKET]>(P, rb, degs, msgs, state_w, vfail_w, fast_idx, lds_tab, cha, tables, hard, msg0);
            else fused_cn_switch<PACK, false, true, kFusedAboDeg[BUCKET]>(P, rb, degs, msgs, state_w, vfail_w, fast_idx, lds_tab, cha, tables, hard, msg0);
        }
    }
    else fused_vn_switch<PACK, CHECK>(P, rb, std::make_integer_sequence<int, MAXVN>{}, lds_tab, msgs, cha, hard, state_w, vfail_w, tables, fast_idx);
}

inline bool match_balanced(const Tree &t, int kind, int d, std::vector<const TreeNode *> &canon) {
    canon.clear();
    const int n = (kind == TT_DEC) ? d : d - 1;
    const TreeNode *root = t.root.get();
    if (!root || root->type != NT_ROOT) return false;
    if (n == 0) {
        if (root->child.size() != 1 || root->child[0]->type != NT_CHA) return false;
        canon.push_back(root);
        return true;
    }
    if (root->child.size() != 2 || root->child[1]->type != NT_CHA || !root->child[1]->child.empty()) return false;
    std::vector<int> left, right, fifo;
    for (int l = 0; l < n; l++) fifo.push_back(l);
    size_t head = 0;
    int next = n;
    while (fifo.size() - head > 1) {
        left.push_back(fifo[head]); right.push_back(fifo[head + 1]);
        head += 2;
        fifo.push_back(next++);
    }
    const int top = fifo[head];
    std::vector<const TreeNode *> node_of((size_t)(2 * n), nullptr);
    struct Item { int id; const TreeNode *tn; };
    std::vector<Item> stack{{top, root->child[0].get()}};
    while (!stack.empty()) {
        Item it = stack.back(); stack.pop_back();
        if (it.id < n) {
            if (it.tn->type != NT_MSG || !it.tn->child.empty()) return false;
            continue;
        }
        if (it.tn->type != NT_IM || it.tn->child.size() != 2) return false;
        node_of[(size_t)it.id] = it.tn;
        stack.push_back({right[(size_t)(it.id - n)], it.tn->child[1].get()});
        stack.push_back({left[(size_t)(it.id - n)], it.tn->child[0].get()});
    }
    for (int j = n; j < 2 * n - 1; j++) { if (!node_of[(size_t)j]) return false; canon.push_back(node_of[(size_t)j]); }
    canon.push_back(root);
    return true;
}

inline bool is_pow2(int x) { return x > 0 && (x & (x - 1)) == 0; }

struct FastClassPlan {
    bool ok = false;
    int n_tables = 0, shift_msg = 0;
    int32_t tab_off[kFastMaxTables] = {}, tab_len[kFastMaxTables] = {}, tab_shift[kFastMaxTables] = {};
};

inline FastClassPlan plan_fast_vn(const Tree &t, int kind, int d, const std::map<const TreeNode *, std::pair<uint32_t, uint32_t>> &tab_of) {
    FastClassPlan fp;
    std::vector<const TreeNode *> canon;
    if (d < 1 || d > 20 || !match_balanced(t, kind, d, canon) || (int)canon.size() > kFastMaxTables) return fp;
    int shift_msg = -1;
    for (size_t j = 0; j < canon.size(); j++) {
        const TreeNode *nd = canon[j];
        auto it = tab_of.find(nd);
        if (it == tab_of.end() || it->second.second > 256u) return fp;
        for (auto &c : nd->child) if (!is_pow2(c->K) || c->K > 128) return fp;
        if (!is_pow2(nd->K) || nd->K > 128) return fp;
        const int sh0 = __builtin_ctz((unsigned)nd->child[0]->K);
        if (j + 1 < canon.size()) {
            if (nd->child[0]->K != nd->child[1]->K) return fp;
            if (shift_msg < 0) shift_msg = sh0; else if (shift_msg != sh0) return fp;
        }
        fp.tab_off[j] = (int32_t)it->second.first;
        fp.tab_len[j] = (int32_t)it->second.second;
        fp.tab_shift[j] = sh0;
    }
    fp.shift_msg = shift_msg < 0 ? 0 : shift_msg;
    fp.n_tables = (int)canon.size();
    fp.ok = true;
    return fp;
}

constexpr int kFastMaxDeg = 20;
constexpr int kFastMaxCnDeg = 32;

inline bool cn_minsum_shape(int nz, int deg) { return is_pow2(nz) && nz <= 64 && deg >= 2 && deg <= kFastMaxCnDeg; }

struct PassBufs {
    uint8_t *msgs; const uint8_t *cha; uint8_t *hard;
    const uint32_t *state_w; uint32_t *vfail_w;
    const uint8_t *tables; const int32_t *fast_idx; const uint8_t *msg0;
};
inline unsigned class_blocks(const ClassParams &P) { return (unsigned)((P.waves_per_group * P.G + 3) / 4); }

template <int KIND, bool CHECK, int PACK, int... DVs>
bool dispatch_vn_fast(std::integer_sequence<int, DVs...>, hipStream_t s, const ClassParams &P, const ClassParams *dP, const PassBufs &B) {
    bool done = false;
    ((P.deg == DVs + 1 ? (launch_k(vn_balanced_fast_kernel<DVs + 1, KIND, CHECK, PACK>, dim3(class_blocks(P)), dim3(256), 0, s, dP, B.msgs, B.cha, B.hard, B.state_w,
                                   B.vfail_w, B.tables, B.fast_idx), done = true) : false), ...);
    return done;
}
template <int KIND, int PACK>
bool launch_vn_fast(hipStream_t s, const ClassParams &P, const ClassParams *dP, const PassBufs &B) {
    constexpr auto seq = std::make_integer_sequence<int, kFastMaxDeg>{};
    if (KIND == TT_VAR && P.check) return dispatch_vn_fast<KIND, true, PACK>(seq, s, P, dP, B);
    return dispatch_vn_fast<KIND, false, PACK>(seq, s, P, dP, B);
}

constexpr int cn_unroll(int deg) { return deg <= 4 ? 4 : deg <= 10 ? 2 : 1; }
template <int PACK, int... Ds>
bool dispatch_cn_fast(std::integer_sequence<int, Ds...>, hipStream_t s, const ClassParams &P, const ClassParams *dP, const PassBufs &B) {
    bool done = false;
    ((P.deg == Ds + 1 ? (launch_k(cn_minsum_fast_kernel<Ds + 1, cn_unroll(Ds + 1), PACK>, dim3(class_blocks(P)), dim3(256), 0, s, dP, B.msgs, B.state_w, B.vfail_w, B.fast_idx), done = true) : false), ...);
    return done;
}
template <int PACK>
bool launch_cn_fast(hipStream_t s, const ClassParams &P, const ClassParams *dP, const PassBufs &B) {
    return dispatch_cn_fast<PACK>(std::make_integer_sequence<int, kFastMaxCnDeg>{}, s, P, dP, B);
}

template <int KIND, int PACK>
hipError_t preload_vn_fast() {
    hipFuncAttributes a;
    return hipFuncGetAttributes(&a, reinterpret_cast<const void *>(&vn_balanced_fast_kernel<2, KIND, false, PACK>));
}
template <int PACK>
hipError_t preload_cn_fast() {
    hipFuncAttributes a;
    return hipFuncGetAttributes(&a, reinterpret_cast<const void *>(&cn_minsum_fast_kernel<2, 4, PACK>));
}

template <int PACK, bool CHECK, int BUCKET>
void launch_fused_one(hipStream_t s, const ClassParams *d_roles, const int32_t *items, int n_blocks, int prio, const PassBufs &B) {
    launch_k(pass_fused_kernel<PACK, CHECK, BUCKET>, dim3((unsigned)n_blocks), dim3(256), 0, s, d_roles, reinterpret_cast<const int2 *>(items), prio, B.msgs, B.cha, B.hard,
             B.state_w, B.vfail_w, B.tables, B.fast_idx, B.msg0);
}
template <int PACK, int BUCKET>
void launch_fused(hipStream_t s, const ClassParams *d_roles, const int32_t *items, int n_blocks, int prio, bool vn_check, const PassBufs &B) {
    if (vn_check) launch_fused_one<PACK, true, BUCKET>(s, d_roles, items, n_blocks, prio, B);
    else launch_fused_one<PACK, false, BUCKET>(s, d_roles, items, n_blocks, prio, B);
}
template <int PACK, int BUCKET>
hipError_t preload_fused() {
    hipFuncAttributes a;
    return hipFuncGetAttributes(&a, reinterpret_cast<const void *>(&pass_fused_kernel<PACK, false, BUCKET>));
}

#define LUTLDPC_CLASS_SIG (hipStream_t, const ClassParams &, const ClassParams *, const PassBufs &)
#define LUTLDPC_FUSED_SIG (hipStream_t, const ClassParams *, const int32_t *, int, int, bool, const PassBufs &)
#define LUTLDPC_FAST_LAUNCHERS(X)                                                                                                           \
    X template bool launch_vn_fast<TT_VAR, 1> LUTLDPC_CLASS_SIG; X template bool launch_vn_fast<TT_VAR, 2> LUTLDPC_CLASS_SIG; \
    X template bool launch_vn_fast<TT_DEC, 1> LUTLDPC_CLASS_SIG; X template bool launch_vn_fast<TT_DEC, 2> LUTLDPC_CLASS_SIG; \
    X template bool launch_cn_fast<1> LUTLDPC_CLASS_SIG; X template bool launch_cn_fast<2> LUTLDPC_CLASS_SIG; \
    X template void launch_fused<1, 0> LUTLDPC_FUSED_SIG; X template void launch_fused<2, 0> LUTLDPC_FUSED_SIG; \
    X template void launch_fused<1, 1> LUTLDPC_FUSED_SIG; X template void launch_fused<2, 1> LUTLDPC_FUSED_SIG; \
    X template void launch_fused<1, 2> LUTLDPC_FUSED_SIG; X template void launch_fused<2, 2> LUTLDPC_FUSED_SIG; \
    X template void launch_fused<1, 3> LUTLDPC_FUSED_SIG; X template void launch_fused<2, 3> LUTLDPC_FUSED_SIG; \
    X template hipError_t preload_fused<2, 0>(); X template hipError_t preload_fused<2, 1>(); X template hipError_t preload_fused<2, 2>(); X template hipError_t preload_fused<2, 3>(); \
    X template hipError_t preload_vn_fast<TT_VAR, 1>(); X template hipError_t preload_vn_fast<TT_VAR, 2>(); X template hipError_t preload_vn_fast<TT_DEC, 2>(); \
    X template hipError_t preload_cn_fast<2>();

}
```

### lut_ldpc_amd/decoder.py

```python
from __future__ import annotations

import ctypes as C
import json

import numpy as np

from . import _capi
from ._capi import lib, check


def _i32(a):
    return np.ascontiguousarray(a, np.int32)


def _p(a, t):
    return a.ctypes.data_as(C.POINTER(t))


MODES = {"all": 0, "active": 1}


class Decoder:
    def __init__(self, nvar, nchk, dv, dc, cn_msg_idx, nq_cha, nq_msg, reuse_vec, max_iters, min_lut,
                 var_trees_txt, chk_trees_txt="", device=0):
        self.nvar, self.nchk = int(nvar), int(nchk)
        self.max_iters = int(max_iters)
        dv, dc, cn = _i32(dv), _i32(dc), _i32(cn_msg_idx)
        nq, ru = _i32(nq_msg), np.ascontiguousarray(reuse_vec, np.uint8)
        assert len(nq) == max_iters and len(ru) == max_iters
        self._h = C.c_void_p()
        self._owned = True
        check(lib.lutldpc_decoder_create(self.nvar, self.nchk, _p(dv, C.c_int32), _p(dc, C.c_int32), _p(cn, C.c_int32),
                                         int(nq_cha), _p(nq, C.c_int32), _p(ru, C.c_uint8), self.max_iters, int(bool(min_lut)),
                                         var_trees_txt.encode(), (chk_trees_txt or "").encode(), int(device),
                                         C.byref(self._h)))
        self.device = device

    def close(self):
        if getattr(self, "_h", None) and getattr(self, "_owned", False):
            lib.lutldpc_decoder_destroy(self._h)
        self._h = None

    def __del__(self):
        self.close()

    def set_exit_conditions(self, max_iters, psc=True, pisc=False):
        check(lib.lutldpc_decoder_set_exit_conditions(self._h, int(max_iters), int(psc), int(pisc)))
        self.max_iters = int(max_iters)

    def lut_decode_batch(self, cha: np.ndarray, msg0: np.ndarray):
        cha = np.ascontiguousarray(cha, np.uint8)
        msg0 = np.ascontiguousarray(msg0, np.uint8)
        B, N = cha.shape
        if N != self.nvar or msg0.shape != cha.shape:
            raise ValueError("cha/msg0 must be [B, nvar]")
        out = np.empty((B, N), np.uint8)
        iters = np.empty(B, np.int32)
        check(lib.lutldpc_decoder_decode_batch(self._h, _p(cha, C.c_uint8), _p(msg0, C.c_uint8), B, _p(out, C.c_uint8),
                                               _p(iters, C.c_int32)))
        return out, iters

    def decode_packed(self, cha, msg0=None, cha2msg_map=None, nibbles=False, first=0, count=None):
        cha = np.ascontiguousarray(cha, np.uint8)
        stride = (self.nvar + 1) // 2 if nibbles else self.nvar
        if cha.ndim != 2 or cha.shape[1] != stride:
            raise ValueError("cha must be [B, ceil(nvar/2)] packed bytes" if nibbles else "cha must be [B, nvar]")
        B = cha.shape[0]
        if msg0 is not None:
            msg0 = np.ascontiguousarray(msg0, np.uint8)
            if msg0.shape != cha.shape:
                raise ValueError("msg0 must have the shape and format of cha")
        mp = _i32(cha2msg_map) if cha2msg_map is not None else None
        count = self.nvar - int(first) if count is None else int(count)
        io = _capi.PackedIO(_capi.IN_NIBBLES if nibbles else _capi.IN_BYTES, _p(mp, C.c_int32) if mp is not None else None, int(first), count)
        words = np.empty((B, max((count + 31) // 32, 0)), np.uint32)
        iters = np.empty(B, np.int32)
        check(lib.lutldpc_decoder_decode_batch_packed(self._h, C.byref(io), _p(cha, C.c_uint8), _p(msg0, C.c_uint8) if msg0 is not None else None, B,
                                                      _p(words, C.c_uint32), _p(iters, C.c_int32)))
        return words, iters

    def lut_decode_batch_trace(self, cha, msg0, level, n_edges):
        cha = np.ascontiguousarray(cha, np.uint8); msg0 = np.ascontiguousarray(msg0, np.uint8)
        B, N = cha.shape
        n_dumps = 1 + self.max_iters * (int(level) - 1)
        out = np.empty((B, N), np.uint8); iters = np.empty(B, np.int32)
        trace = np.empty((n_dumps, B, int(n_edges)), np.uint8)
        got = C.c_int32()
        check(lib.lutldpc_decoder_decode_batch_trace(self._h, _p(cha, C.c_uint8), _p(msg0, C.c_uint8), B, int(level), _p(out, C.c_uint8), _p(iters, C.c_int32),
                                                     _p(trace, C.c_uint8), trace.size, C.byref(got)))
        assert got.value == n_dumps
        return out, iters, trace

    def set_edge_groups(self, edge_group=None, n_groups=1):
        if edge_group is None:
            check(lib.lutldpc_decoder_set_edge_groups(self._h, None, int(n_groups)))
        else:
            eg = _i32(edge_group)
            if eg.shape != (self.histogram_shape(2)[3],):
                raise ValueError("edge_group must hold one entry per edge")
            check(lib.lutldpc_decoder_set_edge_groups(self._h, _p(eg, C.c_int32), int(n_groups)))

    def histogram_shape(self, level=3):
        out = (C.c_int32 * 4)()
        check(lib.lutldpc_decoder_histogram_shape(self._h, int(level), out))
        return tuple(out)

    def new_histogram(self, level=3, n_labels=None) -> np.ndarray:
        n_dumps, n_groups, nq, _ = self.histogram_shape(level)
        return np.zeros((n_dumps, n_groups, 2, int(n_labels or nq)), np.int64)

    def message_histogram(self, cha, msg0, sent=None, level=3, mode="all", n_labels=None, hist=None, decode=True):
        cha = np.ascontiguousarray(cha, np.uint8); msg0 = np.ascontiguousarray(msg0, np.uint8)
        B, N = cha.shape
        if N != self.nvar or msg0.shape != cha.shape:
            raise ValueError("cha/msg0 must be [B, nvar]")
        if sent is not None:
            sent = np.ascontiguousarray(sent, np.uint8)
            if sent.shape != cha.shape:
                raise ValueError("sent must be [B, nvar]")
        hist = self.new_histogram(level, n_labels) if hist is None else hist
        if hist.dtype != np.int64 or not hist.flags.c_contiguous or hist.ndim != 4:
            raise ValueError("hist must be a C-contiguous int64 array [dump, group, 2, label]")
        bits = np.empty((B, N), np.uint8) if decode else None
        iters = np.empty(B, np.int32) if decode else None
        got = C.c_int32()
        check(lib.lutldpc_decoder_histogram_batch(self._h, _p(cha, C.c_uint8), _p(msg0, C.c_uint8), _p(sent, C.c_uint8) if sent is not None else None, B,
                                                  int(level), MODES[mode] if isinstance(mode, str) else int(mode), hist.shape[3],
                                                  _p(bits, C.c_uint8) if decode else None, _p(iters, C.c_int32) if decode else None,
                                                  _p(hist, C.c_int64), hist.size, C.byref(got)))
        assert got.value == hist.shape[0]
        return (hist, bits, iters) if decode else hist

    def error_events(self, cha, msg0, sent=None, select="codeword", max_frames=1024, max_pos=64, max_chk=64, profiles=None, k_info=None, decode=False):
        from .err_events import _Request
        cha = np.ascontiguousarray(cha, np.uint8); msg0 = np.ascontiguousarray(msg0, np.uint8)
        B, N = cha.shape
        if N != self.nvar or msg0.shape != cha.shape:
            raise ValueError("cha/msg0 must be [B, nvar]")
        if sent is not None:
            sent = np.ascontiguousarray(sent, np.uint8)
            if sent.shape != cha.shape:
                raise ValueError("sent must be [B, nvar]")
        rq = _Request(self.nvar, self.nchk, select, max_frames, max_pos, max_chk, profiles)
        bits = np.empty((B, N), np.uint8) if decode else None
        iters = np.empty(B, np.int32) if decode else None
        check(lib.lutldpc_decoder_events_batch(self._h, _p(cha, C.c_uint8), _p(msg0, C.c_uint8), _p(sent, C.c_uint8) if sent is not None else None, B,
                                               int(self.nvar - self.nchk if k_info is None else k_info), _p(bits, C.c_uint8) if decode else None,
                                               _p(iters, C.c_int32) if decode else None, C.byref(rq.c)))
        return (rq.result(), bits, iters) if decode else rq.result()

    def decode_llr_batch(self, llr, qb_cha, qb_msg, mode=0, cha2msg_map=None):
        llr = np.ascontiguousarray(llr, np.float64)
        B, N = llr.shape
        qc = np.ascontiguousarray(qb_cha, np.float64)
        qm = np.ascontiguousarray(qb_msg if qb_msg is not None else [], np.float64)
        mp = _i32(cha2msg_map) if cha2msg_map is not None else None
        out = np.empty((B, N), np.uint8)
        iters = np.empty(B, np.int32)
        check(lib.lutldpc_decoder_decode_llr_batch(self._h, _p(llr, C.c_double), B, _p(qc, C.c_double), len(qc),
                                                   _p(qm, C.c_double), len(qm), int(mode),
                                                   _p(mp, C.c_int32) if mp is not None else None,
                                                   _p(out, C.c_uint8), _p(iters, C.c_int32)))
        return out, iters

    def decode_llr(self, llr, qb_cha, qb_msg=None, cha2msg_map=None, scale=None, first=0, count=None, want_labels=False, decode=True):
        qc = np.ascontiguousarray(qb_cha, np.float64)
        qm = np.ascontiguousarray(qb_msg, np.float64) if qb_msg is not None else None
        mp = _i32(cha2msg_map) if cha2msg_map is not None else None
        if (qm is None) == (mp is None):
            raise ValueError("give either qb_msg (mode CONT) or cha2msg_map (mode QCHA)")
        if mp is not None and len(mp) != len(qc) + 1:
            raise ValueError("cha2msg_map must hold one entry per channel label")
        on_device = not isinstance(llr, np.ndarray) and hasattr(llr, "data_ptr")
        if on_device:
            import torch
            names = {torch.float64: _capi.LLR_F64, torch.float32: _capi.LLR_F32, torch.float16: _capi.LLR_F16, torch.int8: _capi.LLR_I8}
            if not llr.is_cuda:
                raise ValueError("a torch tensor must live on the device; pass host values as a numpy array")
        else:
            if not isinstance(llr, np.ndarray):
                raise ValueError("llr must be a numpy array or a torch tensor on the device")
            names = {np.dtype(np.float64): _capi.LLR_F64, np.dtype(np.float32): _capi.LLR_F32, np.dtype(np.float16): _capi.LLR_F16,
                     np.dtype(np.int8): _capi.LLR_I8}
        if llr.dtype not in names:
            raise ValueError("llr must be float64, float32, float16 or int8")
        dtype = names[llr.dtype]
        if llr.ndim != 2 or llr.shape[1] != self.nvar or llr.shape[0] < 1:
            raise ValueError("llr must be [B, nvar]")
        if dtype == _capi.LLR_I8 and scale is None:
            raise ValueError("int8 values need a scale: LLR = scale * q")
        if not decode and not want_labels:
            want_labels = True
        B, N = int(llr.shape[0]), self.nvar
        count = N - int(first) if count is None else int(count)
        W = max((count + 31) // 32, 0)
        if on_device:
            if llr.stride(1) != 1 or (B > 1 and llr.stride(0) < N):
                raise ValueError("a tensor needs a contiguous last dimension and a row stride of at least nvar")
            stride = int(llr.stride(0)) if B > 1 else N
            dev = llr.device
            torch.cuda.current_stream(dev).synchronize()
            words = torch.empty((B, W), dtype=torch.int32, device=dev) if decode else None
            iters = torch.empty(B, dtype=torch.int32, device=dev) if decode else None
            cha = torch.empty((B, N), dtype=torch.uint8, device=dev) if want_labels else None
            msg = torch.empty((B, N), dtype=torch.uint8, device=dev) if want_labels else None
            ptr = lambda t: C.c_void_p(t.data_ptr()) if t is not None else None
        else:
            llr = np.ascontiguousarray(llr)
            stride = N
            words = np.empty((B, W), np.uint32) if decode else None
            iters = np.empty(B, np.int32) if decode else None
            cha = np.empty((B, N), np.uint8) if want_labels else None
            msg = np.empty((B, N), np.uint8) if want_labels else None
            ptr = lambda a: C.c_void_p(a.ctypes.data) if a is not None else None
        io = _capi.LlrIO(dtype, int(on_device), stride, float(scale) if scale is not None else 0.0, _p(qc, C.c_double), len(qc),
                         _p(qm, C.c_double) if qm is not None else None, len(qm) if qm is not None else 0, 0 if qm is not None else 1,
                         _p(mp, C.c_int32) if mp is not None else None, int(first), count, 1)
        check(lib.lutldpc_decoder_decode_llr_packed(self._h, C.byref(io), ptr(llr), B, ptr(words), ptr(iters), ptr(cha), ptr(msg)))
        out = (words, iters) if decode else ()
        return out + (cha, msg) if want_labels else out

    def lut_decode_batch_device(self, d_cha: int, d_msg0: int, B: int, d_out_bits: int, d_out_iters: int, sync=False):
        check(lib.lutldpc_decoder_decode_batch_device(self._h, C.c_void_p(d_cha), C.c_void_p(d_msg0), int(B),
                                                      C.c_void_p(d_out_bits), C.c_void_p(d_out_iters), int(sync)))

    @property
    def stream(self) -> int:
        return lib.lutldpc_decoder_stream(self._h) or 0

    def set_profiling(self, on: bool):
        check(lib.lutldpc_decoder_set_profiling(self._h, int(on)))

    def reset_profile(self):
        check(lib.lutldpc_decoder_reset_profile(self._h))

    def profile(self) -> dict:
        out = {}
        for k, name in enumerate(_capi.KIND_NAMES):
            ms, n = C.c_double(), C.c_int64()
            check(lib.lutldpc_decoder_get_profile(self._h, k, C.byref(ms), C.byref(n)))
            out[name] = {"ms": ms.value, "launches": n.value}
        return out

    def device_bytes(self) -> int:
        return lib.lutldpc_decoder_device_bytes(self._h)

    def describe(self) -> dict:
        return json.loads(lib.lutldpc_decoder_describe(self._h).decode())

    def jit_source(self, kind: int, tree_set: int, cls: int, compile: bool = False) -> str:
        n = lib.lutldpc_selftest_jit_source(self._h, kind, tree_set, cls, None, 0, int(compile))
        if n < 0:
            check(int(n))
        buf = C.create_string_buffer(n)
        lib.lutldpc_selftest_jit_source(self._h, kind, tree_set, cls, buf, n, 0)
        return buf.value.decode()

    def resident_source(self, G: int, compile: bool = False):
        info = (C.c_int32 * 3)()
        n = lib.lutldpc_selftest_resident_source(self._h, int(G), None, 0, int(compile), info)
        if n < 0:
            check(int(n))
        buf = C.create_string_buffer(n)
        lib.lutldpc_selftest_resident_source(self._h, int(G), buf, n, 0, info)
        return buf.value.decode(), tuple(info)

    def program_eval(self, kind: int, tree_set: int, cls: int, inputs, n_out: int):
        a = _i32(inputs)
        out = np.zeros(n_out, np.int32)
        check(lib.lutldpc_selftest_program_eval(self._h, kind, tree_set, cls, _p(a, C.c_int32), len(a), _p(out, C.c_int32), n_out))
        return out

    def program_stats(self, kind: int, tree_set: int, cls: int):
        a, b, c = C.c_int32(), C.c_int32(), C.c_int32()
        check(lib.lutldpc_selftest_program_stats(self._h, kind, tree_set, cls, C.byref(a), C.byref(b), C.byref(c)))
        return {"ops": a.value, "ops_naive": b.value, "slots": c.value}
```

Before: 258,400.

## Fuse update of non-chain degree-2 variable nodes into check pass via crossed edge table

Extends the chain optimization so that in fixed-work min-LUT decodes, every other degree-2 variable node (not just in-wave chain neighbours) is updated inside the check-node pass, using a crossed edge index table and a per-check cross link. The variable pass then skips those crossed nodes via a reduced node list, which removes a round trip through the edge messages for many degree-2 nodes. Alternating iterations use the crossed index table so that both edges of a crossed node stay consistent. The cost is an extra row load and LUT lookup per check, extra index memory, and more complex scheduling, and it applies only with skew, no parity-check exit and min_lut.

```diff
diff --git a/include/lut_ldpc_hip.h b/include/lut_ldpc_hip.h
--- a/include/lut_ldpc_hip.h
+++ b/include/lut_ldpc_hip.h
@@ -162,6 +162,8 @@
 
 int64_t lutldpc_selftest_jit_source(lutldpc_decoder *d, int kind, int set, int cls, char *buf, int64_t cap, int compile);
 int64_t lutldpc_selftest_resident_source(lutldpc_decoder *d, int G, char *buf, int64_t cap, int compile, int32_t *info);
+int64_t lutldpc_selftest_cross_tables(lutldpc_decoder *d, int cls, int which, int32_t *buf, int64_t cap);
+int lutldpc_selftest_cross_plan(lutldpc_decoder *d, int32_t *plan, int cap);
 
 #ifdef __cplusplus
 }
diff --git a/lut_ldpc_amd/_capi.py b/lut_ldpc_amd/_capi.py
--- a/lut_ldpc_amd/_capi.py
+++ b/lut_ldpc_amd/_capi.py
@@ -85,6 +85,8 @@
     "lutldpc_decoder_decode_batch_trace": (C.c_int, [_vp, _u8p, _u8p, C.c_int, C.c_int, _u8p, _ip, _u8p, C.c_int64, _ip]),
     "lutldpc_selftest_jit_source": (C.c_int64, [_vp, C.c_int, C.c_int, C.c_int, C.c_char_p, C.c_int64, C.c_int]),
     "lutldpc_selftest_resident_source": (C.c_int64, [_vp, C.c_int, C.c_char_p, C.c_int64, C.c_int, C.POINTER(C.c_int32)]),
+    "lutldpc_selftest_cross_tables": (C.c_int64, [_vp, C.c_int, C.c_int, _ip, C.c_int64]),
+    "lutldpc_selftest_cross_plan": (C.c_int, [_vp, _ip, C.c_int]),
     "lutldpc_check_stream": (C.c_int, [C.c_uint32]),
     "lutldpc_decoder_set_generator": (C.c_int, [_vp, C.c_int, C.c_int, C.POINTER(C.c_uint64)]),
     "lutldpc_decoder_encode_random": (C.c_int, [_vp, C.c_uint64, C.c_uint32, C.c_uint64, C.c_int, _u8p]),
diff --git a/lut_ldpc_amd/csrc/hip/decoder.hip b/lut_ldpc_amd/csrc/hip/decoder.hip
--- a/lut_ldpc_amd/csrc/hip/decoder.hip
+++ b/lut_ldpc_amd/csrc/hip/decoder.hip
@@ -61,21 +61,21 @@
             for (size_t j = 0; j < d->cclass[i].nodes.size(); j++) chained += d->fast_idx[(size_t)d->cclass[i].chain_off + 2 * j + 1] != 0;
         const TreeClassPlan *t = d->tree_class(TT_CHK, 0, (int)i);
         o << (i ? "," : "") << "{\"deg\":" << d->cclass[i].deg << ",\"nodes\":" << d->cclass[i].nodes.size() << ",\"nodes_per_wave\":" << d->npw_cn_class(i)
-          << ",\"chain_nodes\":" << chained << ",\"kernel\":\""
+          << ",\"chain_nodes\":" << chained << ",\"cross_nodes\":" << (cross_active(d) ? d->cclass[i].n_cross : 0) << ",\"kernel\":\""
           << (d->min_lut ? minsum
                          : t && t->jit ? "lutldpc_jit_pass" : "tree_pass_kernel<CHK>") << "\"}";
     }
-    o << "],\"resident\":" << (resident_active(d) ? 1 : 0) << ",\"skewed_pipeline\":" << ((d->opt.skew && d->skew_ok) ? 1 : 0) << ",\"fused_bucket\":" << d->fused_bucket_id << ",\"compaction\":" << (d->opt.use_compact < 0 ? 2 : d->opt.use_compact) << ",\"compaction_min_groups\":" << compaction_min_groups(d) << ",\"chain_nodes\":" << (d->opt.use_chain ? d->n_chain_nodes : 0) << ",\"placement\":" << d->place_info;
+    o << "],\"resident\":" << (resident_active(d) ? 1 : 0) << ",\"skewed_pipeline\":" << ((d->opt.skew && d->skew_ok) ? 1 : 0) << ",\"fused_bucket\":" << d->fused_bucket_id << ",\"compaction\":" << (d->opt.use_compact < 0 ? 2 : d->opt.use_compact) << ",\"compaction_min_groups\":" << compaction_min_groups(d) << ",\"chain_nodes\":" << (d->opt.use_chain ? d->n_chain_nodes : 0) << ",\"cross_nodes\":" << (cross_active(d) ? d->n_cross_nodes : 0) << ",\"cross_max\":" << kCrossMax << ",\"placement\":" << d->place_info;
     if (d->gen_set) o << ",\"generator\":{\"K\":" << d->gen_K << ",\"R\":" << d->gen_R << "}";
-    {
+    if (d->describe_static.empty()) {
         uint32_t ops = 0;
         for (const Op &op : d->all_ops) ops = crc32(crc32(ops, &op, offsetof(Op, child) + sizeof(op.child)), &op.mult, sizeof(Op) - offsetof(Op, mult));
         char b[160];
         snprintf(b, sizeof(b), ",\"static\":{\"ops\":%zu,\"ops_crc\":\"%08x\",\"tables_bytes\":%zu,\"tables_crc\":\"%08x\",\"index_words\":%zu,\"index_crc\":\"%08x\"}", d->all_ops.size(), ops,
                  d->all_tables.size(), crc32(0, d->all_tables.data(), d->all_tables.size()), d->fast_idx.size(), crc32(0, d->fast_idx.data(), 4 * d->fast_idx.size()));
-        o << b;
-    }
-    o << "}";
+        d->describe_static = b;
+    }
+    o << d->describe_static << "}";
     d->describe = o.str();
 }
 
@@ -93,6 +93,7 @@
     KNOB_F("LUTLDPC_COMPOSE", use_compose, "1: exact table composition for the resident kernel's trees (measured slower: LDS bank conflicts, see compile_all)"),
     KNOB_I("LUTLDPC_COMPOSE_SPACE", compose_space, 0, 65536, "largest composed table, entries"),
     KNOB_F("LUTLDPC_CHAIN", use_chain, "1: degree-2 nodes between neighbouring checks of a wave are updated inside the check pass (build_fast_index)"),
+    KNOB_F("LUTLDPC_CROSS", use_cross, "1: fixed-work decodes update every other degree-2 node inside the check pass too, through a crossed edge table (build_fast_index); 0: only the in-wave chain nodes"),
     KNOB_F("LUTLDPC_LATE_HARD", late_hard, "1: decided bits of early-terminated frames recovered once, at the end, from their frozen messages; 0: stored by every variable pass"),
     KNOB_F("LUTLDPC_FIRST_FROM_NODES", first_from_nodes, "1: the first check pass reads the initial-message rows; 0: init_edges_kernel copies them to the edge rows first"),
     KNOB_I("LUTLDPC_NODES_PER_BLOCK", nodes_per_block, 1, 4096, "interpreter kernels: nodes per 64-thread block"),
@@ -265,7 +266,9 @@
     if (max_iters < 1 || max_iters > d->max_iters_created) return fail(LUTLDPC_ERR_ARG, "max_iters outside [1, value at creation]");
     if (!d->tree_set(TT_DEC, d->iter_set[(size_t)(max_iters - 1)])->valid)
         return fail(LUTLDPC_ERR_ARG, "the tree set of iteration max_iters-1 is not a decision tree set");
+    const bool same = d->max_iters == max_iters && d->psc == (psc ? 1 : 0);
     d->max_iters = max_iters; d->psc = psc ? 1 : 0; d->pisc = pisc ? 1 : 0;
+    if (!same && d->n_cross_nodes > 0) make_describe(d);
     return LUTLDPC_OK;
 }
 
@@ -403,4 +406,21 @@
     return give_source(src, buf, cap, compile);
 }
 
-}
+int64_t lutldpc_selftest_cross_tables(lutldpc_decoder *d, int cls, int which, int32_t *buf, int64_t cap) {
+    if (!d || cls < 0 || (size_t)cls >= d->cclass.size() || which < 0 || which > 2) return fail(LUTLDPC_ERR_ARG, "NULL decoder / bad class / bad table");
+    const NodeClass &c = d->cclass[(size_t)cls];
+    const int off = which == 0 ? c.idx_off : which == 1 ? c.xidx_off : c.cross_off;
+    const size_t n = off < 0 ? 0 : which == 2 ? (size_t)kCrossMax * c.nodes.size() : c.nodes.size() * (size_t)c.deg;
+    if (buf && n > 0 && cap >= (int64_t)n) std::copy(d->fast_idx.begin() + off, d->fast_idx.begin() + off + (ptrdiff_t)n, buf);
+    return (int64_t)n;
+}
+int lutldpc_selftest_cross_plan(lutldpc_decoder *d, int32_t *plan, int cap) {
+    if (!d || !plan || cap < 2 * d->max_iters) return fail(LUTLDPC_ERR_ARG, "NULL decoder / plan too short");
+    for (int ii = 0; ii < d->max_iters; ii++) {
+        const CrossPass x = cross_active(d) ? cross_pass(d, ii) : CrossPass{0, 0};
+        plan[2 * ii] = x.crossed; plan[2 * ii + 1] = x.fused;
+    }
+    return d->max_iters;
+}
+
+}
diff --git a/lut_ldpc_amd/csrc/hip/decoder_setup.hip b/lut_ldpc_amd/csrc/hip/decoder_setup.hip
--- a/lut_ldpc_amd/csrc/hip/decoder_setup.hip
+++ b/lut_ldpc_amd/csrc/hip/decoder_setup.hip
@@ -52,7 +52,7 @@
     d->fast_idx.clear();
     for (auto &c : d->cclass) { c.chain_off = -1; c.npw = 0; }
     for (auto &c : d->vclass) {
-        c.red_off = -1; c.red_n = 0;
+        c.red_off = -1; c.red_n = 0; c.xred_off = -1; c.xred_n = 0;
         c.idx_off = (int)d->fast_idx.size();
         for (int v : c.nodes) { d->fast_idx.push_back(v); d->fast_idx.push_back(d->vn_ptr[(size_t)v]); }
     }
@@ -89,6 +89,17 @@
             if (deg < 2 || deg > fused_max_cn_deg() || pos_of[(size_t)c2] != pos_of[(size_t)c1] + 1 || pos_of[(size_t)c1] / npw != pos_of[(size_t)c2] / npw) continue;
             if (fwd[(size_t)c1] || back[(size_t)c2]) continue;
             fwd[(size_t)c1] = v + 1; back[(size_t)c2] = v + 1; internal[(size_t)v] = 1;
+        }
+    std::vector<int> xnode((size_t)d->nchk, 0);
+    std::vector<char> crossed((size_t)d->nvar, 0);
+    if (d->opt.use_cross && d->min_lut)
+        for (int v = 0; v < d->nvar; v++) {
+            if (d->dv[(size_t)v] != 2 || internal[(size_t)v]) continue;
+            const int e0 = d->vn_ptr[(size_t)v], c1 = edge_chk[(size_t)e0], c2 = edge_chk[(size_t)e0 + 1];
+            if (c1 < 0 || c2 < 0 || c1 == c2 || xnode[(size_t)c1] || xnode[(size_t)c2]) continue;
+            const int d1 = d->cclass[(size_t)cls_of[(size_t)c1]].deg, d2 = d->cclass[(size_t)cls_of[(size_t)c2]].deg;
+            if (std::min(d1, d2) <= kCrossSlot || std::max(d1, d2) > fused_max_cn_deg()) continue;
+            xnode[(size_t)c1] = xnode[(size_t)c2] = v + 1; crossed[(size_t)v] = 1;
         }
     for (size_t ci = 0; ci < d->cclass.size(); ci++) {
         auto &c = d->cclass[ci];
@@ -107,12 +118,30 @@
                 const int vb = back[(size_t)cn] - 1;
                 if (es[0] != d->vn_ptr[(size_t)vb] && es[0] != d->vn_ptr[(size_t)vb] + 1) to_slot(back[(size_t)cn], 0);
             }
+            to_slot(xnode[(size_t)cn], kCrossSlot);
             for (int e : es) d->fast_idx.push_back(e);
             any = any || back[(size_t)cn] || fwd[(size_t)cn];
         }
         if (any) {
             c.chain_off = (int)d->fast_idx.size();
             for (int cn : c.nodes) { d->fast_idx.push_back(back[(size_t)cn]); d->fast_idx.push_back(fwd[(size_t)cn]); }
+        }
+    }
+    d->n_cross_nodes = 0;
+    for (char x : crossed) d->n_cross_nodes += x;
+    for (auto &c : d->cclass) {
+        c.cross_off = -1; c.xidx_off = c.idx_off; c.n_cross = 0;
+        std::set<int> mine;
+        for (int cn : c.nodes) if (xnode[(size_t)cn]) mine.insert(xnode[(size_t)cn]);
+        if (mine.empty()) continue;
+        c.n_cross = (int)mine.size();
+        c.cross_off = (int)d->fast_idx.size();
+        for (int cn : c.nodes) d->fast_idx.push_back(xnode[(size_t)cn]);
+        const size_t off = (size_t)c.idx_off, cnt = c.nodes.size() * (size_t)c.deg;
+        c.xidx_off = (int)d->fast_idx.size();
+        for (size_t j = 0; j < cnt; j++) {
+            const int e = d->fast_idx[off + j], v = d->edge_vn[(size_t)e];
+            d->fast_idx.push_back(crossed[(size_t)v] ? 2 * d->vn_ptr[(size_t)v] + 1 - e : e);
         }
     }
     for (auto &c : d->cclass) {
@@ -138,6 +167,9 @@
         c.red_off = (int)d->fast_idx.size();
         for (int v : c.nodes)
             if (!internal[(size_t)v]) { d->fast_idx.push_back(v); d->fast_idx.push_back(d->vn_ptr[(size_t)v]); c.red_n++; }
+        c.xred_off = (int)d->fast_idx.size(); c.xred_n = 0;
+        for (int v : c.nodes)
+            if (!internal[(size_t)v] && !crossed[(size_t)v]) { d->fast_idx.push_back(v); d->fast_idx.push_back(d->vn_ptr[(size_t)v]); c.xred_n++; }
         d->chain_vclass = (int)vi;
     }
     d->n_chain_nodes = 0;
@@ -166,7 +198,20 @@
         check("check class edge", c.idx_off, cnt, 0, 1, d->E); check("check class node", c.nidx_off, cnt, 0, 1, d->nvar);
         check("transposed check class edge", c.tidx_off, cnt, 0, 1, d->E); check("transposed check class node", c.tnidx_off, cnt, 0, 1, d->nvar);
         if (c.chain_off >= 0) check("chain link", c.chain_off, 2 * c.nodes.size(), 0, 1, d->nvar + 1);
-    }
+        check("crossed check class edge", c.xidx_off, cnt, 0, 1, d->E);
+        if (c.cross_off >= 0) check("cross node", c.cross_off, (size_t)kCrossMax * c.nodes.size(), 0, 1, d->nvar + 1);
+    }
+    for (const auto &c : d->vclass)
+        if (c.xred_off >= 0) { check("variable class without cross nodes", c.xred_off, 2 * (size_t)c.xred_n, 0, 2, d->nvar); check("variable class without cross nodes", c.xred_off, 2 * (size_t)c.xred_n, 1, 2, d->E - c.deg + 1); }
+    std::vector<int> seen((size_t)d->nvar + 1, 0);
+    int n_cross = 0;
+    for (const auto &c : d->cclass)
+        for (size_t j = 0; !rc && c.cross_off >= 0 && j < (size_t)kCrossMax * c.nodes.size(); j++) seen[(size_t)d->fast_idx[(size_t)c.cross_off + j]]++;
+    for (int v = 1; v <= d->nvar && !rc; v++) {
+        if (seen[(size_t)v] != 0 && seen[(size_t)v] != 2) rc = fail(LUTLDPC_ERR_STATE, "index table check failed: cross node not at exactly two checks");
+        n_cross += seen[(size_t)v] == 2;
+    }
+    if (!rc && n_cross != d->n_cross_nodes) rc = fail(LUTLDPC_ERR_STATE, "index table check failed: cross node count");
     return rc;
 }
 
diff --git a/lut_ldpc_amd/csrc/hip/decoder_state.hpp b/lut_ldpc_amd/csrc/hip/decoder_state.hpp
--- a/lut_ldpc_amd/csrc/hip/decoder_state.hpp
+++ b/lut_ldpc_amd/csrc/hip/decoder_state.hpp
@@ -14,6 +14,7 @@
 #include <map>
 #include <memory>
 #include <mutex>
+#include <set>
 #include <sstream>
 #include <string>
 #include <vector>
@@ -79,6 +80,8 @@
     int idx_off = 0, tidx_off = 0;
     int nidx_off = 0, tnidx_off = 0, chain_off = -1, npw = 0;
     int red_off = -1, red_n = 0;
+    int cross_off = -1, xidx_off = 0, n_cross = 0;
+    int xred_off = -1, xred_n = 0;
 };
 
 struct PassPlan {
@@ -117,6 +120,7 @@
         int use_compose = 0, compose_space = 4096;
         int chk_full_labels = 1;
         int use_chain = 1;
+        int use_cross = 1;
         int use_resident = 1, resident_force_S = 0, resident_force_NT = 0, resident_U = 0, resident_xcd = 1, resident_fm = 1;
         int resident_flag_reduce = -1, resident_cn_persistent = -1, resident_waves_eu = 0;
         int place_candidates = 16;
@@ -160,6 +164,7 @@
     std::vector<int32_t> fast_idx;
     int chain_vclass = -1, n_chain_nodes = 0;
     std::vector<uint8_t> chain_internal;
+    int n_cross_nodes = 0;
     std::vector<int32_t> edge_vn;
     int pack = 1;
     bool skew_ok = false;
@@ -224,6 +229,7 @@
     int npw_vn(int deg) const { return opt.nodes_per_wave > 0 ? opt.nodes_per_wave : std::max(1, opt.vn_edges_per_wave / std::max(deg, 1)); }
     int npw_cn(int deg) const { return opt.nodes_per_wave_cn > 0 ? opt.nodes_per_wave_cn : std::max(1, cn_epw() / std::max(deg, 1)); }
     int npw_cn_class(size_t ci) const { return cclass[ci].npw > 0 ? cclass[ci].npw : npw_cn(cclass[ci].deg); }
+    std::string describe_static;
     std::string place_info = "null";
     struct SkewSlot { int n_roles = 0; size_t role_off = 0; const int32_t *items = nullptr; int nb = 0; int state_half = -1, state_ii = 0; };
     struct SkewPlan { std::vector<SkewSlot> slots; std::vector<ClassParams> h_roles; DevBuf<ClassParams> d_roles; };
@@ -310,6 +316,9 @@
 int launch_transpose_out(lutldpc_decoder *d, const uint8_t *src_rows, uint8_t *dst, int B, int G, int rows = 0);
 int launch_quantize_llr(lutldpc_decoder *d, size_t n, int n_qb_Cha, int n_qb_Msg, int mode);
 bool chain_active(const lutldpc_decoder *d, int set);
+bool cross_active(const lutldpc_decoder *d);
+struct CrossPass { int crossed, fused; };
+CrossPass cross_pass(const lutldpc_decoder *d, int ii);
 struct HalfRange { int g0, G; };
 constexpr int kPerClassLaunch = -1;
 ClassParams cn_class_params(const lutldpc_decoder *d, size_t ci, HalfRange groups, int nz, int check, int skew_ii = kPerClassLaunch);
diff --git a/lut_ldpc_amd/csrc/hip/decoder_stream.hip b/lut_ldpc_amd/csrc/hip/decoder_stream.hip
--- a/lut_ldpc_amd/csrc/hip/decoder_stream.hip
+++ b/lut_ldpc_amd/csrc/hip/decoder_stream.hip
@@ -93,17 +93,25 @@
     if (ii == 0 && d->opt.first_from_nodes) { P.first = 1; P.nidx_off = c.nidx_off; }
     const bool on = ii != d->max_iters - 1 && chain_active(d, d->iter_set[(size_t)ii]);
     const bool hard = d->psc && ii >= 1 && chain_active(d, d->iter_set[(size_t)(ii - 1)]) && !late_hard_active(d, true, nullptr);
+    auto root_table = [&] {
+        const FastClassPlan &F2 = d->tree_class(TT_VAR, d->iter_set[(size_t)ii], d->chain_vclass)->fast;
+        P.chain.tab_off = F2.tab_off[0]; P.chain.tab_len = F2.tab_len[0]; P.chain.tab_shift = F2.tab_shift[0];
+    };
     if ((on || hard) && c.chain_off >= 0) {
         P.chain.idx_off = c.chain_off;
         P.chain.hard = hard ? 1 : 0;
         if (on) {
-            const FastClassPlan &F2 = d->tree_class(TT_VAR, d->iter_set[(size_t)ii], d->chain_vclass)->fast;
             P.chain.on = 1;
-            P.chain.tab_off = F2.tab_off[0]; P.chain.tab_len = F2.tab_len[0]; P.chain.tab_shift = F2.tab_shift[0];
+            root_table();
             P.chain.check = d->psc ? 1 : 0;
             P.chain.vfail_off_w = ((ii + 1) & 1) * buf_w;
             P.chain.sbit_out = __builtin_ctz((unsigned)(d->Nq_Msg[(size_t)(ii + 1)] / 2) | 0x100u);
         }
+    }
+    if (cross_active(d)) {
+        const CrossPass x = cross_pass(d, ii);
+        if (x.crossed) P.idx_off = c.xidx_off;
+        if (x.fused && c.cross_off >= 0) { P.chain.cross = kCrossMax; P.chain.cross_off = c.cross_off; root_table(); }
     }
     return P;
 }
@@ -116,7 +124,10 @@
 ClassParams vn_class_params(const lutldpc_decoder *d, int kind, int set, size_t ci, HalfRange groups, int nz, int check, int write_hard, int skew_ii) {
     const NodeClass &c = d->vclass[ci];
     int n_nodes = (int)c.nodes.size(), idx_off = c.idx_off;
-    if (skew_ii != kPerClassLaunch && chain_active(d, set) && (int)ci == d->chain_vclass) { n_nodes = c.red_n; idx_off = c.red_off; }
+    if (skew_ii != kPerClassLaunch && (int)ci == d->chain_vclass) {
+        if (cross_active(d) && cross_pass(d, skew_ii).fused) { n_nodes = c.xred_n; idx_off = c.xred_off; }
+        else if (chain_active(d, set)) { n_nodes = c.red_n; idx_off = c.red_off; }
+    }
     ClassParams P = class_params(d, 1, c, n_nodes, idx_off, d->npw_vn(c.deg), groups, nz, check);
     P.write_hard = write_hard;
     if (skew_ii != kPerClassLaunch) P.vfail_off_w = ((skew_ii + 1) & 1) * (kVfailSlots * d->Bcap / 4);
@@ -146,9 +157,13 @@
         if (R.idx_off < 0 || (size_t)R.idx_off + (size_t)R.n_nodes * (size_t)R.deg > idx_n) return bad("edge table");
         if (!k.generated && (!is_pow2(R.nz) || R.nz > 64)) return bad("nz");
         if (R.first && (R.nidx_off < 0 || (size_t)R.nidx_off + (size_t)R.n_nodes * (size_t)R.deg > idx_n || R.check || R.chain.hard)) return bad("node table of the first check pass");
-        if (R.chain.on || R.chain.hard) {
-            if (R.chain.idx_off < 0 || (size_t)R.chain.idx_off + 2 * (size_t)R.n_nodes > idx_n) return bad("chain link table");
-            if (R.chain.on && (R.chain.tab_off < 0 || R.chain.tab_len < 4 || R.chain.tab_len > 1024 || (size_t)R.chain.tab_off + (size_t)R.chain.tab_len > tab_n)) return bad("chain table");
+        if (R.chain.cross) {
+            if (R.chain.cross < 0 || R.chain.cross > kCrossMax || R.deg <= kCrossSlot || R.check || R.chain.check || R.chain.hard) return bad("cross slots");
+            if (R.chain.cross_off < 0 || (size_t)R.chain.cross_off + (size_t)kCrossMax * (size_t)R.n_nodes > idx_n) return bad("cross node table");
+        }
+        if (R.chain.on || R.chain.hard || R.chain.cross) {
+            if ((R.chain.on || R.chain.hard) && (R.chain.idx_off < 0 || (size_t)R.chain.idx_off + 2 * (size_t)R.n_nodes > idx_n)) return bad("chain link table");
+            if ((R.chain.on || R.chain.cross) && (R.chain.tab_off < 0 || R.chain.tab_len < 4 || R.chain.tab_len > 1024 || (size_t)R.chain.tab_off + (size_t)R.chain.tab_len > tab_n)) return bad("chain table");
             if (R.chain.on && R.chain.check && (R.chain.vfail_off_w < 0 || (size_t)R.chain.vfail_off_w + (size_t)kVfailSlots * (size_t)R.vfail_stride_w > vfail_w)) return bad("chain flag buffer");
         }
     } else {
@@ -268,6 +283,21 @@
     return t && t->fast.ok && t->fast.n_tables == 1 && t->fast.tab_len[0] <= 1024;
 }
 
+bool cross_active(const lutldpc_decoder *d) {
+    if (!d->opt.use_cross || !d->opt.skew || !d->skew_ok || d->psc || !d->min_lut || d->chain_vclass < 0 || d->n_cross_nodes == 0) return false;
+    for (int ii = 0; ii + 1 < d->max_iters; ii++) {
+        const TreeClassPlan *t = d->tree_class(TT_VAR, d->iter_set[(size_t)ii], d->chain_vclass);
+        if (!(t && t->fast.ok && t->fast.n_tables == 1 && t->fast.tab_len[0] <= 1024)) return false;
+    }
+    return true;
+}
+CrossPass cross_pass(const lutldpc_decoder *d, int ii) {
+    const int I = d->max_iters;
+    const int f0 = (d->opt.first_from_nodes || ((I - 1) & 1) == 0) ? 0 : 1;
+    if (ii < f0 || ii > I - 1) return {0, 0};
+    return {(I - 1 - ii) & 1, ii <= I - 2 ? 1 : 0};
+}
+
 int launch_late_hard(lutldpc_decoder *d, bool skewed, int g0, int G, const int32_t *ctl) {
     bool chain_skip = false;
     if (!late_hard_active(d, skewed, &chain_skip) || G <= 0) return LUTLDPC_OK;
diff --git a/lut_ldpc_amd/csrc/hip/kernels_common.hpp b/lut_ldpc_amd/csrc/hip/kernels_common.hpp
--- a/lut_ldpc_amd/csrc/hip/kernels_common.hpp
+++ b/lut_ldpc_amd/csrc/hip/kernels_common.hpp
@@ -143,7 +143,11 @@
     int32_t idx_off;
     int32_t tab_off, tab_len, tab_shift;
     int32_t check, hard, vfail_off_w, sbit_out;
-};
+    int32_t cross;
+    int32_t cross_off;
+};
+constexpr int kCrossMax = 1;
+constexpr int kCrossSlot = 2;
 struct ClassParams {
     int32_t kind;
     int32_t deg;
diff --git a/lut_ldpc_amd/csrc/hip/kernels_fast.hpp b/lut_ldpc_amd/csrc/hip/kernels_fast.hpp
--- a/lut_ldpc_amd/csrc/hip/kernels_fast.hpp
+++ b/lut_ldpc_amd/csrc/hip/kernels_fast.hpp
@@ -17,7 +17,7 @@
     const ChainParams CH = P.chain;
     if constexpr (CHAIN) {
         const int i = threadIdx.x;
-        if (CH.on && i < CH.tab_len / 4) reinterpret_cast<uint32_t *>(lds_tab)[i] = reinterpret_cast<const uint32_t *>(tables + CH.tab_off)[i];
+        if ((CH.on || CH.cross) && i < CH.tab_len / 4) reinterpret_cast<uint32_t *>(lds_tab)[i] = reinterpret_cast<const uint32_t *>(tables + CH.tab_off)[i];
         __syncthreads();
     }
     const int lane = threadIdx.x & 63;
@@ -54,13 +54,19 @@
     uint32_t xc = 0, xcn = 0;
     uint32_t pend = 0, pend_old = 0, chainfail = 0;
     int pend_e = 0;
+    constexpr bool CROSS = CHAIN && DEG > kCrossSlot;
+    const bool has_links = CH.on || CH.hard;
+    const int32_t *xlinks = CROSS ? fast_idx + CH.cross_off : nullptr;
+    int xp = 0, xpn = 0;
+    uint32_t xr = 0, xrn = 0;
     auto fetch = [&](int i, uint32_t (&xx)[UNR][DEG], int (&ee)[UNR][DEG]) {
 #pragma unroll
         for (int u = 0; u < UNR; u++) {
             const int ii = (i + u < last) ? i + u : last - 1;
 #pragma unroll
             for (int k = 0; k < DEG; k++) ee[u][k] = edges[(size_t)ii * DEG + k];
-            if constexpr (CHAIN) { lbn = links[2 * (size_t)ii]; lfn = links[2 * (size_t)ii + 1]; }
+            if constexpr (CHAIN) { lbn = has_links ? links[2 * (size_t)ii] : 0; lfn = has_links ? links[2 * (size_t)ii + 1] : 0; }
+            if constexpr (CROSS) xpn = CH.cross ? xlinks[(size_t)ii] : 0;
         }
 #pragma unroll
         for (int u = 0; u < UNR; u++) {
@@ -73,6 +79,7 @@
                 } else xx[u][k] = ld_row(base, (uint32_t)ee[u][k] * kRowBytes, off);
             }
             if constexpr (CHAIN) xcn = ld_row(cbase, (uint32_t)(lbn > 0 ? lbn - 1 : 0) * kRowBytes, (i + u < last && lbn > 0 && CH.on) ? lane4 : (lane4 | 0x80000000u));
+            if constexpr (CROSS) xrn = ld_row(cbase, (uint32_t)(xpn > 0 ? xpn - 1 : 0) * kRowBytes, (i + u < last && xpn > 0) ? lane4 : (lane4 | 0x80000000u));
         }
     };
     auto to_mc = [&](uint32_t xh) -> uint32_t {
@@ -154,6 +161,28 @@
             }
             }
             if (P.check) failw |= tn >> sbit;
+            if constexpr (CROSS) {
+                if (xp) {
+                    uint32_t o = 0;
+                    if constexpr (PACK == 2) {
+                        constexpr uint32_t NIB = 0x0F0F0F0Fu;
+                        const uint32_t i_lo = lshl_or(xr & NIB, CH.tab_shift, r[kCrossSlot] & NIB), i_hi = lshl_or((xr >> 4) & NIB, CH.tab_shift, (r[kCrossSlot] >> 4) & NIB);
+#pragma unroll 1
+                        for (int s = 0; s < 32; s += 8) {
+                            const uint32_t v0 = lds_tab[__builtin_amdgcn_ubfe(i_lo, (uint32_t)s, 8u)], v1 = lds_tab[__builtin_amdgcn_ubfe(i_hi, (uint32_t)s, 8u)];
+                            o = lshl_or(v0, s, o);
+                            o = lshl_or(v1, s + 4, o);
+                        }
+                    } else {
+#pragma unroll 1
+                        for (int s = 0; s < 32; s += 8) {
+                            const uint32_t b = __builtin_amdgcn_ubfe(r[kCrossSlot], (uint32_t)s, 8u), c = __builtin_amdgcn_ubfe(xr, (uint32_t)s, 8u);
+                            o = lshl_or((uint32_t)lds_tab[lshl_or(c, CH.tab_shift, b)], s, o);
+                        }
+                    }
+                    r[kCrossSlot] = o;
+                }
+            }
             if constexpr (CHAIN) {
                 [[maybe_unused]] constexpr int F = 4 * PACK, BITS = 8 / PACK;
                 if (lb && CH.hard) {
@@ -212,7 +241,7 @@
         uint32_t x[UNR][DEG], xn[UNR][DEG];
         int e[UNR][DEG], en[UNR][DEG];
         fetch(first, x, e);
-        if constexpr (CHAIN) { lb = lbn; lf = lfn; xc = xcn; }
+        if constexpr (CHAIN) { lb = lbn; lf = lfn; xc = xcn; xp = xpn; xr = xrn; }
         fetch(first + UNR, xn, en);
         eval(first, x, e);
         pipeline_entry_fence();
@@ -221,7 +250,7 @@
             for (int u = 0; u < UNR; u++)
 #pragma unroll
                 for (int k = 0; k < DEG; k++) { x[u][k] = xn[u][k]; e[u][k] = en[u][k]; }
-            if constexpr (CHAIN) { lb = lbn; lf = lfn; xc = xcn; }
+            if constexpr (CHAIN) { lb = lbn; lf = lfn; xc = xcn; xp = xpn; xr = xrn; }
             fetch(i + UNR, xn, en);
             eval(i, x, e);
         }
@@ -230,7 +259,7 @@
             uint32_t x[UNR][DEG];
             int e[UNR][DEG];
             fetch(i, x, e);
-            if constexpr (CHAIN) { lb = lbn; lf = lfn; xc = xcn; }
+            if constexpr (CHAIN) { lb = lbn; lf = lfn; xc = xcn; xp = xpn; xr = xrn; }
             eval(i, x, e);
         }
     }
@@ -519,10 +548,10 @@
     if (P.kind == 0) {
         constexpr auto degs = std::make_integer_sequence<int, MAXCN - 1>{};
         if (!P.first) {
-            if (P.chain.on || P.chain.hard) fused_cn_switch<PACK, true, false, kFusedAboDeg[BUCKET]>(P, rb, degs, msgs, state_w, vfail_w, fast_idx, lds_tab, cha, tables, hard, msg0);
+            if (P.chain.on || P.chain.hard || P.chain.cross) fused_cn_switch<PACK, true, false, kFusedAboDeg[BUCKET]>(P, rb, degs, msgs, state_w, vfail_w, fast_idx, lds_tab, cha, tables, hard, msg0);
             else fused_cn_switch<PACK, false, false, kFusedAboDeg[BUCKET]>(P, rb, degs, msgs, state_w, vfail_w, fast_idx, lds_tab, cha, tables, hard, msg0);
         } else {
-            if (P.chain.on) fused_cn_switch<PACK, true, true, kFusedAboDeg[BUCKET]>(P, rb, degs, msgs, state_w, vfail_w, fast_idx, lds_tab, cha, tables, hard, msg0);
+            if (P.chain.on || P.chain.cross) fused_cn_switch<PACK, true, true, kFusedAboDeg[BUCKET]>(P, rb, degs, msgs, state_w, vfail_w, fast_idx, lds_tab, cha, tables, hard, msg0);
             else fused_cn_switch<PACK, false, true, kFusedAboDeg[BUCKET]>(P, rb, degs, msgs, state_w, vfail_w, fast_idx, lds_tab, cha, tables, hard, msg0);
         }
     }
diff --git a/lut_ldpc_amd/decoder.py b/lut_ldpc_amd/decoder.py
--- a/lut_ldpc_amd/decoder.py
+++ b/lut_ldpc_amd/decoder.py
@@ -265,6 +265,25 @@
         lib.lutldpc_selftest_resident_source(self._h, int(G), buf, n, 0, info)
         return buf.value.decode(), tuple(info)
 
+    def cross_tables(self, cls: int):
+        out = []
+        for which in range(3):
+            n = lib.lutldpc_selftest_cross_tables(self._h, cls, which, None, 0)
+            if n < 0:
+                check(int(n))
+            a = np.zeros(max(int(n), 1), np.int32)
+            lib.lutldpc_selftest_cross_tables(self._h, cls, which, _p(a, C.c_int32), int(n))
+            out.append(a[:int(n)])
+        deg = self.describe()["cn_classes"][cls]["deg"]
+        return out[0].reshape(-1, deg), out[1].reshape(-1, deg), out[2]
+
+    def cross_plan(self):
+        plan = np.zeros(2 * 4096, np.int32)
+        n = lib.lutldpc_selftest_cross_plan(self._h, _p(plan, C.c_int32), len(plan))
+        if n < 0:
+            check(int(n))
+        return plan[:2 * n].reshape(n, 2)
+
     def program_eval(self, kind: int, tree_set: int, cls: int, inputs, n_out: int):
         a = _i32(inputs)
         out = np.zeros(n_out, np.int32)
```

Result: slower. 255,000 (-1.3%).
